# 0215Arthur/Pytorch_News_Recommender

Measured on AMD Instinct MI355X. Metric: users/sec (train step) NRMS MIND-small hist=50 cand=5, higher is better.
Workload: dtype f16 (MFMA inputs and saved activations; fp32 accumulate, softmax, loss, master weights and Adam); 1 GPU; configs[1] shapes: NRMS(nrms_v0) train step, 512 users/GPU, hist=50, cand=5, title_len=30, d=300, h=10, q=200, V=45800, dropout=0.2, Adam(lr=1e-3); users_per_gpu=512, global_batch=512, parallelism=dp1, precision=fp16, resident_batches=32

## Files before the change

include/nrms_hip.h:

```cpp
#ifndef NRMS_HIP_H
#define NRMS_HIP_H

#include <stddef.h>
#include <stdint.h>

#ifdef __cplusplus
extern "C" {
#endif

#define NRMS_OK            0
#define NRMS_EINVAL       -1
#define NRMS_ELAUNCH      -2
#define NRMS_EWORKSPACE   -3

#define NRMS_PRECISION_FP32   0
#define NRMS_PRECISION_BF16X3 1
#define NRMS_PRECISION_BF16   2
#define NRMS_FP16_KP 320
#define NRMS_FP16_DP 320
#define NRMS_FP16_QP 224
#define NRMS_PRECISION_FP16   3

#define NRMS_FLAG_PAD_ROW_ZERO 1
#define NRMS_FLAG_DEFER_WQKV 2
#define NRMS_FLAG_FWD_SCRATCH_KEPT 4
#define NRMS_FLAG_FUSED_SEQ64 8
#define NRMS_FLAG_DEFER_USER_JOIN 16

#define NRMS_FLAG_TABLE_ADAM 32

typedef struct nrms_encoder_desc {
    int32_t  n_seq;
    int32_t  seq_len;
    int32_t  d_model;
    int32_t  n_heads;
    int32_t  q_dim;
    int32_t  vocab;
    float    p_drop_embed;
    float    p_drop_ctx;
    int32_t  precision;
    int32_t  use_output_proj;
    int32_t  mask_mode;
    int32_t  flags;
    uint64_t seed;
    float    loss_scale;
    float    p_drop_attn;
    const int32_t* seq_index;
} nrms_encoder_desc;

typedef struct nrms_encoder_weights {
    const float* table;
    const float* w_qkv;
    const float* b_qkv;
    const float* w_o;
    const float* b_o;
    const float* w_add;
    const float* b_add;
    const float* q_vec;
} nrms_encoder_weights;

typedef struct nrms_encoder_grads {
    float* table;
    float* w_qkv;
    float* b_qkv;
    float* w_o;
    float* b_o;
    float* w_add;
    float* b_add;
    float* q_vec;
} nrms_encoder_grads;

typedef struct nrms_encoder_acts {
    float* x;
    float* qkv;
    float* attn;
    float* ctx;
    float* t;
    float* w;
    void*  scratch;
} nrms_encoder_acts;

size_t nrms_encoder_fwd_scratch_bytes(const nrms_encoder_desc* desc);
size_t nrms_encoder_fused_qkv_bytes(const nrms_encoder_desc* desc);
int nrms_encoder_fwd(const nrms_encoder_desc* desc, const nrms_encoder_weights* w,
                     const int64_t* ids, const float* x, const uint8_t* mask ,
                     const nrms_encoder_acts* acts, float* out, void* stream);

size_t nrms_encoder_bwd_workspace_bytes(const nrms_encoder_desc* desc);
int nrms_encoder_bwd(const nrms_encoder_desc* desc, const nrms_encoder_weights* w,
                     const int64_t* ids, const float* x, const uint8_t* mask,
                     const nrms_encoder_acts* acts, const float* dout,
                     const nrms_encoder_grads* grads, float* dx,
                     void* workspace, size_t workspace_bytes, void* stream);
typedef struct nrms_table_adam {
    float*   param;
    float*   exp_avg;
    float*   exp_avg_sq;
    double   lr, beta1, beta2, eps;
    int32_t  step;
    float    grad_scale;
    int32_t* n_nonfinite;
} nrms_table_adam;
int nrms_encoder_bwd_adam(const nrms_encoder_desc* desc, const nrms_encoder_weights* w,
                          const int64_t* ids, const float* x, const uint8_t* mask,
                          const nrms_encoder_acts* acts, const float* dout,
                          const nrms_encoder_grads* grads, float* dx,
                          void* workspace, size_t workspace_bytes, const nrms_table_adam* table_adam, void* stream);
int nrms_encoder_bwd_wqkv(const nrms_encoder_desc* desc, const int64_t* ids, const float* x,
                          const nrms_encoder_acts* acts, const nrms_encoder_grads* grads,
                          void* workspace, size_t workspace_bytes, void* stream);
int nrms_encoder_join(void* stream);

int nrms_sanitize_ids(const int64_t* src, int64_t* dst, int64_t n, int32_t vocab, int32_t* n_bad, void* stream);
int nrms_sanitize_ids_i32(const int32_t* src, int64_t* dst, int64_t n, int32_t vocab, int32_t* n_bad, void* stream);

int nrms_title_dedup(const int64_t* ids, int64_t n_titles, int32_t seq_len, int32_t* table, int64_t table_size,
                     int32_t* inverse, int32_t* rep_rows, int32_t* n_unique, void* stream);

int nrms_click_score_fwd(int32_t B, int32_t C, int32_t d, const float* cand, const float* user,
                         const uint8_t* mask, float* scores, void* stream);
int nrms_click_score_indexed(int32_t B, int32_t C, int32_t d, const float* news_vec, int64_t n_vec, const int32_t* index,
                             const float* user, const uint8_t* mask, float* scores, void* stream);
int nrms_click_score_bwd(int32_t B, int32_t C, int32_t d, const float* cand, const float* user,
                         const uint8_t* mask, const float* dscores, float* dcand, float* duser,
                         void* stream);

int nrms_ce_loss_fwd_bwd(int32_t B, int32_t C, const float* scores, float* loss_sum,
                         float* dscores, float grad_scale, void* stream);

int nrms_adam_step(size_t n, float* param, const float* grad, float* exp_avg, float* exp_avg_sq,
                   double lr, double beta1, double beta2, double eps, int32_t step, float grad_scale,
                   void* stream);

int nrms_adam_step_guarded(size_t n, float* param, const float* grad, float* exp_avg, float* exp_avg_sq,
                           double lr, double beta1, double beta2, double eps, int32_t step, float grad_scale,
                           int32_t* n_nonfinite, void* stream);
int nrms_adam_step_rest(size_t n, float* param, const float* grad, float* exp_avg, float* exp_avg_sq,
                        double lr, double beta1, double beta2, double eps, int32_t step, float grad_scale,
                        int32_t* n_nonfinite, void* stream);
int nrms_grad_guard(size_t n, float* grad, int32_t* n_nonfinite, void* stream);

int nrms_impression_auc(int32_t n_imp, int32_t max_c, const float* scores, const uint8_t* labels,
                        const int32_t* lens, double* auc, void* stream);

int nrms_impression_metrics(int32_t n_imp, int32_t max_c, const float* scores, const uint8_t* labels,
                            const int32_t* lens, int32_t k_a, int32_t k_b, double* auc, double* mrr, double* ndcg_a,
                            double* ndcg_b, int32_t* ranks, void* stream);

size_t nrms_topk_dot_workspace_bytes(int32_t B, int64_t N, int32_t d, int32_t k);
int nrms_topk_dot(int32_t B, int64_t N, int32_t d, int32_t k, const float* user, const float* items, const int64_t* exclude,
                  int32_t n_exclude, float* top_scores, int64_t* top_ids, void* workspace, size_t workspace_bytes, void* stream);

size_t nrms_topk_grouped_dot_workspace_bytes(int32_t B, int64_t N, int32_t d, int32_t k, int32_t G);
int nrms_topk_grouped_dot(int32_t B, int64_t N, int32_t d, int32_t k, int32_t G, const float* query, const float* items,
                          const int32_t* item_ids, const int64_t* group_ptr, const int64_t* exclude, int32_t n_exclude,
                          float* top_scores, int64_t* top_ids, void* workspace, size_t workspace_bytes, void* stream);

size_t nrms_rank_dot_workspace_bytes(int32_t B, int64_t N, int32_t d, int32_t T, int32_t n_exclude);
int nrms_rank_dot(int32_t B, int64_t N, int32_t d, int32_t T, const float* user, const float* items, const int64_t* targets,
                  const int64_t* exclude, int32_t n_exclude, int32_t* ranks, float* target_scores, void* workspace,
                  size_t workspace_bytes, void* stream);

size_t nrms_topk_dot_biased_workspace_bytes(int32_t B, int64_t N, int32_t d, int32_t k);
int nrms_topk_dot_biased(int32_t B, int64_t N, int32_t d, int32_t k, const float* user, const float* items,
                         const float* bias , const int64_t* exclude, int32_t n_exclude, float* top_scores,
                         int64_t* top_ids, void* workspace, size_t workspace_bytes, void* stream);
size_t nrms_rank_dot_biased_workspace_bytes(int32_t B, int64_t N, int32_t d, int32_t T, int32_t n_exclude);
int nrms_rank_dot_biased(int32_t B, int64_t N, int32_t d, int32_t T, const float* user, const float* items,
                         const float* bias , const int64_t* targets, const int64_t* exclude,
                         int32_t n_exclude, int32_t* ranks, float* target_scores, void* workspace, size_t workspace_bytes,
                         void* stream);

size_t nrms_softmax_sample_dot_workspace_bytes(int32_t B, int64_t N, int32_t d, int32_t S, int32_t n_exclude);
int nrms_softmax_sample_dot(int32_t B, int64_t N, int32_t d, int32_t S, const float* user, const float* items,
                            const int64_t* row_key , float inv_temperature, uint64_t seed,
                            const int64_t* exclude , int32_t n_exclude, int64_t* ids ,
                            float* keys , void* workspace, size_t workspace_bytes, void* stream);
int nrms_softmax_sample_noise(int32_t B, int64_t N, const int64_t* row_key , uint64_t seed,
                              uint32_t* words , float* gumbel , void* stream);

size_t nrms_mmr_rerank_workspace_bytes(int32_t B, int32_t M, int32_t d, int32_t k);
int nrms_mmr_rerank(int32_t B, int32_t M, int32_t d, int32_t k, int64_t N, float lambda,
                    const float* items , const int64_t* short_ids ,
                    const float* short_scores ,
                    int64_t* out_ids , float* out_scores ,
                    float* out_value , float* ild ,
                    void* workspace, size_t workspace_bytes, void* stream);

int nrms_layernorm_fwd(int64_t n_rows, int32_t d, const float* x, const float* gamma, const float* beta, float eps,
                       float* y, float* stats, void* stream);
size_t nrms_layernorm_bwd_workspace_bytes(int32_t d);
int nrms_layernorm_bwd(int64_t n_rows, int32_t d, const float* x, const float* gamma, const float* stats, const float* dy,
                       float* dx, float* dgamma_dbeta, void* workspace, size_t workspace_bytes, void* stream);

typedef struct nrms_news_features {
    int64_t n;
    int32_t d_text;
    int32_t d_cat;
    int32_t n_cat, n_sub;
    float   p_drop;
    uint64_t seed;
    const float* title_vec;
    const float* abst_vec;
    const float* cat_table;
    const float* sub_table;
    const int64_t* categ;
    const int64_t* subcateg;
} nrms_news_features;
// ... 130 lines not shown
```

pytorch_news_recommender_amd/_lib.py:

```python
from __future__ import annotations

import ctypes as C
import os

PKG = os.path.dirname(os.path.abspath(__file__))
LIB_PATH = os.environ.get("NRMS_HIP_LIB") or os.path.join(PKG, "libnrms_hip.so")

NRMS_OK, NRMS_EINVAL, NRMS_ELAUNCH, NRMS_EWORKSPACE = 0, -1, -2, -3
NRMS_FLAG_PAD_ROW_ZERO = 1
NRMS_FLAG_DEFER_WQKV = 2
NRMS_FLAG_FWD_SCRATCH_KEPT = 4
NRMS_FLAG_FUSED_SEQ64 = 8
NRMS_FLAG_DEFER_USER_JOIN = 16
NRMS_FLAG_TABLE_ADAM = 32
NRMS_PRECISION_FP32 = 0
NRMS_PRECISION_BF16X3 = 1
NRMS_PRECISION_BF16 = 2
NRMS_PRECISION_FP16 = 3
NRMS_DROPOUT_FIELDS16 = 0x100
NRMS_DROPOUT_SITE_NEWSVEC = 4
NRMS_FP16_KP, NRMS_FP16_DP, NRMS_FP16_QP = 320, 320, 224
PRECISIONS = {"fp32": 0, "bf16x3": 1, "bf16": 2, "fp16": 3}


class NrmsError(RuntimeError):
    pass


class EncoderDesc(C.Structure):
    _fields_ = [("n_seq", C.c_int32), ("seq_len", C.c_int32), ("d_model", C.c_int32),
                ("n_heads", C.c_int32), ("q_dim", C.c_int32), ("vocab", C.c_int32),
                ("p_drop_embed", C.c_float), ("p_drop_ctx", C.c_float), ("precision", C.c_int32),
                ("use_output_proj", C.c_int32), ("mask_mode", C.c_int32), ("flags", C.c_int32),
                ("seed", C.c_uint64), ("loss_scale", C.c_float), ("p_drop_attn", C.c_float), ("seq_index", C.c_void_p)]


class EncoderWeights(C.Structure):
    _fields_ = [("table", C.c_void_p), ("w_qkv", C.c_void_p), ("b_qkv", C.c_void_p), ("w_o", C.c_void_p),
                ("b_o", C.c_void_p), ("w_add", C.c_void_p), ("b_add", C.c_void_p), ("q_vec", C.c_void_p)]


class EncoderGrads(C.Structure):
    _fields_ = [("table", C.c_void_p), ("w_qkv", C.c_void_p), ("b_qkv", C.c_void_p), ("w_o", C.c_void_p),
                ("b_o", C.c_void_p), ("w_add", C.c_void_p), ("b_add", C.c_void_p), ("q_vec", C.c_void_p)]


class TableAdam(C.Structure):
    _fields_ = [("param", C.c_void_p), ("exp_avg", C.c_void_p), ("exp_avg_sq", C.c_void_p), ("lr", C.c_double), ("beta1", C.c_double),
                ("beta2", C.c_double), ("eps", C.c_double), ("step", C.c_int32), ("grad_scale", C.c_float), ("n_nonfinite", C.c_void_p)]


class EncoderActs(C.Structure):
    _fields_ = [("x", C.c_void_p), ("qkv", C.c_void_p), ("attn", C.c_void_p), ("ctx", C.c_void_p),
                ("t", C.c_void_p), ("w", C.c_void_p), ("scratch", C.c_void_p)]


class SegPoolDesc(C.Structure):
    _fields_ = [("n_rows", C.c_int64), ("n_seg", C.c_int64), ("nnz", C.c_int64), ("d", C.c_int32), ("q", C.c_int32),
                ("precision", C.c_int32), ("flags", C.c_int32)]


NRMS_SEGPOOL_ROWS_UNIQUE = 1


class ClickGraphDesc(C.Structure):
    _fields_ = [("n_users", C.c_int64), ("n_news", C.c_int64), ("n_edges", C.c_int64), ("user_ptr", C.c_void_p),
                ("user_news", C.c_void_p), ("news_ptr", C.c_void_p), ("news_users", C.c_void_p)]


class NewsFeatures(C.Structure):
    _fields_ = [("n", C.c_int64), ("d_text", C.c_int32), ("d_cat", C.c_int32), ("n_cat", C.c_int32), ("n_sub", C.c_int32),
                ("p_drop", C.c_float), ("seed", C.c_uint64), ("title_vec", C.c_void_p), ("abst_vec", C.c_void_p),
                ("cat_table", C.c_void_p), ("sub_table", C.c_void_p), ("categ", C.c_void_p), ("subcateg", C.c_void_p)]


class NewsvecDesc(C.Structure):
    _fields_ = [("n_slots", C.c_int64), ("n_rows", C.c_int32), ("d", C.c_int32), ("precision", C.c_int32),
                ("p_drop", C.c_float), ("seed", C.c_uint64)]


SIGNATURES = {
    "nrms_encoder_fwd": (C.c_int, [C.POINTER(EncoderDesc), C.POINTER(EncoderWeights), C.c_void_p, C.c_void_p,
                                   C.c_void_p, C.POINTER(EncoderActs), C.c_void_p, C.c_void_p]),
    "nrms_encoder_bwd_workspace_bytes": (C.c_size_t, [C.POINTER(EncoderDesc)]),
    "nrms_encoder_fwd_scratch_bytes": (C.c_size_t, [C.POINTER(EncoderDesc)]),
    "nrms_encoder_fused_qkv_bytes": (C.c_size_t, [C.POINTER(EncoderDesc)]),
    "nrms_encoder_bwd": (C.c_int, [C.POINTER(EncoderDesc), C.POINTER(EncoderWeights), C.c_void_p, C.c_void_p,
                                   C.c_void_p, C.POINTER(EncoderActs), C.c_void_p, C.POINTER(EncoderGrads), C.c_void_p,
                                   C.c_void_p, C.c_size_t, C.c_void_p]),
    "nrms_encoder_bwd_adam": (C.c_int, [C.POINTER(EncoderDesc), C.POINTER(EncoderWeights), C.c_void_p, C.c_void_p,
                                        C.c_void_p, C.POINTER(EncoderActs), C.c_void_p, C.POINTER(EncoderGrads), C.c_void_p,
                                        C.c_void_p, C.c_size_t, C.POINTER(TableAdam), C.c_void_p]),
    "nrms_encoder_bwd_wqkv": (C.c_int, [C.POINTER(EncoderDesc), C.c_void_p, C.c_void_p, C.POINTER(EncoderActs),
                                        C.POINTER(EncoderGrads), C.c_void_p, C.c_size_t, C.c_void_p]),
    "nrms_encoder_join": (C.c_int, [C.c_void_p]),
    "nrms_sanitize_ids": (C.c_int, [C.c_void_p, C.c_void_p, C.c_int64, C.c_int32, C.c_void_p, C.c_void_p]),
    "nrms_sanitize_ids_i32": (C.c_int, [C.c_void_p, C.c_void_p, C.c_int64, C.c_int32, C.c_void_p, C.c_void_p]),
    "nrms_title_dedup": (C.c_int, [C.c_void_p, C.c_int64, C.c_int32, C.c_void_p, C.c_int64, C.c_void_p, C.c_void_p,
                                   C.c_void_p, C.c_void_p]),
    "nrms_click_score_indexed": (C.c_int, [C.c_int32, C.c_int32, C.c_int32, C.c_void_p, C.c_int64, C.c_void_p, C.c_void_p,
                                           C.c_void_p, C.c_void_p, C.c_void_p]),
    "nrms_click_score_fwd": (C.c_int, [C.c_int32, C.c_int32, C.c_int32, C.c_void_p, C.c_void_p, C.c_void_p,
                                       C.c_void_p, C.c_void_p]),
    "nrms_click_score_bwd": (C.c_int, [C.c_int32, C.c_int32, C.c_int32, C.c_void_p, C.c_void_p, C.c_void_p,
                                       C.c_void_p, C.c_void_p, C.c_void_p, C.c_void_p]),
    "nrms_ce_loss_fwd_bwd": (C.c_int, [C.c_int32, C.c_int32, C.c_void_p, C.c_void_p, C.c_void_p, C.c_float,
                                       C.c_void_p]),
    "nrms_adam_step": (C.c_int, [C.c_size_t, C.c_void_p, C.c_void_p, C.c_void_p, C.c_void_p, C.c_double,
                                 C.c_double, C.c_double, C.c_double, C.c_int32, C.c_float, C.c_void_p]),
    "nrms_adam_step_guarded": (C.c_int, [C.c_size_t, C.c_void_p, C.c_void_p, C.c_void_p, C.c_void_p, C.c_double,
                                         C.c_double, C.c_double, C.c_double, C.c_int32, C.c_float, C.c_void_p, C.c_void_p]),
    "nrms_adam_step_rest": (C.c_int, [C.c_size_t, C.c_void_p, C.c_void_p, C.c_void_p, C.c_void_p, C.c_double,
                                      C.c_double, C.c_double, C.c_double, C.c_int32, C.c_float, C.c_void_p, C.c_void_p]),
    "nrms_grad_guard": (C.c_int, [C.c_size_t, C.c_void_p, C.c_void_p, C.c_void_p]),
    "nrms_segment_pool_workspace_bytes": (C.c_size_t, [C.POINTER(SegPoolDesc)]),
    "nrms_segment_pool_fwd": (C.c_int, [C.POINTER(SegPoolDesc)] + [C.c_void_p] * 10 + [C.c_void_p, C.c_size_t, C.c_void_p]),
    "nrms_segment_pool_bwd": (C.c_int, [C.POINTER(SegPoolDesc)] + [C.c_void_p] * 12 + [C.c_void_p, C.c_size_t, C.c_void_p]),
    "nrms_hier_tree_scratch_bytes": (C.c_size_t, [C.c_int32, C.c_int32]),
    "nrms_hier_tree_build": (C.c_int, [C.c_int32, C.c_int32] + [C.c_void_p] * 16 + [C.c_size_t, C.c_void_p]),
    "nrms_hier_add_embedding_fwd": (C.c_int, [C.c_int64, C.c_int32, C.c_int32, C.c_void_p, C.c_void_p, C.c_void_p, C.c_void_p, C.c_void_p]),
    "nrms_sequence_partition_count_ints": (C.c_size_t, [C.c_int32]),
    "nrms_sequence_partition": (C.c_int, [C.c_void_p, C.c_int32, C.c_int32, C.c_void_p, C.c_void_p, C.c_void_p]),
    "nrms_encoder_empty_workspace_bytes": (C.c_size_t, [C.POINTER(EncoderDesc)]),
    "nrms_encoder_empty_saved_bytes": (C.c_size_t, [C.POINTER(EncoderDesc)]),
    "nrms_encoder_empty_fwd": (C.c_int, [C.POINTER(EncoderDesc), C.POINTER(EncoderWeights), C.c_void_p, C.c_void_p, C.c_void_p, C.c_void_p, C.c_size_t,
                                         C.c_void_p]),
    "nrms_encoder_empty_bwd": (C.c_int, [C.POINTER(EncoderDesc), C.POINTER(EncoderWeights), C.c_void_p, C.c_void_p, C.c_void_p, C.POINTER(EncoderGrads),
                                         C.c_void_p, C.c_size_t, C.c_void_p]),
    "nrms_csr_from_padded": (C.c_int, [C.c_int64, C.c_int32, C.c_void_p, C.c_int64, C.c_void_p, C.c_void_p, C.c_void_p]),
    "nrms_graph_sample_workspace_bytes": (C.c_size_t, [C.c_int64, C.c_int32]),
    "nrms_graph_sample_neighbors": (C.c_int, [C.POINTER(ClickGraphDesc), C.c_int64, C.c_int32, C.c_void_p, C.c_uint64, C.c_void_p, C.c_void_p,
                                              C.c_void_p, C.c_size_t, C.c_void_p]),
    "nrms_graph_resolve_workspace_bytes": (C.c_size_t, [C.c_int64]),
    "nrms_graph_resolve_rows": (C.c_int, [C.c_int64, C.c_int32, C.c_int64, C.c_void_p, C.c_void_p, C.c_int32] + [C.c_void_p] * 4
                                + [C.c_void_p, C.c_size_t, C.c_void_p]),
    "nrms_negative_sample_workspace_bytes": (C.c_size_t, [C.c_int64, C.c_int64, C.c_int32]),
    "nrms_negative_sample": (C.c_int, [C.c_int64] + [C.c_void_p] * 4 + [C.c_int32, C.c_int32, C.c_uint64] + [C.c_void_p] * 3
                             + [C.c_void_p, C.c_size_t, C.c_void_p]),
    "nrms_catalogue_negative_sample_workspace_bytes": (C.c_size_t, [C.c_int64, C.c_int64, C.c_int32]),
    "nrms_catalogue_negative_sample": (C.c_int, [C.c_int64] + [C.c_void_p] * 3 + [C.c_int64, C.c_void_p, C.c_void_p, C.c_int64, C.c_void_p, C.c_int32,
                                                 C.c_uint64] + [C.c_void_p] * 4 + [C.c_void_p, C.c_size_t, C.c_void_p]),
    "nrms_hier_add_embedding_bwd_workspace_bytes": (C.c_size_t, [C.c_int64, C.c_int32, C.c_int32]),
    "nrms_hier_add_embedding_bwd": (C.c_int, [C.c_int64, C.c_int32, C.c_int32, C.c_void_p, C.c_void_p, C.c_void_p, C.c_void_p, C.c_void_p,
                                              C.c_size_t, C.c_void_p]),
    "nrms_hier_match": (C.c_int, [C.c_int32, C.c_int32, C.c_int32] + [C.c_void_p] * 11 + [C.c_void_p]),
    "nrms_hier_score_fwd": (C.c_int, [C.c_int32, C.c_int32, C.c_int32] + [C.c_void_p] * 9 + [C.c_float, C.c_float, C.c_void_p, C.c_void_p]),
    "nrms_hier_score_bwd": (C.c_int, [C.c_int32, C.c_int32, C.c_int32] + [C.c_void_p] * 9 + [C.c_float, C.c_float] + [C.c_void_p] * 5 + [C.c_void_p]),
    "nrms_impression_auc": (C.c_int, [C.c_int32, C.c_int32, C.c_void_p, C.c_void_p, C.c_void_p, C.c_void_p,
                                      C.c_void_p]),
    "nrms_impression_metrics": (C.c_int, [C.c_int32, C.c_int32, C.c_void_p, C.c_void_p, C.c_void_p, C.c_int32, C.c_int32]
                                + [C.c_void_p] * 5 + [C.c_void_p]),
    "nrms_topk_dot_workspace_bytes": (C.c_size_t, [C.c_int32, C.c_int64, C.c_int32, C.c_int32]),
    "nrms_topk_dot": (C.c_int, [C.c_int32, C.c_int64, C.c_int32, C.c_int32, C.c_void_p, C.c_void_p, C.c_void_p, C.c_int32,
                                C.c_void_p, C.c_void_p, C.c_void_p, C.c_size_t, C.c_void_p]),
    "nrms_topk_grouped_dot_workspace_bytes": (C.c_size_t, [C.c_int32, C.c_int64, C.c_int32, C.c_int32, C.c_int32]),
    "nrms_topk_grouped_dot": (C.c_int, [C.c_int32, C.c_int64, C.c_int32, C.c_int32, C.c_int32] + [C.c_void_p] * 5 + [C.c_int32]
                              + [C.c_void_p] * 3 + [C.c_size_t, C.c_void_p]),
    "nrms_rank_dot_workspace_bytes": (C.c_size_t, [C.c_int32, C.c_int64, C.c_int32, C.c_int32, C.c_int32]),
    "nrms_rank_dot": (C.c_int, [C.c_int32, C.c_int64, C.c_int32, C.c_int32] + [C.c_void_p] * 4 + [C.c_int32]
                      + [C.c_void_p] * 3 + [C.c_size_t, C.c_void_p]),
    "nrms_topk_dot_biased_workspace_bytes": (C.c_size_t, [C.c_int32, C.c_int64, C.c_int32, C.c_int32]),
    "nrms_topk_dot_biased": (C.c_int, [C.c_int32, C.c_int64, C.c_int32, C.c_int32] + [C.c_void_p] * 4 + [C.c_int32]
                             + [C.c_void_p] * 3 + [C.c_size_t, C.c_void_p]),
    "nrms_rank_dot_biased_workspace_bytes": (C.c_size_t, [C.c_int32, C.c_int64, C.c_int32, C.c_int32, C.c_int32]),
    "nrms_rank_dot_biased": (C.c_int, [C.c_int32, C.c_int64, C.c_int32, C.c_int32] + [C.c_void_p] * 5 + [C.c_int32]
                             + [C.c_void_p] * 3 + [C.c_size_t, C.c_void_p]),
    "nrms_softmax_sample_dot_workspace_bytes": (C.c_size_t, [C.c_int32, C.c_int64, C.c_int32, C.c_int32, C.c_int32]),
    "nrms_softmax_sample_dot": (C.c_int, [C.c_int32, C.c_int64, C.c_int32, C.c_int32] + [C.c_void_p] * 3 + [C.c_float, C.c_uint64, C.c_void_p,
                                          C.c_int32] + [C.c_void_p] * 3 + [C.c_size_t, C.c_void_p]),
    "nrms_mmr_rerank_workspace_bytes": (C.c_size_t, [C.c_int32] * 4),
    "nrms_mmr_rerank": (C.c_int, [C.c_int32] * 4 + [C.c_int64, C.c_float] + [C.c_void_p] * 8 + [C.c_size_t, C.c_void_p]),
    "nrms_softmax_sample_noise": (C.c_int, [C.c_int32, C.c_int64, C.c_void_p, C.c_uint64, C.c_void_p, C.c_void_p, C.c_void_p]),
    "nrms_hier_query": (C.c_int, [C.c_int32] * 4 + [C.c_void_p] * 10 + [C.c_float, C.c_float, C.c_void_p, C.c_void_p]),
    "nrms_dropout_keep_mask": (C.c_int, [C.c_uint64, C.c_int32, C.c_int64, C.c_int32, C.c_float, C.c_void_p,
                                         C.c_void_p]),
    "nrms_layernorm_fwd": (C.c_int, [C.c_int64, C.c_int32, C.c_void_p, C.c_void_p, C.c_void_p, C.c_float, C.c_void_p,
                                     C.c_void_p, C.c_void_p]),
    "nrms_layernorm_bwd_workspace_bytes": (C.c_size_t, [C.c_int32]),
    "nrms_layernorm_bwd": (C.c_int, [C.c_int64, C.c_int32, C.c_void_p, C.c_void_p, C.c_void_p, C.c_void_p, C.c_void_p,
                                     C.c_void_p, C.c_void_p, C.c_size_t, C.c_void_p]),
    "nrms_news_features_fwd": (C.c_int, [C.POINTER(NewsFeatures), C.c_void_p, C.c_void_p]),
    "nrms_news_features_bwd": (C.c_int, [C.POINTER(NewsFeatures), C.c_void_p, C.c_void_p, C.c_void_p, C.c_void_p,
                                         C.c_void_p, C.c_void_p]),
    "nrms_newsvec_saved_bytes": (C.c_size_t, [C.POINTER(NewsvecDesc)]),
    "nrms_newsvec_workspace_bytes": (C.c_size_t, [C.POINTER(NewsvecDesc)]),
    "nrms_newsvec_fwd": (C.c_int, [C.POINTER(NewsvecDesc)] + [C.c_void_p] * 6 + [C.c_size_t, C.c_void_p, C.c_void_p, C.c_size_t,
                                                                                C.c_void_p]),
    "nrms_newsvec_bwd": (C.c_int, [C.POINTER(NewsvecDesc)] + [C.c_void_p] * 4 + [C.c_size_t] + [C.c_void_p] * 4
# ... 44 lines not shown
```

pytorch_news_recommender_amd/csrc/capi.hip:

```cpp
#include <stdarg.h>

#include <algorithm>

#include <mutex>
#include <vector>

#include "gemm.h"

namespace nrms {

int launch_attention(bool bwd, int n_seq, int S, int d, int h, const float* qkv, float* ctx, const Dropout& drop,
                     const float* dctx, float* dqkv, const uint8_t* mask, const int64_t* ids, const float* bias_hm,
                     const int* pos, float* padsum, float* dbias, hipStream_t stream, const Dropout* pdrop = nullptr,
                     bool split = false);
size_t attention_padsum_floats();
int launch_addattn_fwd(int n_seq, int S, int d, int q, const float* ctx, const float* w_add, const float* b_add,
                       const float* q_vec, float* T, float* wout, float* out, const uint8_t* mask, int npass,
                       void* wplanes, hipStream_t stream);
int addattn_bwd_rows_waves(int n_seq);
int launch_addattn_bwd_rows(int n_seq, int S, int d, int q, const float* ctx, const float* dout, const float* w,
                            const float* T, float* ds, float* dq_partial, float* dq, const uint8_t* mask,
                            hipStream_t stream);

int launch_attention_wide(bool bwd, int n_seq, int S, int d, int h, const float* qkv, float* ctx, const Dropout& pdrop,
// ... 274 lines not shown
        if (!forked) return NRMS_OK;
        forked = false;
        if (hipEventRecord(ss->ev[4], s_prep) != hipSuccess || hipStreamWaitEvent(s, ss->ev[4], 0) != hipSuccess) {
            set_error("encoder_fwd(fp16): joining the helper stream failed");
            return NRMS_ELAUNCH;
        }
        return NRMS_OK;
    };
    rc = v1 ? launch_prep16v1(d, h, q, w->w_qkv, w->b_qkv, w->w_o, w->b_o, w->w_add, w->b_add, w->q_vec, base + fs.planes, s_prep)
            : launch_prep16(d, h, q, w->w_qkv, w->b_qkv, w->w_add, w->b_add, w->q_vec, base + fs.planes, s_prep);
    if (rc) { (void)join_prep(); return rc; }
    Fused16Fwd f{};
    f.n_seq = desc->n_seq; f.S = S; f.d = d; f.h = h; f.q = q;
    f.planes = base + fs.planes; f.x16 = acts->x; f.ctx16 = acts->ctx; f.t16 = acts->t; f.w = acts->w; f.out = out;
    f.drop = make_dropout(desc->seed, desc->p_drop_ctx);
    if (gather) {
        const Dropout drop_e = make_dropout(desc->seed, desc->p_drop_embed);
        if (skip_pad_rows(desc)) {
            int* live = (int*)(base + fs.live);
            int* pos = (int*)(base + fs.pos);
            int* n_live = (int*)(base + fs.n_live);
            int* order = (int*)(base + fs.order);
            int* order_cnt = (int*)(base + fs.order_cnt);
            rc = S <= 32 ? launch_title_order(desc->n_seq, S, ids, order, order_cnt, s_prep, 3) : NRMS_OK;
            if (rc) { (void)join_prep(); return rc; }
            rc = launch_compact_live_rows(M, ids, live, pos, n_live, (int*)(base + fs.cscr), s);
            if (rc == NRMS_OK) rc = launch_gather16(M, d, L.KP, ids, live, n_live, w->table, drop_e, acts->x, s);
            const int rj = join_prep();
            if (rc) return rc;
            if (rj) return rj;
            f.pos = pos;
            f.n_rows = n_live;
            f.ids = ids;
            if (S <= 32) { f.order = order; f.order_cnt = order_cnt; }
        } else {
            rc = launch_gather16(M, d, L.KP, ids, nullptr, nullptr, w->table, drop_e, acts->x, s);
            if (rc) return rc;
        }
    } else {
        rc = launch_cast16(M, d, L.KP, x, acts->x, s);
        if (rc) return rc;
    }
    rc = v1 ? launch_fused_fwd16v1(f, h, acts->attn, s) : launch_fused_fwd16(f, s);
    if (rc == NRMS_OK && gather && skip_pad_rows(desc)) kept_record(desc, acts->scratch, ids);
    return rc;
}

struct Bwd16Layout { size_t fused, live, pos, n_live, cscr, order, order_cnt, dxc, sscr, total; };
static Bwd16Layout bwd16_layout(const nrms_encoder_desc* d) {
    Bwd16Layout L;
    const size_t M = (size_t)d->n_seq * d->seq_len;
    const bool gather = d->vocab > 0;
    size_t off = 0;
    auto take = [&](size_t bytes) { size_t o = off; off = align_up(off + bytes, 256); return o; };
    L.fused = take(d->use_output_proj ? fused16v1_bwd_bytes((long)M, d->n_seq, d->n_heads) : fused16_bwd_layout((long)M, d->n_seq).total);
    L.live = take(gather ? M * sizeof(int) : 0);
    L.pos = take(gather ? M * sizeof(int) : 0);
    L.n_live = take(gather ? 256 : 0);
    L.cscr = take(gather ? compact_scratch_ints((long)M) * sizeof(int) : 0);
    L.order = take(gather ? (size_t)3 * d->n_seq * sizeof(int) : 0);
    L.order_cnt = take(gather ? title_order_cnt_ints(d->n_seq) * sizeof(int) : 0);
    L.dxc = take(gather ? M * std::max((size_t)d->d_model * sizeof(float), (size_t)NRMS_FP16_KP * 2) : 0);
    L.sscr = take(gather ? scatter_grouped_scratch_ints((long)M, d->vocab) * sizeof(int) : 0);
    L.total = off;
    return L;
}

static int table_adam_args(const nrms_encoder_desc* desc, const nrms_encoder_weights* w, const nrms_encoder_grads* grads,
                           const nrms_table_adam* ta, TableAdam* out) {
    NRMS_REQUIRE(ta->param && ta->exp_avg && ta->exp_avg_sq && ta->step >= 1, "encoder_bwd: NRMS_FLAG_TABLE_ADAM: bad operands");
    NRMS_REQUIRE(w != nullptr && ta->param == w->table, "encoder_bwd: NRMS_FLAG_TABLE_ADAM: param must be the table the encoder reads");
    NRMS_REQUIRE(grads != nullptr && grads->table != nullptr, "encoder_bwd: NRMS_FLAG_TABLE_ADAM: grads.table missing");
    NRMS_REQUIRE((((uintptr_t)ta->param | (uintptr_t)grads->table | (uintptr_t)ta->exp_avg | (uintptr_t)ta->exp_avg_sq) & 15) == 0,
                 "encoder_bwd: NRMS_FLAG_TABLE_ADAM: buffers must be 16-byte aligned");
    out->p = ta->param; out->m = ta->exp_avg; out->v = ta->exp_avg_sq;
    out->c = adam_consts(ta->lr, ta->beta1, ta->beta2, ta->eps, ta->step);
    out->gscale = ta->grad_scale;
    out->n_bad = (int*)ta->n_nonfinite;
    return NRMS_OK;
}

static int encoder_bwd16(const nrms_encoder_desc* desc, const nrms_encoder_weights* w, const int64_t* ids, const float* x,
                         const nrms_encoder_acts* acts, const float* dout, const nrms_encoder_grads* grads, float* dx,
                         void* workspace, size_t workspace_bytes, const TableAdam* tadam, hipStream_t s) {
    NRMS_REQUIRE(w && acts && dout && grads && workspace, "encoder_bwd(fp16): null argument");
    const bool v1 = desc->use_output_proj != 0;
    NRMS_REQUIRE(!v1 || (w->w_o && acts->attn && grads->w_o && grads->b_o),
                 "encoder_bwd(fp16): use_output_proj needs w_o, acts.attn, grads.w_o, grads.b_o");
    NRMS_REQUIRE(acts->x && acts->ctx && acts->t && acts->w, "encoder_bwd(fp16): acts.x, ctx, t, w are required");
    NRMS_REQUIRE(grads->w_qkv && grads->b_qkv && grads->w_add && grads->b_add && grads->q_vec, "encoder_bwd(fp16): null gradient buffer");
    const bool gather = desc->vocab > 0;
    NRMS_REQUIRE(gather ? (ids != nullptr && grads->table != nullptr) : (dx != nullptr), "encoder_bwd(fp16): %s missing",
                 gather ? "ids / grads.table" : "dx");
    const Bwd16Layout L = bwd16_layout(desc);
    if (workspace_bytes < L.total) { set_error("encoder_bwd(fp16): workspace %zu < required %zu bytes", workspace_bytes, L.total); return NRMS_EWORKSPACE; }
    NRMS_REQUIRE(((uintptr_t)workspace & 255) == 0, "encoder_bwd(fp16): workspace must be 256-byte aligned");
    if (desc->n_seq == 0) return NRMS_OK;
    const int S = desc->seq_len, d = desc->d_model;
    const long M = (long)desc->n_seq * S;
    char* base = (char*)workspace;
    Fused16Bwd f{};
    f.n_seq = desc->n_seq; f.S = S; f.d = d; f.h = desc->n_heads; f.q = desc->q_dim;
    f.workspace = base + L.fused;
    f.w_qkv = w->w_qkv; f.b_qkv = w->b_qkv; f.w_add = w->w_add; f.q_vec = w->q_vec;
    f.x16 = acts->x; f.ctx16 = acts->ctx; f.t16 = acts->t; f.w = acts->w; f.dout = dout;
    f.loss_scale = desc->loss_scale;
    f.drop = make_dropout(desc->seed, desc->p_drop_ctx);
    f.dw_qkv = grads->w_qkv; f.db_qkv = grads->b_qkv; f.dw_add = grads->w_add; f.db_add = grads->b_add; f.dq_vec = grads->q_vec;
    if (v1) { f.w_o = w->w_o; f.attn16 = acts->attn; f.dw_o = grads->w_o; f.db_o = grads->b_o; }
    int rc;
    int* live = (int*)(base + L.live);
    int* n_live = (int*)(base + L.n_live);
    if (gather) {
        const bool kept = (desc->flags & NRMS_FLAG_FWD_SCRATCH_KEPT) != 0 && skip_pad_rows(desc) && acts->scratch != nullptr &&
                          kept_matches(desc, acts->scratch, ids);
        if (kept) {
            const Fwd16Scratch fs = fwd16_scratch(desc);
            char* fb = (char*)acts->scratch;
            live = (int*)(fb + fs.live);
            n_live = (int*)(fb + fs.n_live);
            f.pos = (int*)(fb + fs.pos); f.n_rows_dev = n_live; f.ids = ids;
            if (S <= 32) { f.order = (int*)(fb + fs.order); f.order_cnt = (int*)(fb + fs.order_cnt); }
        } else {
            int* pos = (int*)(base + L.pos);
            rc = launch_compact_live_rows(M, ids, live, pos, n_live, (int*)(base + L.cscr), s);
            if (rc) return rc;
            if (skip_pad_rows(desc)) {
                int* order = (int*)(base + L.order);
                int* order_cnt = (int*)(base + L.order_cnt);
                f.pos = pos; f.n_rows_dev = n_live; f.ids = ids;
                if (S <= 32) {
                    rc = launch_title_order(desc->n_seq, S, ids, order, order_cnt, s, 3);
                    if (rc) return rc;
                    f.order = order; f.order_cnt = order_cnt;
                }
            }
        }
        f.dx = (float*)(base + L.dxc);
        f.dx_fp16 = skip_pad_rows(desc);
    } else {
        f.dx = dx;
    }
    SideSet* ss_prep = (gather && skip_pad_rows(desc)) ? side_streams_for(s) : nullptr;
    bool prepared = false;
    if (ss_prep != nullptr) {
        rc = side_order(ss_prep, 5, s, ss_prep->s[1], "encoder_bwd(fp16)");
        if (rc) return rc;
        rc = launch_scatter_prepare(M, desc->vocab, ids, live, n_live, (int*)(base + L.sscr), ss_prep->s[1]);
        if (hipEventRecord(ss_prep->ev[4], ss_prep->s[1]) != hipSuccess) { set_error("encoder_bwd(fp16): hipEventRecord failed"); return NRMS_ELAUNCH; }
        if (rc) { (void)hipStreamWaitEvent(s, ss_prep->ev[4], 0); return rc; }
        prepared = true;
    }
    auto join_prepare = [&]() -> int {
        if (!prepared) return NRMS_OK;
        if (hipStreamWaitEvent(s, ss_prep->ev[4], 0) != hipSuccess) { set_error("encoder_bwd(fp16): hipStreamWaitEvent failed"); return NRMS_ELAUNCH; }
        return NRMS_OK;
    };
    const float* sc_dev = nullptr;
    f.sc_out = &sc_dev;
    f.defer_join = (desc->flags & NRMS_FLAG_DEFER_WQKV) != 0;
    rc = v1 ? launch_fused_bwd16v1(f, s) : launch_fused_bwd16(f, s);
    {
        const int rj = join_prepare();
        if (rc) return rc;
        if (rj) return rj;
    }
    if (gather) {
        const Dropout drop_e = make_dropout(desc->seed, desc->p_drop_embed);
        if (tadam != nullptr)
            rc = launch_scatter_grouped_adam(M, desc->vocab, d, ids, live, n_live, f.dx, drop_e, grads->table, (int*)(base + L.sscr), s,
                                             f.dx_fp16, NRMS_FP16_KP, sc_dev, prepared, *tadam);
        else if (skip_pad_rows(desc))
            rc = launch_scatter_grouped(M, desc->vocab, d, ids, live, n_live, f.dx, drop_e, grads->table, (int*)(base + L.sscr), s,
                                        f.dx_fp16, NRMS_FP16_KP, sc_dev, prepared);
        else
            rc = launch_scatter_dense_rows(M, d, ids, live, n_live, f.dx, drop_e, grads->table, s);
    }
    return rc;
}

extern "C" int nrms_encoder_fwd(const nrms_encoder_desc* desc, const nrms_encoder_weights* w, const int64_t* ids,
                                const float* x, const uint8_t* mask, const nrms_encoder_acts* acts, float* out,
                                void* stream) {
    int rc = validate_desc(desc, "encoder_fwd");
    if (rc) return rc;
    NRMS_REQUIRE((desc->flags & NRMS_FLAG_TABLE_ADAM) == 0, "encoder_fwd: flags 0x%x: NRMS_FLAG_TABLE_ADAM belongs to nrms_encoder_bwd_adam", desc->flags);
    if (acts != nullptr) kept_forget(acts->scratch);
    if (desc->precision == NRMS_PRECISION_FP16) {
        NRMS_REQUIRE(w && acts && out, "encoder_fwd: null argument");
        NRMS_REQUIRE(w->w_qkv && w->b_qkv && w->w_add && w->b_add && w->q_vec, "encoder_fwd: null weight");
        NRMS_REQUIRE(desc->vocab > 0 ? (ids != nullptr && w->table != nullptr) : (x != nullptr), "encoder_fwd: input missing");
        if (desc->n_seq == 0) return NRMS_OK;
        return encoder_fwd16(desc, w, ids, x, acts, out, (hipStream_t)stream);
    }
    NRMS_REQUIRE(w && acts && out, "encoder_fwd: null argument");
    NRMS_REQUIRE(w->w_qkv && w->b_qkv && w->w_add && w->b_add && w->q_vec, "encoder_fwd: null weight");
    if (desc->flags & NRMS_FLAG_FUSED_SEQ64) {
        NRMS_REQUIRE(x != nullptr && acts->qkv != nullptr && acts->scratch != nullptr, "encoder_fwd(fused): x, acts.qkv and acts.scratch are required");
        const bool train = acts->ctx != nullptr && acts->t != nullptr && acts->w != nullptr;
        if (desc->n_seq == 0) return NRMS_OK;
        rc = fused_bwd16_join((hipStream_t)stream);
        if (rc) return rc;
        return launch_user64_fwd(desc->n_seq, desc->seq_len, desc->d_model, desc->n_heads, desc->q_dim, x, w->w_qkv, w->b_qkv, w->w_add,
                                 w->b_add, w->q_vec, acts->scratch, acts->ctx, acts->t, acts->w, acts->qkv, out, train, (hipStream_t)stream);
    }
    NRMS_REQUIRE(acts->qkv && acts->ctx, "encoder_fwd: acts.qkv / acts.ctx are required");
    const bool gather = desc->vocab > 0, wo = desc->use_output_proj != 0;
    NRMS_REQUIRE(gather ? (ids != nullptr && w->table != nullptr) : (x != nullptr),
                 "encoder_fwd: %s input missing", gather ? "ids/table" : "x");
    NRMS_REQUIRE(!wo || (w->w_o && w->b_o && acts->attn), "encoder_fwd: use_output_proj needs w_o, b_o and acts.attn");
    NRMS_REQUIRE(desc->mask_mode == 0 || mask != nullptr, "encoder_fwd: mask_mode=%d but mask is null", desc->mask_mode);
    if (desc->n_seq == 0) return NRMS_OK;
    hipStream_t s = (hipStream_t)stream;
    const int S = desc->seq_len, d = desc->d_model, q = desc->q_dim, M = desc->n_seq * S;
    const Dropout drop_e = make_dropout(desc->seed, desc->p_drop_embed);
    const Dropout drop_c = make_dropout(desc->seed, desc->p_drop_ctx);
    const Dropout no_drop = make_dropout(0, 0.f);
    const uint8_t* amask = (desc->mask_mode & 1) ? mask : nullptr;
    const uint8_t* pmask = (desc->mask_mode & 2) ? mask : nullptr;

    NRMS_REQUIRE(acts->scratch != nullptr, "encoder_fwd: acts.scratch (nrms_encoder_fwd_scratch_bytes) is required");
    const FwdScratch fs = fwd_scratch(desc);
    float* wq_hm = (float*)((char*)acts->scratch + fs.wq);
    float* bq_hm = (float*)((char*)acts->scratch + fs.bq);
    void* wplanes = (char*)acts->scratch + fs.planes;
    const HeadPerm perm{d / desc->n_heads, desc->n_heads};
    rc = launch_permute_rows(w->w_qkv, w->b_qkv, wq_hm, bq_hm, 3 * d, d, perm, s);
    if (rc) return rc;

    NTArgs g{};
    g.M = M; g.N = 3 * d; g.K = d; g.rows_per_tile = NT_BM;
    g.W = wq_hm; g.bias = bq_hm; g.C = acts->qkv; g.ldc = 3 * d;
    const float* xin = x;
    if (gather) {
        NRMS_REQUIRE(acts->x != nullptr, "encoder_fwd: acts.x (gathered embeddings) is required for the news encoder");
        if (skip_pad_rows(desc)) {
            int* live = (int*)((char*)acts->scratch + fs.live);
            int* n_live = (int*)((char*)acts->scratch + fs.n_live);
            int* cscr = (int*)((char*)acts->scratch + fs.cscr);
            rc = launch_compact_live_rows((long)M, ids, live, nullptr, n_live, cscr, s);
            if (rc) return rc;
            rc = launch_gather_dropout_compact((long)M, d, ids, live, n_live, w->table, drop_e, acts->x, s);
            if (rc) return rc;
// ... 72 lines not shown
        if (e.device == dev && e.caller == caller) return e.set;
    if (g_side_sets.size() >= 32) return nullptr;
    SideSet* ss = new SideSet();
    bool ok = true;
    for (int i = 0; i < 2 && ok; ++i) ok = hipStreamCreateWithFlags(&ss->s[i], hipStreamNonBlocking) == hipSuccess;
    for (int i = 0; i < SIDE_EVENTS && ok; ++i) ok = hipEventCreateWithFlags(&ss->ev[i], hipEventDisableTiming) == hipSuccess;
    if (!ok) {
        for (int i = 0; i < 2; ++i) if (ss->s[i]) (void)hipStreamDestroy(ss->s[i]);
        for (int i = 0; i < SIDE_EVENTS; ++i) if (ss->ev[i]) (void)hipEventDestroy(ss->ev[i]);
        delete ss;
        ss = nullptr;
        (void)hipGetLastError();
    }
    g_side_sets.push_back(SideEntry{dev, caller, ss});
    return ss;
}

int side_order(SideSet* ss, int e, hipStream_t from, hipStream_t to, const char* what) {
    if (hipEventRecord(ss->ev[e], from) != hipSuccess || hipStreamWaitEvent(to, ss->ev[e], 0) != hipSuccess) {
        set_error("%s: ordering the helper stream failed: %s", what, hipGetErrorString(hipGetLastError()));
        return NRMS_ELAUNCH;
    }
    return NRMS_OK;
}

int side_join_user(SideSet* ss, hipStream_t caller, const char* what) {
    if (ss == nullptr || !ss->pending_user) return NRMS_OK;
    ss->pending_user = false;
    if (hipStreamWaitEvent(caller, ss->ev[SIDE_EV_USER], 0) != hipSuccess) {
        set_error("%s: hipStreamWaitEvent failed", what);
        return NRMS_ELAUNCH;
    }
    return NRMS_OK;
}

SideJoinGuard::~SideJoinGuard() {
    if (!armed) return;
    for (int i = 0; i < 2; ++i)
        if (hipEventRecord(ss->ev[6 + i], ss->s[i]) == hipSuccess) (void)hipStreamWaitEvent(caller, ss->ev[6 + i], 0);
}
}

static int bwd_wqkv(const nrms_encoder_desc* desc, const float* xin, const float* dqkv, const int* n_live,
                    const nrms_encoder_grads* grads, float* tn_partial, hipStream_t s) {
    const int d = desc->d_model, M = desc->n_seq * desc->seq_len;
    TNArgs t{};
    t.M = M; t.N = 3 * d; t.K = d; t.amode = A_PLAIN;
    t.A = dqkv; t.lda = 3 * d; t.B = xin; t.ldb = d;
    t.dW = grads->w_qkv; t.dbias = grads->b_qkv; t.partial = tn_partial;
    t.perm = HeadPerm{d / desc->n_heads, desc->n_heads};
    if (skip_pad_rows(desc)) t.m_dev = n_live;
    return tn_gemm(desc, t, s, "dwqkv_bwd");
}

extern "C" int nrms_encoder_bwd_wqkv(const nrms_encoder_desc* desc, const int64_t* ids, const float* x,
                                     const nrms_encoder_acts* acts, const nrms_encoder_grads* grads, void* workspace,
                                     size_t workspace_bytes, void* stream) {
    int rc = validate_desc(desc, "encoder_bwd_wqkv");
    if (rc) return rc;
    NRMS_REQUIRE((desc->flags & NRMS_FLAG_TABLE_ADAM) == 0, "encoder_bwd_wqkv: flags 0x%x: NRMS_FLAG_TABLE_ADAM belongs to nrms_encoder_bwd_adam", desc->flags);
    if (desc->precision == NRMS_PRECISION_FP16) return fused_bwd16_join((hipStream_t)stream);
    NRMS_REQUIRE(acts && grads && workspace, "encoder_bwd_wqkv: null argument");
    NRMS_REQUIRE(grads->w_qkv && grads->b_qkv, "encoder_bwd_wqkv: null gradient buffer");
    const bool gather = desc->vocab > 0;
    NRMS_REQUIRE(gather ? (ids != nullptr && acts->x != nullptr) : (x != nullptr), "encoder_bwd_wqkv: input missing");
    if (desc->n_seq == 0) return NRMS_OK;
    const BwdWorkspace L = bwd_layout(desc);
    if (workspace_bytes < L.total) {
        set_error("encoder_bwd_wqkv: workspace %zu < required %zu bytes", workspace_bytes, L.total);
        return NRMS_EWORKSPACE;
    }
    rc = fused_bwd16_join((hipStream_t)stream);
    if (rc) return rc;
    char* base = (char*)workspace;
    return bwd_wqkv(desc, gather ? acts->x : x, (const float*)(base + L.dqkv), (const int*)(base + L.n_live), grads,
                    (float*)(base + L.tn_partial), (hipStream_t)stream);
}

extern "C" int nrms_encoder_join(void* stream) { return fused_bwd16_join((hipStream_t)stream); }

static int encoder_bwd_chain(const nrms_encoder_desc* desc, const nrms_encoder_weights* w, const int64_t* ids,
                             const float* x, const uint8_t* mask, const nrms_encoder_acts* acts, const float* dout,
                             const nrms_encoder_grads* grads, float* dx, void* workspace, size_t workspace_bytes,
                             const TableAdam* tadam, hipStream_t s) {
    int rc;
    NRMS_REQUIRE(w && acts && dout && grads && workspace, "encoder_bwd: null argument");
    NRMS_REQUIRE(acts->qkv && acts->ctx && acts->t && acts->w, "encoder_bwd: all saved activations are required");
    NRMS_REQUIRE(grads->w_qkv && grads->b_qkv && grads->w_add && grads->b_add && grads->q_vec,
                 "encoder_bwd: null gradient buffer");
    const bool gather = desc->vocab > 0, wo = desc->use_output_proj != 0;
    NRMS_REQUIRE(gather ? (ids != nullptr && acts->x != nullptr && grads->table != nullptr) : (x != nullptr && dx != nullptr),
                 "encoder_bwd: %s missing", gather ? "ids/acts.x/grads.table" : "x/dx");
    NRMS_REQUIRE(!wo || (w->w_o && acts->attn && grads->w_o && grads->b_o),
                 "encoder_bwd: use_output_proj needs w_o, acts.attn, grads.w_o, grads.b_o");
    NRMS_REQUIRE(desc->mask_mode == 0 || mask != nullptr, "encoder_bwd: mask_mode=%d but mask is null", desc->mask_mode);
    const BwdWorkspace L = bwd_layout(desc);
    if (workspace_bytes < L.total) {
        set_error("encoder_bwd: workspace %zu < required %zu bytes", workspace_bytes, L.total);
        return NRMS_EWORKSPACE;
    }
    NRMS_REQUIRE(((uintptr_t)workspace & 255) == 0, "encoder_bwd: workspace must be 256-byte aligned");
    if (desc->n_seq == 0) return NRMS_OK;
    const int S = desc->seq_len, d = desc->d_model, q = desc->q_dim, M = desc->n_seq * S;
    const Dropout drop_e = make_dropout(desc->seed, desc->p_drop_embed);
    const Dropout drop_c = make_dropout(desc->seed, desc->p_drop_ctx);
    const Dropout no_drop = make_dropout(0, 0.f);
    const uint8_t* amask = (desc->mask_mode & 1) ? mask : nullptr;
    const uint8_t* pmask = (desc->mask_mode & 2) ? mask : nullptr;
    char* base = (char*)workspace;
    float* dctx = (float*)(base + L.dctx);
    float* dqkv = (float*)(base + L.dqkv);
    float* dattn = (float*)(base + L.dattn);
    float* ds = (float*)(base + L.ds);
    float* wqkv_t = (float*)(base + L.wqkv_t);
    float* wadd_t = (float*)(base + L.wadd_t);
    float* wo_t = (float*)(base + L.wo_t);
    float* tn_partial = (float*)(base + L.tn_partial);
    float* dq_partial = (float*)(base + L.dq_partial);
    void* wplanes = (void*)(base + L.wplanes);

    rc = fused_bwd16_join(s);
    if (rc) return rc;
    SideSet* ss = side_streams_for(s);
    const bool side = ss != nullptr;
    hipStream_t s2 = side ? ss->s[0] : s;
    SideJoinGuard join_guard(ss, s);
    auto fork = [&](int i) -> int {
        return side ? side_order(ss, i, s, s2, "encoder_bwd") : NRMS_OK;
    };

    const bool fused64 = (desc->flags & NRMS_FLAG_FUSED_SEQ64) != 0;
    if (fused64) {
        rc = launch_user64_bwd(desc->n_seq, S, d, desc->n_heads, q, w->w_add, w->q_vec, base + L.u64planes, dout, acts->t, acts->w,
                               acts->qkv, ds, dq_partial, grads->q_vec, dqkv, s);
        if (rc) return rc;
    } else {
        if (wide_additive(desc))
            rc = launch_addattn_rows_bwd_wide(desc->n_seq, S, d, q, acts->ctx, dout, acts->w, acts->t, ds, dq_partial, grads->q_vec,
                                              pmask, s);
        else
            rc = launch_addattn_bwd_rows(desc->n_seq, S, d, q, acts->ctx, dout, acts->w, acts->t, ds, dq_partial, grads->q_vec,
                                         pmask, s);
        if (rc) return rc;
    }
    rc = fork(0);
    if (rc) return rc;
    {
        TNArgs t{};
        t.M = M; t.N = q; t.K = d; t.amode = A_DZ;
        t.ds = ds; t.qv = w->q_vec; t.T = acts->t; t.B = acts->ctx; t.ldb = d;
        t.dW = grads->w_add; t.dbias = grads->b_add; t.partial = tn_partial;
        rc = tn_gemm(desc, t, s2, "dwadd_bwd");
        if (rc) return rc;
    }
    if (!fused64) {
        rc = launch_transpose(w->w_add, wadd_t, q, d, s);
        if (rc) return rc;
        {
            NTArgs g{};
            g.M = M; g.N = d; g.K = q; g.rows_per_tile = NT_BM;
            g.ds = ds; g.qv = w->q_vec; g.T = acts->t;
            g.W = wadd_t; g.C = dctx; g.ldc = d;
            g.wrow = acts->w; g.dout = dout; g.seq_of_row = make_row_div((uint32_t)S);
            g.drop = drop_c;
            rc = nt_gemm(desc, A_DZ, E_DCTX, g, wplanes, s, "dctx_bwd");
            if (rc) return rc;
        }
}
    const float* dattn_in = dctx;
    if (wo) {
        rc = fork(1);
        if (rc) return rc;
        TNArgs t{};
        t.M = M; t.N = d; t.K = d; t.amode = A_PLAIN;
        t.A = dctx; t.lda = d; t.B = acts->attn; t.ldb = d;
        t.dW = grads->w_o; t.dbias = grads->b_o; t.partial = tn_partial;
        rc = tn_gemm(desc, t, s2, "dwo_bwd");
        if (rc) return rc;
        if (side && hipEventRecord(ss->ev[3], s2) != hipSuccess) {
            set_error("encoder_bwd: hipEventRecord failed");
            return NRMS_ELAUNCH;
        }
        rc = launch_transpose(w->w_o, wo_t, d, d, s);
        if (rc) return rc;
        NTArgs g{};
        g.M = M; g.N = d; g.K = d; g.rows_per_tile = NT_BM;
        g.A = dctx; g.lda = d; g.W = wo_t; g.C = dattn; g.ldc = d;
        rc = nt_gemm(desc, A_PLAIN, E_STORE, g, wplanes, s, "dattn_bwd");
        if (rc) return rc;
        dattn_in = dattn;
    }
    int* live = (int*)(base + L.live);
    int* pos = (int*)(base + L.pos);
    int* n_live = (int*)(base + L.n_live);
    const bool compact = skip_pad_rows(desc);
    const HeadPerm perm{d / desc->n_heads, desc->n_heads};
    if (gather) {
        rc = launch_compact_live_rows((long)M, ids, live, compact ? pos : nullptr, n_live, (int*)(base + L.cscr), s);
        if (rc) return rc;
    }
    Dropout pdrop_attn = make_dropout(desc->seed, desc->p_drop_attn);
    pdrop_attn.seq_index = desc->seq_index; pdrop_attn.seq_h = desc->n_heads;
    if (fused64)
        rc = NRMS_OK;
    else if (wide_attention(desc))
        rc = launch_attention_wide(true, desc->n_seq, S, d, desc->n_heads, acts->qkv, nullptr, pdrop_attn, dattn_in, dqkv, amask, s);
    else
        rc = launch_attention(true, desc->n_seq, S, d, desc->n_heads, acts->qkv, nullptr, no_drop, dattn_in, dqkv, amask,
                              nullptr, nullptr, compact ? pos : nullptr, compact ? (float*)(base + L.padsum) : nullptr,
                              compact ? grads->b_qkv : nullptr, s, &pdrop_attn, desc->precision != NRMS_PRECISION_FP32);
    if (rc) return rc;
    if ((desc->flags & NRMS_FLAG_DEFER_WQKV) == 0) {
        rc = fork(2);
        if (rc) return rc;
        rc = bwd_wqkv(desc, gather ? acts->x : x, dqkv, n_live, grads, tn_partial, s2);
        if (rc) return rc;
    }
    rc = launch_transpose(w->w_qkv, wqkv_t, 3 * d, d, s, perm);
    if (rc) return rc;
    {
        NTArgs g{};
        g.M = M; g.N = d; g.K = 3 * d; g.rows_per_tile = NT_BM;
        g.A = dqkv; g.lda = 3 * d; g.W = wqkv_t;
        g.C = gather ? dctx : dx; g.ldc = d;
        if (gather) { g.a_rows = compact ? nullptr : live; g.m_dev = n_live; }
        if (side && wo && gather && hipStreamWaitEvent(s, ss->ev[3], 0) != hipSuccess) {
            set_error("encoder_bwd: hipStreamWaitEvent failed");
            return NRMS_ELAUNCH;
        }
        rc = nt_gemm(desc, A_PLAIN, E_STORE, g, wplanes, s, "dx_bwd");
        if (rc) return rc;
    }
    if (gather) {
        const bool atomic_scatter = getenv("NRMS_ATOMIC_SCATTER") != nullptr;
        if (tadam != nullptr)
            rc = launch_scatter_grouped_adam((long)M, desc->vocab, d, ids, live, n_live, dctx, drop_e, grads->table,
                                             (int*)(base + L.sscr), s, false, 0, nullptr, false, *tadam);
        else if (atomic_scatter) rc = launch_scatter_dropout_compact((long)M, d, ids, live, n_live, dctx, drop_e, grads->table, s);
        else rc = launch_scatter_grouped((long)M, desc->vocab, d, ids, live, n_live, dctx, drop_e, grads->table,
                                         (int*)(base + L.sscr), s);
    }
    if (side && rc == NRMS_OK) {
        if (!gather && (desc->flags & NRMS_FLAG_DEFER_USER_JOIN) != 0) {
            if (hipEventRecord(ss->ev[SIDE_EV_USER], s2) != hipSuccess) { set_error("encoder_bwd: hipEventRecord failed"); return NRMS_ELAUNCH; }
            ss->pending_user = true;
            join_guard.disarm();
        } else {
            rc = side_order(ss, 4, s2, s, "encoder_bwd");
            if (rc == NRMS_OK) join_guard.disarm();
        }
    }
    return rc;
}

extern "C" int nrms_encoder_bwd(const nrms_encoder_desc* desc, const nrms_encoder_weights* w, const int64_t* ids,
                                const float* x, const uint8_t* mask, const nrms_encoder_acts* acts, const float* dout,
                                const nrms_encoder_grads* grads, float* dx, void* workspace, size_t workspace_bytes,
                                void* stream) {
    return nrms_encoder_bwd_adam(desc, w, ids, x, mask, acts, dout, grads, dx, workspace, workspace_bytes, nullptr, stream);
}

extern "C" int nrms_encoder_bwd_adam(const nrms_encoder_desc* desc, const nrms_encoder_weights* w, const int64_t* ids,
                                     const float* x, const uint8_t* mask, const nrms_encoder_acts* acts, const float* dout,
                                     const nrms_encoder_grads* grads, float* dx, void* workspace, size_t workspace_bytes,
                                     const nrms_table_adam* table_adam, void* stream) {
    int rc = validate_desc(desc, "encoder_bwd");
    if (rc) return rc;
    NRMS_REQUIRE(((desc->flags & NRMS_FLAG_TABLE_ADAM) != 0) == (table_adam != nullptr),
                 "encoder_bwd: NRMS_FLAG_TABLE_ADAM and the nrms_table_adam operands (nrms_encoder_bwd_adam) go together");
    TableAdam tadam_v{};
    const TableAdam* tadam = nullptr;
    if (table_adam != nullptr) {
        rc = table_adam_args(desc, w, grads, table_adam, &tadam_v);
        if (rc) return rc;
        tadam = &tadam_v;
        NRMS_REQUIRE(desc->precision == NRMS_PRECISION_FP16 || getenv("NRMS_ATOMIC_SCATTER") == nullptr,
                     "encoder_bwd: NRMS_FLAG_TABLE_ADAM needs the grouped scatter (NRMS_ATOMIC_SCATTER is set)");
    }
    if (desc->precision == NRMS_PRECISION_FP16)
        rc = encoder_bwd16(desc, w, ids, x, acts, dout, grads, dx, workspace, workspace_bytes, tadam, (hipStream_t)stream);
    else
        rc = encoder_bwd_chain(desc, w, ids, x, mask, acts, dout, grads, dx, workspace, workspace_bytes, tadam, (hipStream_t)stream);
    if (rc == NRMS_OK && tadam != nullptr && desc->n_seq == 0) {
        const size_t n = (size_t)desc->vocab * desc->d_model;
        if (hipMemsetAsync(grads->table, 0, n * sizeof(float), (hipStream_t)stream) != hipSuccess) {
            set_error("encoder_bwd: memset failed");
            return NRMS_ELAUNCH;
        }
        rc = table_adam->n_nonfinite != nullptr
                 ? nrms_adam_step_guarded(n, table_adam->param, grads->table, table_adam->exp_avg, table_adam->exp_avg_sq, table_adam->lr,
                                          table_adam->beta1, table_adam->beta2, table_adam->eps, table_adam->step, table_adam->grad_scale,
                                          table_adam->n_nonfinite, stream)
                 : nrms_adam_step(n, table_adam->param, grads->table, table_adam->exp_avg, table_adam->exp_avg_sq, table_adam->lr,
                                  table_adam->beta1, table_adam->beta2, table_adam->eps, table_adam->step, table_adam->grad_scale, stream);
    }
    return rc;
}

extern "C" int nrms_layernorm_fwd(int64_t n_rows, int32_t d, const float* x, const float* gamma, const float* beta, float eps,
                                  float* y, float* stats, void* stream) {
    NRMS_REQUIRE(n_rows >= 0 && d > 0 && eps > 0.f, "layernorm_fwd: n_rows=%ld d=%d eps=%g", (long)n_rows, d, (double)eps);
    NRMS_REQUIRE(n_rows == 0 || (x && gamma && beta && y), "layernorm_fwd: null argument");
    return launch_layernorm_fwd((long)n_rows, d, x, gamma, beta, eps, y, stats, (hipStream_t)stream);
}

extern "C" size_t nrms_layernorm_bwd_workspace_bytes(int32_t d) { return d > 0 ? layernorm_bwd_workspace_floats(d) * sizeof(float) : 0; }

extern "C" int nrms_layernorm_bwd(int64_t n_rows, int32_t d, const float* x, const float* gamma, const float* stats,
                                  const float* dy, float* dx, float* dgamma_dbeta, void* workspace, size_t workspace_bytes,
                                  void* stream) {
    NRMS_REQUIRE(n_rows >= 0 && d > 0, "layernorm_bwd: n_rows=%ld d=%d", (long)n_rows, d);
    NRMS_REQUIRE(n_rows == 0 || (x && gamma && stats && dy && dx && dgamma_dbeta && workspace), "layernorm_bwd: null argument");
    if (workspace_bytes < nrms_layernorm_bwd_workspace_bytes(d)) {
        set_error("layernorm_bwd: workspace %zu < required %zu bytes", workspace_bytes, nrms_layernorm_bwd_workspace_bytes(d));
        return NRMS_EWORKSPACE;
    }
    return launch_layernorm_bwd((long)n_rows, d, x, gamma, stats, dy, dx, dgamma_dbeta, (float*)workspace, (hipStream_t)stream);
}

static int features_args(const nrms_news_features* f, FeatArgs* a, const char* who) {
    NRMS_REQUIRE(f != nullptr, "%s: null descriptor", who);
    NRMS_REQUIRE(f->n >= 0 && f->d_text > 0 && f->d_cat > 0 && f->n_cat > 0 && f->n_sub > 0, "%s: bad sizes", who);
    NRMS_REQUIRE(f->p_drop >= 0.f && f->p_drop < 1.f, "%s: p_drop must be in [0,1)", who);
    NRMS_REQUIRE((long)f->n * (2 * f->d_text + 2 * f->d_cat) < (1L << 40), "%s: too many elements", who);
    NRMS_REQUIRE(f->n == 0 || (f->categ && f->subcateg), "%s: null ids", who);
    a->n = (long)f->n; a->dt = f->d_text; a->dc = f->d_cat; a->n_cat = f->n_cat; a->n_sub = f->n_sub;
    a->title = f->title_vec; a->abst = f->abst_vec; a->cat_table = f->cat_table; a->sub_table = f->sub_table;
    a->categ = f->categ; a->subcateg = f->subcateg;
    a->drop = make_dropout(f->seed, f->p_drop);
    return NRMS_OK;
}

extern "C" int nrms_news_features_fwd(const nrms_news_features* f, float* out, void* stream) {
    FeatArgs a{};
    int rc = features_args(f, &a, "news_features_fwd");
    if (rc) return rc;
    NRMS_REQUIRE(f->n == 0 || (f->title_vec && f->abst_vec && f->cat_table && f->sub_table && out), "news_features_fwd: null argument");
    a.out = out;
    return launch_features_fwd(a, (hipStream_t)stream);
}

extern "C" int nrms_news_features_bwd(const nrms_news_features* f, const float* dout, float* d_title_vec, float* d_abst_vec,
                                      float* d_cat_table, float* d_sub_table, void* stream) {
    FeatArgs a{};
    int rc = features_args(f, &a, "news_features_bwd");
    if (rc) return rc;
    NRMS_REQUIRE(f->n == 0 || (dout && d_title_vec && d_abst_vec && d_cat_table && d_sub_table), "news_features_bwd: null argument");
    a.dout = dout; a.d_title = d_title_vec; a.d_abst = d_abst_vec; a.d_cat_table = d_cat_table; a.d_sub_table = d_sub_table;
    return launch_features_bwd(a, (hipStream_t)stream);
}

extern "C" int nrms_sanitize_ids(const int64_t* src, int64_t* dst, int64_t n, int32_t vocab, int32_t* n_bad, void* stream) {
    NRMS_REQUIRE(n >= 0 && vocab > 0, "sanitize_ids: n=%ld vocab=%d", (long)n, vocab);
    NRMS_REQUIRE(n == 0 || (src && dst && n_bad), "sanitize_ids: null argument");
    return launch_sanitize_ids((long)n, src, false, dst, vocab, n_bad, (hipStream_t)stream);
}

extern "C" int nrms_sanitize_ids_i32(const int32_t* src, int64_t* dst, int64_t n, int32_t vocab, int32_t* n_bad, void* stream) {
    NRMS_REQUIRE(n >= 0 && vocab > 0, "sanitize_ids_i32: n=%ld vocab=%d", (long)n, vocab);
    NRMS_REQUIRE(n == 0 || (src && dst && n_bad), "sanitize_ids_i32: null argument");
    return launch_sanitize_ids((long)n, src, true, dst, vocab, n_bad, (hipStream_t)stream);
}

extern "C" size_t nrms_sequence_partition_count_ints(int32_t n_seq) { return n_seq >= 0 ? title_order_cnt_ints(n_seq) : 0; }

// ... 50 lines not shown
```

pytorch_news_recommender_amd/csrc/common.h:

```cpp
#pragma once
#include <hip/hip_runtime.h>
#include <stdint.h>
#include <stdio.h>
#include <string>

#include "../../include/nrms_hip.h"

namespace nrms {

typedef float f32x4 __attribute__((ext_vector_type(4)));
typedef float f32x16 __attribute__((ext_vector_type(16)));

constexpr int WAVE = 64;

__device__ __forceinline__ f32x4 mfma16(float a, float b, f32x4 c) {
    return __builtin_amdgcn_mfma_f32_16x16x4f32(a, b, c, 0, 0, 0);
}
__device__ __forceinline__ f32x16 mfma32(float a, float b, f32x16 c) {
    return __builtin_amdgcn_mfma_f32_32x32x2f32(a, b, c, 0, 0, 0);
}
__device__ __forceinline__ int crow32(int r, int hh) { return (r & 3) + 8 * (r >> 2) + 4 * hh; }

struct Keep4 { bool k[4]; };

// ... 54 lines not shown
    uint32_t r[4];
    philox4x32_7(seed, group8, site, r);
#pragma unroll
    for (int w = 0; w < 4; ++w) {
        s[2 * w] = (r[w] & 0xFFFFu) >= thresh16 ? inv_keep : 0.f;
        s[2 * w + 1] = (r[w] >> 16) >= thresh16 ? inv_keep : 0.f;
    }
}
__device__ __forceinline__ float dropout_scale1(uint64_t seed, uint32_t site, uint64_t elem,
                                                uint32_t thresh, float inv_keep) {
    uint32_t r[4];
    philox4x32_7(seed, elem >> 2, site, r);
    return r[elem & 3] >= thresh ? inv_keep : 0.f;
}

__device__ __forceinline__ float fast_tanh(float x) {
    const float e = __expf(2.0f * x);
    const float r = 1.0f - 2.0f * __builtin_amdgcn_rcpf(e + 1.0f);
    const float x2 = x * x;
    const float p = x * (1.0f + x2 * (-0.33333333f + x2 * (0.13333333f + x2 * -0.053968254f)));
    return fabsf(x) < 0.12f ? p : r;
}

struct HeadPerm {
    int dk, h;
    __host__ __device__ __forceinline__ int src(int np) const {
        if (dk == 0) return np;
        const int head = np / (3 * dk), r = np - head * 3 * dk;
        const int which = r / dk, j = r - which * dk;
        return which * h * dk + head * dk + j;
    }
};

struct Dropout {
    uint64_t seed;
    uint32_t thresh;
    float inv_keep;
    uint32_t thresh16;
    const int* seq_index;
    int seq_h;
    __device__ __forceinline__ long unit_of(long unit) const {
        if (seq_index == nullptr) return unit;
        const long seq = unit / seq_h;
        return (long)seq_index[seq] * seq_h + (unit - seq * seq_h);
    }
};

inline Dropout make_dropout(uint64_t seed, float p) {
    Dropout d;
    d.seed = seed;
    d.thresh = drop_threshold(p);
    d.thresh16 = drop_threshold16(p);
    d.inv_keep = p > 0.f ? 1.0f / (1.0f - p) : 1.0f;
    d.seq_index = nullptr;
    d.seq_h = 1;
    return d;
}

__device__ __forceinline__ float wave_sum(float v) {
#pragma unroll
    for (int o = 32; o > 0; o >>= 1) v += __shfl_xor(v, o, 64);
    return v;
}
__device__ __forceinline__ float wave_max(float v) {
#pragma unroll
    for (int o = 32; o > 0; o >>= 1) v = fmaxf(v, __shfl_xor(v, o, 64));
    return v;
}

__device__ __forceinline__ void adam_update(float& p, float& m, float& v, float g, float step_size, float b1, float b2, float omb1,
                                            float omb2, float inv_sqrt_bc2, float eps) {
#pragma clang fp contract(off)
    m = b1 * m + omb1 * g;
    v = b2 * v + omb2 * g * g;
    const float denom = sqrtf(v) * inv_sqrt_bc2 + eps;
    p = __builtin_fmaf(-step_size, m / denom, p);
}
struct AdamConsts { float step_size, b1, b2, omb1, omb2, inv_sqrt_bc2, eps; };
AdamConsts adam_consts(double lr, double beta1, double beta2, double eps, int32_t step);

void set_error(const char* fmt, ...);
int check_launch(const char* what);

constexpr int SIDE_EVENTS = 9, SIDE_EV_USER = 8;
struct SideSet {
    hipStream_t s[2] = {nullptr, nullptr};
    hipEvent_t ev[SIDE_EVENTS] = {nullptr, nullptr, nullptr, nullptr, nullptr, nullptr, nullptr, nullptr, nullptr};
    bool pending = false;
    bool pending_user = false;
};
int side_join_user(SideSet* ss, hipStream_t caller, const char* what);
SideSet* side_streams_for(hipStream_t caller);
int side_order(SideSet* ss, int e, hipStream_t from, hipStream_t to, const char* what);
struct SideJoinGuard {
    SideSet* ss; hipStream_t caller; bool armed;
    SideJoinGuard(SideSet* set, hipStream_t c) : ss(set), caller(c), armed(set != nullptr) {}
    void disarm() { armed = false; }
    ~SideJoinGuard();
};

struct TimingScope {
    TimingScope(const char* name, hipStream_t s);
    ~TimingScope();
    bool active;
    int slot;
    hipStream_t stream;
};

#define NRMS_REQUIRE(cond, ...)                         \
    do {                                                \
        if (!(cond)) {                                  \
            ::nrms::set_error(__VA_ARGS__);             \
            return NRMS_EINVAL;                         \
        }                                               \
    } while (0)

__host__ __device__ inline int cdiv(long a, long b) { return (int)((a + b - 1) / b); }

}
```

pytorch_news_recommender_amd/csrc/fused16_bwd.hip:

```cpp
#include <stdlib.h>

#include "fused16_bwd.h"

namespace nrms {

template <int SB>
__global__ __launch_bounds__(F16_THREADS, SB == 1 ? 8 / F16_WAVES : 1) void fused_bwd16_pool_kernel(Bwd16Args a) {
    extern __shared__ __attribute__((aligned(16))) char smem[];
    float* red = reinterpret_cast<float*>(smem + 3 * F16_SLOT);
    float* stg_t = red + B16_RED;
    float* stg_h = stg_t + F16_WAVES * SB * 2 * F16_QT * 32;
    const int tid = threadIdx.x, lane = tid & 63;
    const int wave = __builtin_amdgcn_readfirstlane(tid >> 6);
    const int l32 = lane & 31, hh = lane >> 5;
    const int S = a.S;
    constexpr int DP = F16_DP, QP = F16_QP;

    for (int i = tid; i < B16_RED; i += F16_THREADS) red[i] = 0.f;

    h8 idf[2], sel[2];
#pragma unroll
    for (int s = 0; s < 2; ++s)
#pragma unroll
        for (int j = 0; j < 8; ++j) {
// ... 800 lines not shown
            }
        }
#pragma unroll
        for (int i = 0; i < T16_B_IT; ++i) {
            int r, c;
            slot_rc(tid + T16_THREADS * i, T16_BW, r, c);
            if (r < T16_MC) {
                const bool ok = m0 + r < m_end && kcol0 + c < a.K;
                *reinterpret_cast<h8*>(st + T16_A_BYTES + (r * T16_PB + c) * 2) = ok ? R.b[i] : z8;
            }
        }
    };
    f32x4 acc[T16_NTN][T16_NTK];
#pragma unroll
    for (int i = 0; i < T16_NTN; ++i)
#pragma unroll
        for (int j = 0; j < T16_NTK; ++j) acc[i][j] = f32x4{0.f, 0.f, 0.f, 0.f};
    auto compute = [&](const char* st) {
        h8 bf[T16_NTK];
#pragma unroll
        for (int j = 0; j < T16_NTK; ++j) bf[j] = tr16_frag(st + T16_A_BYTES, T16_PB * 2, (wk * T16_NTK + j) * 16, lane);
#pragma unroll
        for (int i = 0; i < T16_NTN; ++i) {
            const h8 af = tr16_frag(st, T16_PA * 2, (wn * T16_NTN + i) * 16, lane);
#pragma unroll
            for (int j = 0; j < T16_NTK; ++j) acc[i][j] = __builtin_amdgcn_mfma_f32_16x16x32_f16(af, bf[j], acc[i][j], 0, 0, 0);
        }
    };
    int n_stage = m_end > m_begin ? (m_end - m_begin + T16_MC - 1) / T16_MC : 0;
    if (n_stage > 0) {
        n_stage = (n_stage + 1) & ~1;
        Regs R0, R1;
        load_stage(R1, m_begin);
        store_stage(R1, m_begin, smem);
        load_stage(R0, m_begin + T16_MC);
        __syncthreads();
        auto body = [&](const Regs& Rs, Regs& Rl, int s) {
            load_stage(Rl, m_begin + (s + 2) * T16_MC);
            store_stage(Rs, m_begin + (s + 1) * T16_MC, smem + ((s + 1) & 1) * T16_STAGE);
            compute(smem + (s & 1) * T16_STAGE);
            __syncthreads();
        };
        for (int s = 0; s < n_stage; s += 2) {
            body(R0, R1, s);
            body(R1, R0, s + 1);
        }
    }
    float* slab = a.partial + (long)split * a.N * a.K;
    const int r16 = lane & 15, kq = lane >> 4;
#pragma unroll
    for (int i = 0; i < T16_NTN; ++i)
#pragma unroll
        for (int j = 0; j < T16_NTK; ++j)
#pragma unroll
            for (int reg = 0; reg < 4; ++reg) {
                const int nn = ncol0 + (wn * T16_NTN + i) * 16 + 4 * kq + reg;
                const int kk = kcol0 + (wk * T16_NTK + j) * 16 + r16;
                if (nn < a.N && kk < a.K) slab[(long)nn * a.K + kk] = acc[i][j][reg];
            }
}

__global__ void tn16_reduce_kernel(const float* partial, int splits, int N, int K, const int* nmap, const int* kmap,
                                   const float* nscale, int ldw, float* dW, float* dbias) {
    const long total = (long)N * K;
    for (long idx = (long)blockIdx.x * blockDim.x + threadIdx.x; idx < total; idx += (long)gridDim.x * blockDim.x) {
        const int n = (int)(idx / K), k = (int)(idx - (long)n * K);
        const int nd = nmap[n], kd = kmap[k];
        if (nd < 0 || kd == -1 || (kd < 0 && dbias == nullptr)) continue;
        const float* pp = partial + idx;
        float s[8] = {0.f, 0.f, 0.f, 0.f, 0.f, 0.f, 0.f, 0.f};
        int sp = 0;
        for (; sp + 8 <= splits; sp += 8) {
#pragma unroll
            for (int u = 0; u < 8; ++u) s[u] += pp[(long)(sp + u) * total];
        }
        for (; sp < splits; ++sp) s[0] += pp[(long)sp * total];
        const float tot = (((s[0] + s[1]) + (s[2] + s[3])) + ((s[4] + s[5]) + (s[6] + s[7]))) * nscale[n];
        if (kd >= 0) dW[(long)nd * ldw + kd] += tot;
        else dbias[nd] += tot;
    }
}

__global__ __launch_bounds__(1024) void red16_kernel(const float* red, int n_wg, int h, int dk, int d, int q, const float* sc,
                                                    float qscale, float* db_qkv, float* db_add, float* dq_vec) {
    const float inv_scale = sc[1];
    __shared__ float part[32][33];
    const int c = threadIdx.x & 31, rg = threadIdx.x >> 5;
    const int i = blockIdx.x * 32 + c;
    float s = 0.f;
    if (i < B16_RED) {
        float s0 = 0.f, s1 = 0.f, s2 = 0.f, s3 = 0.f;
        int g = rg;
        for (; g + 96 < n_wg; g += 128) {
            s0 += red[(long)g * B16_RED + i];
            s1 += red[(long)(g + 32) * B16_RED + i];
            s2 += red[(long)(g + 64) * B16_RED + i];
            s3 += red[(long)(g + 96) * B16_RED + i];
        }
        for (; g < n_wg; g += 32) s0 += red[(long)g * B16_RED + i];
        s = (s0 + s1) + (s2 + s3);
    }
    part[rg][c] = s;
    __syncthreads();
    if (rg != 0 || i >= B16_RED) return;
    s = 0.f;
#pragma unroll
    for (int r = 0; r < 32; ++r) s += part[r][c];
    s *= inv_scale;
    if (i < B16_RED_QKV) {
        const int tile = i >> 5, f = i & 31, head = tile / 3, which = tile - 3 * head;
        if (head < h && f < dk) db_qkv[which * d + head * dk + f] += s * (which == 0 ? qscale : 1.0f);
    } else if (i < B16_RED_QKV + F16_QP) {
        const int qq = i - B16_RED_QKV;
        if (qq < q) db_add[qq] += s;
    } else {
        const int qq = i - B16_RED_QKV - F16_QP;
        if (qq < q) dq_vec[qq] += s;
    }
}

struct Maps16 { int *nmap_qkv, *kmap_x, *nmap_add, *kmap_ctx; float *nscale_qkv, *nscale_add; };
__device__ __forceinline__ void maps16_entry(int i, int d, int h, int dk, int q, float inv_scale, float qscale, const Maps16& m) {
    int* const nmap_qkv = m.nmap_qkv; int* const kmap_x = m.kmap_x; int* const nmap_add = m.nmap_add; int* const kmap_ctx = m.kmap_ctx;
    float* const nscale_qkv = m.nscale_qkv; float* const nscale_add = m.nscale_add;
    if (i < B16_DQ) {
        const int head = i / 96, rem = i - head * 96, which = rem >> 5, p = rem & 31;
        const int s = p >> 4, t = p & 15, hh = t >> 3, jj = t & 7;
        const int f = 16 * s + 8 * (jj >> 2) + 4 * hh + (jj & 3);
        nmap_qkv[i] = (head < h && f < dk) ? which * d + head * dk + f : -1;
        nscale_qkv[i] = inv_scale * (which == 0 ? qscale : 1.0f);
    }
    if (i < F16_KP) kmap_x[i] = i < d ? i : -1;
    if (i < F16_QP) { nmap_add[i] = i < q ? i : -1; nscale_add[i] = inv_scale; }
    if (i < F16_DP) {
        const int b16 = i >> 4, t = i & 15, hh = t >> 3, jj = t & 7;
        const int fpad = 16 * b16 + 8 * (jj >> 2) + 4 * hh + (jj & 3);
        const int head = fpad >> 5, f = fpad & 31;
        kmap_ctx[i] = (head < h && f < dk) ? head * dk + f : -1;
    }
}

constexpr int MAPS16_BLOCKS = (B16_DQ + 255) / 256;
static_assert(B16_DQ >= F16_KP && B16_DQ >= F16_QP && B16_DQ >= F16_DP, "maps16_entry: one thread per entry of the longest map");
__global__ __launch_bounds__(256) void dout16_maps_kernel(long n_seq, int d, int h, int dk, int q, float fixed_scale, float qscale,
                                                          const unsigned* max_bits, float* sc, const float* dout, _Float16* dout16,
                                                          Maps16 m) {
    const float scale = loss_scale_from_max(*max_bits, fixed_scale);
    const int n_rows_blocks = (int)gridDim.x - MAPS16_BLOCKS;
    if ((int)blockIdx.x >= n_rows_blocks) {
        maps16_entry(((int)blockIdx.x - n_rows_blocks) * 256 + (int)threadIdx.x, d, h, dk, q, 1.0f / scale, qscale, m);
        return;
    }
    dout16_rows(n_seq, d, h, dk, scale, sc, dout, dout16, n_rows_blocks);
}

static size_t up256(size_t x) { return (x + 255) / 256 * 256; }


Fused16BwdLayout fused16_bwd_layout(long M, int n_seq) {
    Fused16BwdLayout L;
    const long Mp = (long)n_seq * (M > (long)n_seq * 32 ? 64 : 32);
    size_t off = 0;
    auto take = [&](size_t bytes) { size_t o = off; off = up256(off + bytes); return o; };
    L.n_wg = 512;
    L.btiles = take((size_t)40 * 32 * F16_KP * 2);
    L.xtiles = take((size_t)DX_SLABS * DX_B_BYTES);
    L.qv16 = take((size_t)F16_QP * 2);
    L.bqkv32 = take((size_t)30 * 32 * 4);
    L.dout16 = take((size_t)n_seq * F16_DP * 2);
    L.dz16 = take((size_t)Mp * F16_QP * 2);
    L.dctx16 = take((size_t)Mp * F16_DP * 2);
    L.dqkv16 = take((size_t)(M + 32) * B16_DQ * 2);
    L.red = take((size_t)2 * L.n_wg * B16_RED * 4);
    L.maps = take((size_t)(B16_DQ * 2 + F16_KP + F16_QP * 2 + F16_DP) * 4);
    L.scale = take(256);
    L.tn_splits_qkv = 40;
    L.tn_splits_add = 192;
    if (const char* e = getenv("NRMS_TN_SPLITS_QKV")) L.tn_splits_qkv = atoi(e);
    if (const char* e = getenv("NRMS_TN_SPLITS_ADD")) L.tn_splits_add = atoi(e);
    const size_t p1 = (size_t)L.tn_splits_qkv * B16_DQ * F16_KP * 4, p2 = (size_t)L.tn_splits_add * F16_QP * F16_DP * 4;
    L.partial = take(up256(p1) + p2);
    L.total = off;
    return L;
}

int launch_tn16(int geom, const _Float16* A, int lda, int N, const _Float16* B, int ldb, int K, int M, const int* m_dev,
                float* partial, int splits, const int* nmap, const int* kmap, const float* nscale, int ldw, float* dW,
                hipStream_t stream, const char* name, float* dbias, const int* blk_list, const int* blk_cnt, int blk_stride) {
    Tn16Args t{};
    t.M = M; t.m_dev = m_dev; t.A = A; t.lda = lda; t.N = N; t.B = B; t.ldb = ldb; t.K = K; t.partial = partial;
    t.blk_list = geom != 0 ? blk_list : nullptr; t.blk_cnt = blk_cnt; t.blk_stride = blk_stride;
    typedef void (*Kern)(Tn16Args);
    const Kern fn = geom == 1 ? (Kern)gemm16_tn_kernel<true, 2, 7, 4, 5> : geom == 2 ? (Kern)gemm16_tn_kernel<true, 4, 5, 2, 5>
                                                                                     : (Kern)gemm16_tn_kernel<false, 4, 5, 2, 5>;
    const int aw = geom == 1 ? Tn16Add::AW : Tn16Qkv::AW, bw = geom == 1 ? Tn16Add::BW : Tn16Qkv::BW;
    t.splits = splits; t.n_blk = cdiv(N, aw); t.k_blk = cdiv(K, bw);
    const size_t lds = 2 * (size_t)(geom == 1 ? Tn16Add::STAGE : Tn16Qkv::STAGE);
    const hipError_t e = hipFuncSetAttribute((const void*)fn, hipFuncAttributeMaxDynamicSharedMemorySize, (int)lds);
    if (e != hipSuccess) { set_error("%s: hipFuncSetAttribute: %s", name, hipGetErrorString(e)); return NRMS_ELAUNCH; }
    {
        TimingScope ts(name, stream);
        hipLaunchKernelGGL(fn, dim3(splits * t.n_blk * t.k_blk), dim3(T16_THREADS), lds, stream, t);
    }
    int rc = check_launch(name);
    if (rc) return rc;
    TimingScope ts("tn_reduce", stream);
    hipLaunchKernelGGL(tn16_reduce_kernel, dim3(cdiv((long)N * K, 256)), dim3(256), 0, stream, partial, splits, N, K, nmap, kmap,
                       nscale, ldw, dW, dbias);
    return check_launch("tn16_reduce");
}

size_t bwd16_fused_lds(bool two) {
    static_assert(F16_WAVES * 2 * F16_QT * 32 + 2 * F16_WAVES * 32 >= 2 * F16_WAVES * 3 * 32, "the attention kernel's staging fits the same size");
    return (size_t)3 * F16_SLOT + (size_t)B16_RED * 4 + (size_t)(F16_WAVES * (two ? 2 : 1) * 2 * F16_QT * 32 + 2 * F16_WAVES * 32) * 4;
}

int launch_bwd16_pool(const Bwd16Args& a, int n_wg, bool two, hipStream_t stream) {
    const size_t lds = bwd16_fused_lds(two);
    const void* fp = two ? (const void*)fused_bwd16_pool_kernel<2> : (const void*)fused_bwd16_pool_kernel<1>;
    const hipError_t e = hipFuncSetAttribute(fp, hipFuncAttributeMaxDynamicSharedMemorySize, (int)lds);
    if (e != hipSuccess) { set_error("fused_bwd16: hipFuncSetAttribute: %s", hipGetErrorString(e)); return NRMS_ELAUNCH; }
    TimingScope ts(two ? "fused64_bwd16_pool" : "fused_bwd16_pool", stream);
    if (two) hipLaunchKernelGGL(fused_bwd16_pool_kernel<2>, dim3(n_wg), dim3(F16_THREADS), lds, stream, a);
    else hipLaunchKernelGGL(fused_bwd16_pool_kernel<1>, dim3(n_wg), dim3(F16_THREADS), lds, stream, a);
    return check_launch("fused_bwd16_pool");
}

int launch_dx16(const Dx16Args& g, bool out16, hipStream_t stream) {
    if ((g.d & 3) != 0 || ((uintptr_t)g.c & 15) != 0) { set_error("gemm16_dx: dx must be 16-byte aligned, d %% 4 == 0"); return NRMS_EINVAL; }
    const size_t lds = (size_t)2 * DX_SLOT;
    const void* fn = out16 ? (const void*)gemm16_dx_kernel<true> : (const void*)gemm16_dx_kernel<false>;
    const hipError_t e = hipFuncSetAttribute(fn, hipFuncAttributeMaxDynamicSharedMemorySize, (int)lds);
    if (e != hipSuccess) { set_error("gemm16_dx: hipFuncSetAttribute: %s", hipGetErrorString(e)); return NRMS_ELAUNCH; }
    TimingScope ts("dx_bwd", stream);
    if (out16) hipLaunchKernelGGL(gemm16_dx_kernel<true>, dim3(cdiv(g.M, DX_BM)), dim3(DX_THREADS), lds, stream, g);
    else hipLaunchKernelGGL(gemm16_dx_kernel<false>, dim3(cdiv(g.M, DX_BM)), dim3(DX_THREADS), lds, stream, g);
    return check_launch("gemm16_dx");
}

int launch_dout16(long n_seq, int d, int h, int dk, float fixed_scale, float* sc, const float* dout, _Float16* dout16, hipStream_t stream) {
    unsigned* max_bits = (unsigned*)(sc + 2);
    if (hipMemsetAsync(max_bits, 0, sizeof(unsigned), stream) != hipSuccess) { set_error("fused_bwd16: memset failed"); return NRMS_ELAUNCH; }
    const long nd = n_seq * d;
    if (!(fixed_scale > 0.f))
        hipLaunchKernelGGL(absmax_kernel, dim3(nd > 512L * 1024 ? 512 : (int)cdiv(nd, 1024)), dim3(256), 0, stream, nd, dout, max_bits);
    hipLaunchKernelGGL(dout16_kernel, dim3(cdiv(n_seq * F16_DP, 256) > 4096 ? 4096 : cdiv(n_seq * F16_DP, 256)),
                       dim3(256), 0, stream, n_seq, d, h, dk, fixed_scale, max_bits, sc, dout, dout16);
    return check_launch("dout16");
}

static int launch_dout16_maps(long n_seq, int d, int h, int dk, int q, float fixed_scale, float qscale, float* sc, const float* dout,
                              _Float16* dout16, const Maps16& m, hipStream_t stream) {
    unsigned* max_bits = (unsigned*)(sc + 2);
    const long nd = n_seq * d;
    if (!(fixed_scale > 0.f))
        hipLaunchKernelGGL(absmax_kernel, dim3(nd > 512L * 1024 ? 512 : (int)cdiv(nd, 1024)), dim3(256), 0, stream, nd, dout, max_bits);
    const int row_blocks = cdiv(n_seq * F16_DP, 256) > 4096 ? 4096 : cdiv(n_seq * F16_DP, 256);
    hipLaunchKernelGGL(dout16_maps_kernel, dim3(row_blocks + MAPS16_BLOCKS), dim3(256), 0, stream, n_seq, d, h, dk, q, fixed_scale,
                       qscale, max_bits, sc, dout, dout16, m);
    return check_launch("dout16");
}

int launch_fused_bwd16(const Fused16Bwd& f, hipStream_t stream) {
    if (f.n_seq <= 0) return NRMS_OK;
    const long M = (long)f.n_seq * f.S;
    const Fused16BwdLayout L = fused16_bwd_layout(M, f.n_seq);
    char* base = (char*)f.workspace;
    const int dk = f.d / f.h;
    const float qscale = 1.0f / sqrtf((float)dk);
    _Float16* btiles = (_Float16*)(base + L.btiles);
    _Float16* xtiles = (_Float16*)(base + L.xtiles);
    _Float16* qv16 = (_Float16*)(base + L.qv16);
    float* bqkv32 = (float*)(base + L.bqkv32);
    _Float16* dout16 = (_Float16*)(base + L.dout16);
    _Float16* dz16 = (_Float16*)(base + L.dz16);
    _Float16* dctx16 = (_Float16*)(base + L.dctx16);
    _Float16* dqkv16 = (_Float16*)(base + L.dqkv16);
    float* red = (float*)(base + L.red);
    int* nmap_qkv = (int*)(base + L.maps);
    float* nscale_qkv = (float*)(nmap_qkv + B16_DQ);
    int* kmap_x = (int*)(nscale_qkv + B16_DQ);
    int* nmap_add = kmap_x + F16_KP;
    float* nscale_add = (float*)(nmap_add + F16_QP);
    int* kmap_ctx = (int*)(nscale_add + F16_QP);
    float* sc = (float*)(base + L.scale);
    if (f.sc_out != nullptr) *f.sc_out = sc;
    float* partial_qkv = (float*)(base + L.partial);
    float* partial_add = (float*)(base + L.partial + up256((size_t)L.tn_splits_qkv * B16_DQ * F16_KP * 4));
    { const int jr = fused_bwd16_join(stream, false); if (jr) return jr; }
    SideSet* ss = side_streams_for(stream);
    const bool side = ss != nullptr;
    hipStream_t s_add = side ? ss->s[0] : stream, s_qkv = side ? ss->s[1] : stream;
    SideJoinGuard join_guard(ss, stream);
    const int Mp = f.n_seq * 32 * (f.S > 32 ? 2 : 1);
    {
        Prep16bArgs p{};
        p.d = f.d; p.h = f.h; p.dk = dk; p.q = f.q; p.w_qkv = f.w_qkv; p.b_qkv = f.b_qkv; p.w_add = f.w_add; p.q_vec = f.q_vec;
        p.btiles = btiles; p.xtiles = xtiles; p.qv16 = qv16; p.bqkv32 = bqkv32;
        p.max_bits = (unsigned*)(sc + 2);
        TimingScope ts("prep16", stream);
        hipLaunchKernelGGL(prep16b_kernel, dim3(2048), dim3(256), 0, stream, p);
        int rc = check_launch("prep16b");
        if (rc) return rc;
        Maps16 mp;
        mp.nmap_qkv = nmap_qkv; mp.nscale_qkv = nscale_qkv; mp.kmap_x = kmap_x; mp.nmap_add = nmap_add; mp.nscale_add = nscale_add;
        mp.kmap_ctx = kmap_ctx;
        rc = launch_dout16_maps((long)f.n_seq, f.d, f.h, dk, f.q, f.loss_scale, qscale, sc, f.dout, dout16, mp, stream);
        if (rc) return rc;
    }
    Bwd16Args a{};
    a.n_seq = f.n_seq; a.S = f.S; a.d = f.d; a.h = f.h; a.dk = dk; a.q = f.q;
    const bool lists = f.order != nullptr && f.S <= 32;
    a.n_groups = cdiv(f.n_seq, F16_WAVES) + (lists ? 2 : 0);
    a.n_cls = lists ? 3 : 2;
    a.x16 = (const _Float16*)f.x16; a.pos = f.pos; a.n_rows = f.n_rows_dev; a.ids = f.ids;
    a.order = lists ? f.order : nullptr; a.order_cnt = lists ? f.order_cnt : nullptr;
    a.btiles = btiles; a.bqkv32 = bqkv32; a.qv16 = qv16;
    a.ctx16 = (const _Float16*)f.ctx16; a.t16 = (const _Float16*)f.t16; a.w = f.w; a.dout16 = dout16;
    a.dz16 = dz16; a.dctx16 = dctx16; a.dqkv16 = dqkv16; a.red = red; a.drop = f.drop;
    a.dbg = 0;
#ifdef NRMS_F16_EXPERIMENTS
    { const char* e = getenv("NRMS_F16_DBG"); a.dbg = e ? atoi(e) : 0; }
#endif
    const int n_wg = a.n_groups < L.n_wg ? a.n_groups : L.n_wg;
    {
        const bool two = f.S > 32;
        const size_t lds = bwd16_fused_lds(two);
        const void* fa = two ? (const void*)fused_bwd16_attn_kernel<2> : (const void*)fused_bwd16_attn_kernel<1>;
        const hipError_t e = hipFuncSetAttribute(fa, hipFuncAttributeMaxDynamicSharedMemorySize, (int)lds);
        if (e != hipSuccess) { set_error("fused_bwd16: hipFuncSetAttribute: %s", hipGetErrorString(e)); return NRMS_ELAUNCH; }
        {
            const int rcp = launch_bwd16_pool(a, n_wg, two, stream);
            if (rcp) return rcp;
        }
        if (side) {
            int rc = side_order(ss, 0, stream, s_add, "fused_bwd16");
            if (rc) return rc;
            rc = launch_tn16(1, dz16, F16_QP, F16_QP, (const _Float16*)f.ctx16, F16_DP, F16_DP, Mp, nullptr, partial_add,
                             L.tn_splits_add, nmap_add, kmap_ctx, nscale_add, f.d, f.dw_add, s_add, "dwadd_bwd");
            if (rc) return rc;
            if (hipEventRecord(ss->ev[2], s_add) != hipSuccess) { set_error("fused_bwd16: hipEventRecord failed"); return NRMS_ELAUNCH; }
        }
        Bwd16Args b = a;
        b.red = red + (long)n_wg * B16_RED;
        {
            TimingScope ts(two ? "fused64_bwd16_attn" : "fused_bwd16_attn", stream);
            if (two) hipLaunchKernelGGL(fused_bwd16_attn_kernel<2>, dim3(n_wg), dim3(F16_THREADS), lds, stream, b);
            else hipLaunchKernelGGL(fused_bwd16_attn_kernel<1>, dim3(n_wg), dim3(F16_THREADS), lds, stream, b);
        }
        int rc = check_launch("fused_bwd16");
        if (rc) return rc;
    }
    int rc = NRMS_OK;
    if (!side) {
        rc = launch_tn16(1, dz16, F16_QP, F16_QP, (const _Float16*)f.ctx16, F16_DP, F16_DP, Mp, nullptr, partial_add,
                         L.tn_splits_add, nmap_add, kmap_ctx, nscale_add, f.d, f.dw_add, stream, "dwadd_bwd");
        if (rc) return rc;
    }
    if (side) {
        rc = side_order(ss, 1, stream, s_qkv, "fused_bwd16");
        if (rc) return rc;
    }
    rc = launch_tn16(0, dqkv16, B16_DQ, B16_DQ, (const _Float16*)f.x16, F16_KP, F16_KP, (int)M, f.n_rows_dev, partial_qkv,
                     L.tn_splits_qkv, nmap_qkv, kmap_x, nscale_qkv, f.d, f.dw_qkv, s_qkv, "dwqkv_bwd");
    if (rc) return rc;
    if (side && hipEventRecord(ss->ev[3], s_qkv) != hipSuccess) { set_error("fused_bwd16: hipEventRecord failed"); return NRMS_ELAUNCH; }
    {
        Dx16Args g{};
        g.M = (int)M; g.m_dev = f.n_rows_dev; g.a16 = dqkv16; g.xtiles = xtiles; g.c = f.dx; g.ldc = f.d; g.d = f.d;
        g.sc = sc; g.lda = B16_DQ; g.n_slabs = DX_SLABS;
        rc = launch_dx16(g, f.dx_fp16, stream);
    }
    if (rc == NRMS_OK) {
        TimingScope ts("red16", stream);
        hipLaunchKernelGGL(red16_kernel, dim3(cdiv(B16_RED, 32)), dim3(1024), 0, stream, red, 2 * n_wg, f.h, dk, f.d, f.q, sc,
                           qscale, f.db_qkv, f.db_add, f.dq_vec);
        rc = check_launch("red16");
    }
    if (side && rc == NRMS_OK) {
        if (f.defer_join) ss->pending = true;
        else if (hipStreamWaitEvent(stream, ss->ev[2], 0) != hipSuccess || hipStreamWaitEvent(stream, ss->ev[3], 0) != hipSuccess) {
            set_error("fused_bwd16: hipStreamWaitEvent failed");
            return NRMS_ELAUNCH;
        } else if ((rc = side_join_user(ss, stream, "fused_bwd16")) != NRMS_OK) return rc;
        join_guard.disarm();
    }
    return rc;
}

int fused_bwd16_join(hipStream_t stream, bool user) {
    SideSet* ss = side_streams_for(stream);
    if (ss == nullptr) return NRMS_OK;
    if (ss->pending) {
        ss->pending = false;
        if (hipStreamWaitEvent(stream, ss->ev[2], 0) != hipSuccess || hipStreamWaitEvent(stream, ss->ev[3], 0) != hipSuccess) {
            set_error("fused_bwd16_join: hipStreamWaitEvent failed");
            return NRMS_ELAUNCH;
        }
    }
    return user ? side_join_user(ss, stream, "fused_bwd16_join") : NRMS_OK;
}

}
```

pytorch_news_recommender_amd/csrc/gemm.h:

```cpp
#pragma once
#include "common.h"
#include "rowdiv.h"

namespace nrms {

constexpr int NT_BM = 128;
constexpr int NT_BK = 16;
constexpr int NT_STAGE_A = NT_BM * NT_BK;

enum { A_PLAIN = 0, A_DZ = 2 };
enum { E_STORE = 0, E_DCTX = 1 };

struct NTArgs {
    int M, N, K;
    int rows_per_tile;
    const float* A; int lda;
    const float* ds;
    const float* qv;
    const float* T;
    const float* W;
    const float* bias;
    float* C; int ldc;
    const float* wrow;
    const float* dout;
    RowDiv seq_of_row;
    Dropout drop;
    const int* a_rows;
    const int* m_dev;
    const int* c_rows;
};

__device__ __forceinline__ int nt_swz(int row) { return (0x1230 >> (((row >> 2) & 3) * 4)) & 3; }

template <int NT, int AMODE>
__device__ __forceinline__ void gemm_nt_mainloop(const NTArgs& a, int row0, int rows_valid, int col0,
                                                 f32x4 (&acc)[2][NT], float* lds) {
    constexpr int STAGE = (NT_BM + 16 * NT) * NT_BK;
    constexpr int B_F4 = NT * 16 * 4;
    constexpr int B_IT = (B_F4 + 255) / 256;
    const int tid = threadIdx.x;
    const int lane = tid & 63, wave = tid >> 6;
    const int r16 = lane & 15, kq = lane >> 4;

    const int chunk = tid & 3;
    const float* arow[2];
    float ascale[2];
    bool a_ok[2];
    int a_lds[2];
#pragma unroll
    for (int i = 0; i < 2; ++i) {
        const int r = (tid >> 2) + 64 * i;
        const long g = (long)row0 + min(r, rows_valid - 1);
        a_ok[i] = r < rows_valid;
        a_lds[i] = (r * 4 + (chunk ^ nt_swz(r))) * 4;
        if (AMODE == A_PLAIN) { arow[i] = a.A + (a.a_rows != nullptr ? (long)a.a_rows[g] : g) * a.lda; ascale[i] = 0.f; }
        else { arow[i] = a.T + g * (long)a.K; ascale[i] = a.ds[g]; }
    }
    const float* brow[B_IT];
    bool b_ok[B_IT];
    int b_lds[B_IT];
#pragma unroll
    for (int i = 0; i < B_IT; ++i) {
        const int idx = tid + 256 * i;
        const int r = idx >> 2;
        const int n = col0 + r;
        b_ok[i] = idx < B_F4 && n < a.N;
        brow[i] = a.W + (long)min(n, a.N - 1) * a.K;
        b_lds[i] = idx < B_F4 ? NT_STAGE_A + (r * 4 + (chunk ^ nt_swz(r))) * 4 : -1;
    }
    const int fsw = kq ^ nt_swz(r16);
    const int a_frag0 = ((32 * wave + r16) * 4 + fsw) * 4;
    const int a_frag1 = ((32 * wave + 16 + r16) * 4 + fsw) * 4;
    const int b_frag = NT_STAGE_A + (r16 * 4 + fsw) * 4;

    f32x4 av[2], bv[B_IT], qv4;
    const int k_last = a.K - 4;
    auto load_stage = [&](int k0) {
        const int k = min(k0 + chunk * 4, k_last);
#pragma unroll
        for (int i = 0; i < 2; ++i) av[i] = *reinterpret_cast<const f32x4*>(arow[i] + k);
        if (AMODE == A_DZ) qv4 = *reinterpret_cast<const f32x4*>(a.qv + k);
#pragma unroll
        for (int i = 0; i < B_IT; ++i) bv[i] = *reinterpret_cast<const f32x4*>(brow[i] + k);
    };
    const f32x4 zero4 = {0.f, 0.f, 0.f, 0.f};
    auto store_stage = [&](int k0, float* st) {
        const bool kok = k0 + chunk * 4 < a.K;
#pragma unroll
        for (int i = 0; i < 2; ++i) {
            f32x4 v = av[i];
            if (AMODE == A_DZ) v = ascale[i] * qv4 * (1.0f - v * v);
            *reinterpret_cast<f32x4*>(st + a_lds[i]) = (a_ok[i] && kok) ? v : zero4;
        }
#pragma unroll
        for (int i = 0; i < B_IT; ++i)
            if (b_lds[i] >= 0) *reinterpret_cast<f32x4*>(st + b_lds[i]) = (b_ok[i] && kok) ? bv[i] : zero4;
    };

    const int n_stage = (a.K + NT_BK - 1) / NT_BK;
    load_stage(0);
    store_stage(0, lds);
    __syncthreads();
    for (int s = 0; s < n_stage; ++s) {
        const float* cur = lds + (s & 1) * STAGE;
        load_stage((s + 1) * NT_BK);
        const f32x4 a0 = *reinterpret_cast<const f32x4*>(cur + a_frag0);
        const f32x4 a1 = *reinterpret_cast<const f32x4*>(cur + a_frag1);
#pragma unroll
        for (int nt = 0; nt < NT; ++nt) {
            const f32x4 b = *reinterpret_cast<const f32x4*>(cur + b_frag + nt * 16 * NT_BK);
#pragma unroll
            for (int e = 0; e < 4; ++e) {
                acc[0][nt] = mfma16(a0[e], b[e], acc[0][nt]);
                acc[1][nt] = mfma16(a1[e], b[e], acc[1][nt]);
            }
        }
        store_stage((s + 1) * NT_BK, lds + ((s + 1) & 1) * STAGE);
        __syncthreads();
    }
}

template <int NT, int EMODE>
__device__ __forceinline__ void nt_epilogue(const NTArgs& g, const f32x4 (&acc)[2][NT], int row0, int rows_valid,
                                            int col0, int wave, int lane, float* wave_lds) {
    constexpr int S = 16 * NT + 8;
    constexpr int F4_ROW = 4 * NT;
    constexpr int LPR = F4_ROW >= 64 ? 64 : F4_ROW;
    constexpr int RPI = 64 / LPR;
    constexpr int REM = F4_ROW - LPR * (RPI == 1 ? 1 : 0) > 0 && F4_ROW > 64 ? F4_ROW - 64 : 0;
    static_assert(8 % RPI == 0, "strip rows must divide into store instructions");
    const int r16 = lane & 15, kq = lane >> 4;
    const int sub = RPI == 1 ? 0 : lane / LPR;
    const int c4a = RPI == 1 ? lane : lane - sub * LPR;
    const int na = col0 + 4 * c4a;
    const bool ok_a = c4a < F4_ROW && sub < RPI && na < g.N;
    f32x4 bias_a = {0.f, 0.f, 0.f, 0.f};
    if (EMODE == E_STORE && g.bias != nullptr && ok_a) bias_a = *reinterpret_cast<const f32x4*>(g.bias + na);

    auto fix = [&](f32x4 v, long gr, int n, const f32x4& bias4) {
        if (EMODE == E_STORE) return v + bias4;
        const long seq = (long)row_div((uint32_t)gr, g.seq_of_row);
        return v + g.wrow[gr] * *reinterpret_cast<const f32x4*>(g.dout + seq * (long)g.N + n);
    };
    const bool dropped = g.drop.thresh != 0u;
    auto rem_pos = [&](int idx, int rbase, int& sr, int& c4, int& rl, int& n) {
        constexpr int REMD = REM > 0 ? REM : 1;
        sr = idx / REMD; c4 = 64 + idx - sr * REMD;
        rl = rbase + 4 * (sr >> 1) + (sr & 1);
        n = col0 + 4 * c4;
        return rl < rows_valid && n < g.N;
    };

#pragma unroll
    for (int mt = 0; mt < 2; ++mt) {
#pragma unroll
        for (int h = 0; h < 2; ++h) {
#pragma unroll
            for (int b = 0; b < 2; ++b)
#pragma unroll
                for (int nt = 0; nt < NT; ++nt) wave_lds[(2 * kq + b) * S + 16 * nt + r16] = acc[mt][nt][2 * h + b];
            __builtin_amdgcn_fence(__ATOMIC_RELEASE, "wavefront");
            __builtin_amdgcn_wave_barrier();
            __builtin_amdgcn_fence(__ATOMIC_ACQUIRE, "wavefront");
            const int rbase = 32 * wave + 16 * mt + 2 * h;
            if (dropped) {
#pragma unroll 1
                for (int it = 0; it < 8 / RPI; ++it) {
                    const int sr = it * RPI + sub;
                    const int rl = rbase + 4 * (sr >> 1) + (sr & 1);
                    if (ok_a && rl < rows_valid) {
                        const long gr = (long)row0 + rl;
                        f32x4* q = reinterpret_cast<f32x4*>(wave_lds + sr * S + 4 * c4a);
                        *q = fix(*q, gr, na, bias_a) *
                             dropout_scale4(g.drop.seed, 1u, (uint64_t)(gr * g.N + na) >> 2, g.drop.thresh, g.drop.inv_keep);
                    }
                }
                if (REM > 0) {
                    for (int idx = lane; idx < 8 * REM; idx += 64) {
                        int sr, c4, rl, n;
                        if (!rem_pos(idx, rbase, sr, c4, rl, n)) continue;
                        const long gr = (long)row0 + rl;
                        f32x4 b4 = {0.f, 0.f, 0.f, 0.f};
                        if (EMODE == E_STORE && g.bias != nullptr) b4 = *reinterpret_cast<const f32x4*>(g.bias + n);
                        f32x4* q = reinterpret_cast<f32x4*>(wave_lds + sr * S + 4 * c4);
                        *q = fix(*q, gr, n, b4) *
                             dropout_scale4(g.drop.seed, 1u, (uint64_t)(gr * g.N + n) >> 2, g.drop.thresh, g.drop.inv_keep);
                    }
                }
                __builtin_amdgcn_fence(__ATOMIC_RELEASE, "wavefront");
                __builtin_amdgcn_wave_barrier();
                __builtin_amdgcn_fence(__ATOMIC_ACQUIRE, "wavefront");
            }
#pragma unroll
            for (int it = 0; it < 8 / RPI; ++it) {
                const int sr = it * RPI + sub;
                const int rl = rbase + 4 * (sr >> 1) + (sr & 1);
                if (ok_a && rl < rows_valid) {
                    const long gr = (long)row0 + rl;
                    f32x4 v = *reinterpret_cast<const f32x4*>(wave_lds + sr * S + 4 * c4a);
                    if (!dropped) v = fix(v, gr, na, bias_a);
                    *reinterpret_cast<f32x4*>(g.C + (g.c_rows != nullptr ? (long)g.c_rows[gr] : gr) * g.ldc + na) = v;
                }
            }
            if (REM > 0) {
                for (int idx = lane; idx < 8 * REM; idx += 64) {
                    int sr, c4, rl, n;
                    if (!rem_pos(idx, rbase, sr, c4, rl, n)) continue;
                    const long gr = (long)row0 + rl;
                    f32x4 v = *reinterpret_cast<const f32x4*>(wave_lds + sr * S + 4 * c4);
                    if (!dropped) {
                        f32x4 b4 = {0.f, 0.f, 0.f, 0.f};
                        if (EMODE == E_STORE && g.bias != nullptr) b4 = *reinterpret_cast<const f32x4*>(g.bias + n);
                        v = fix(v, gr, n, b4);
                    }
                    *reinterpret_cast<f32x4*>(g.C + (g.c_rows != nullptr ? (long)g.c_rows[gr] : gr) * g.ldc + n) = v;
                }
            }
            __builtin_amdgcn_fence(__ATOMIC_RELEASE, "wavefront");
            __builtin_amdgcn_wave_barrier();
            __builtin_amdgcn_fence(__ATOMIC_ACQUIRE, "wavefront");
        }
    }
}

int launch_gemm_nt(int amode, int emode, const NTArgs& a, hipStream_t stream, const char* name);

struct TNArgs {
    int M, N, K;
    int amode;
    const float* A; int lda;
    const float* ds;
    const float* qv;
    const float* T;
    const float* B; int ldb;
    float* dW;
    float* dbias;
    float* partial;
    int splits;
    int rows_per_split;
    HeadPerm perm;
    const int* m_dev;
};
size_t gemm_tn_workspace_floats(int M, int N, int K, int* splits_out);
int launch_gemm_tn(const TNArgs& a, hipStream_t stream, const char* name);

int launch_transpose(const float* in, float* out, int rows, int cols, hipStream_t stream, HeadPerm perm = HeadPerm{0, 0});
int launch_permute_rows(const float* w, const float* b, float* w2, float* b2, int rows, int cols, HeadPerm perm,
                        hipStream_t stream);

int launch_gemm_nt_bf16(int amode, int emode, int npass, const NTArgs& a, void* wplanes, hipStream_t stream,
                        const char* name);
size_t gemm_nt_bf16_wplane_bytes(int N, int K);
int launch_gemm_tn_bf16(int npass, const TNArgs& a, hipStream_t stream, const char* name);

struct AddFwdArgs {
    NTArgs g;
    const float* qv;
    float* T;
    float* wout;
    float* out;
    int S, d;
    const uint8_t* mask;
};
int launch_addattn_fwd_bf16(int npass, const AddFwdArgs& a, void* wplanes, hipStream_t stream);
int launch_colsum_add(const float* partial, int rows, int cols, float* out, hipStream_t stream);

struct Fused16Layout { int KP, DP, QP; size_t wqkv16, wadd16, bqkv32, badd32, qv32, total; };
Fused16Layout fused16_layout(int d, int h, int q);
bool fused16_supported(int S, int d, int h, int q, const char** why);
int launch_prep16(int d, int h, int q, const float* w_qkv, const float* b_qkv, const float* w_add, const float* b_add,
                  const float* q_vec, void* planes, hipStream_t stream);
int launch_gather16(long M, int d, int KP, const int64_t* ids, const int* live, const int* n_live, const float* table,
                    const Dropout& drop, void* x16, hipStream_t stream);
int launch_cast16(long M, int d, int KP, const float* x, void* x16, hipStream_t stream);
struct Fused16Fwd {
    int n_seq, S, d, h, q;
    const void* planes;
    const void* x16;
    const int* pos;
    const int* n_rows;
    const int64_t* ids;
    const int* order;
    const int* order_cnt;
    void* ctx16;
    void* t16;
    float* w;
    float* out;
    Dropout drop;
};
int launch_fused_fwd16(const Fused16Fwd& f, hipStream_t stream);
bool fused16v1_supported(int S, int d, int h, int q, const char** why);
size_t fused16v1_planes_bytes(int d, int h, int q);
int launch_prep16v1(int d, int h, int q, const float* w_qkv, const float* b_qkv, const float* w_o, const float* b_o,
                    const float* w_add, const float* b_add, const float* q_vec, void* planes, hipStream_t stream);
int launch_fused_fwd16v1(const Fused16Fwd& f, int h, void* attn16, hipStream_t stream);
size_t title_order_cnt_ints(int n_seq);
int launch_title_order(int n_seq, int S, const int64_t* ids, int* order, int* cnt, hipStream_t stream, int n_classes = 2);

struct Fused16BwdLayout { int n_wg, tn_splits_qkv, tn_splits_add; size_t btiles, xtiles, qv16, bqkv32, dout16, dz16, dctx16, dqkv16, red, maps, scale, partial, total; };
Fused16BwdLayout fused16_bwd_layout(long M, int n_seq);
struct Fused16Bwd {
    int n_seq, S, d, h, q;
    void* workspace;
    const float* w_qkv; const float* b_qkv; const float* w_add; const float* q_vec;
    const void* x16;
    const int* pos;
    const int* n_rows_dev;
    const int64_t* ids;
    const int* order; const int* order_cnt;
    const void* ctx16; const void* t16; const float* w;
    const float* dout;
    float loss_scale;
    Dropout drop;
    float* dw_qkv; float* db_qkv; float* dw_add; float* db_add; float* dq_vec;
    float* dx;
    bool dx_fp16;
    const float** sc_out;
    bool defer_join;
    const float* w_o; const void* attn16; float* dw_o; float* db_o;
};
int launch_fused_bwd16(const Fused16Bwd& f, hipStream_t stream);
size_t fused16v1_bwd_bytes(long M, int n_seq, int h);
int launch_fused_bwd16v1(const Fused16Bwd& f, hipStream_t stream);
int fused_bwd16_join(hipStream_t stream, bool user = true);

bool user64_supported(int S, int d, int h, int q, const char** why);
size_t user64_qkv_bytes(int n_seq, int h);
size_t user64_fwd_planes_bytes(int h);
size_t user64_bwd_planes_bytes(int h);
size_t user64_dq_partial_floats(int n_seq);
int launch_user64_fwd(int n_seq, int S, int d, int h, int q, const float* x, const float* w_qkv, const float* b_qkv,
                      const float* w_add, const float* b_add, const float* q_vec, void* planes, float* ctx, float* t, float* w,
                      void* qkv, float* out, bool train, hipStream_t stream);
int launch_user64_bwd(int n_seq, int S, int d, int h, int q, const float* w_add, const float* q_vec, void* planes, const float* dout,
                      const float* t, const float* w, const void* qkv, float* ds, float* dq_partial, float* dq_vec, float* dqkv,
                      hipStream_t stream);

int launch_sanitize_ids(long n, const void* src, bool src_is_int32, int64_t* dst, int vocab, int* n_bad, hipStream_t stream);
int launch_title_dedup(long n, int L, const int64_t* ids, int* table, long table_size, int* inverse, int* rep_rows,
                       int* n_unique, hipStream_t stream);
int launch_gather_dropout(long M, int d, const int64_t* ids, const float* table, const Dropout& drop, float* x,
                          hipStream_t stream);
int launch_gather_dropout_compact(long M, int d, const int64_t* ids, const int* live, const int* n_live,
                                  const float* table, const Dropout& drop, float* x, hipStream_t stream);
int launch_fill_pad_rows(long n_seq, int S, int n, const int64_t* ids, const float* row, float* out, bool skip_all_pad,
                         hipStream_t stream);
size_t compact_scratch_ints(long M);
int launch_compact_live_rows(long M, const int64_t* ids, int* live, int* pos, int* n_live, int* scratch,
                             hipStream_t stream);
size_t scatter_grouped_scratch_ints(long M, int V);
int launch_scatter_grouped(long M, int V, int d, const int64_t* ids, const int* live, const int* n_live, const void* dx,
                           const Dropout& drop, float* dtable, int* scratch, hipStream_t stream, bool dx_fp16 = false, int ldx = 0,
                           const float* sc = nullptr, bool prepared = false);
struct TableAdam {
    float *p, *m, *v;
    AdamConsts c;
    float gscale;
    int* n_bad;
};
int launch_scatter_grouped_adam(long M, int V, int d, const int64_t* ids, const int* live, const int* n_live, const void* dx,
                                const Dropout& drop, float* dtable, int* scratch, hipStream_t stream, bool dx_fp16, int ldx,
                                const float* sc, bool prepared, const TableAdam& a);
int launch_scatter_prepare(long M, int V, const int64_t* ids, const int* live, const int* n_live, int* scratch, hipStream_t stream);
int launch_scatter_dense_rows(long M, int d, const int64_t* ids, const int* live, const int* n_live, const float* dx,
                              const Dropout& drop, float* dtable, hipStream_t stream);
int launch_scatter_dropout_compact(long M, int d, const int64_t* ids, const int* live, const int* n_live, const float* dx,
                                   const Dropout& drop, float* dtable, hipStream_t stream);

}
```

pytorch_news_recommender_amd/csrc/gemm.hip:

```cpp
#include "gemm.h"

namespace nrms {

template <int NT, int AMODE, int EMODE>
__global__ __launch_bounds__(256, 2) void gemm_nt_kernel(NTArgs a) {
    __shared__ __attribute__((aligned(16))) float lds[2 * (NT_BM + 16 * NT) * NT_BK];

    const int n_ct = (a.N + NT * 16 - 1) / (NT * 16);
    const int xcd = blockIdx.x & 7, j = blockIdx.x >> 3;
    const int rt = (j / n_ct) * 8 + xcd;
    const int row0 = rt * a.rows_per_tile;
    const int M = a.m_dev != nullptr ? *a.m_dev : a.M;
    if (row0 >= M) return;
    const int rows_valid = min(a.rows_per_tile, M - row0);
    const int col0 = (j % n_ct) * (NT * 16);

    f32x4 acc[2][NT];
#pragma unroll
    for (int mt = 0; mt < 2; ++mt)
#pragma unroll
        for (int nt = 0; nt < NT; ++nt) acc[mt][nt] = f32x4{0.f, 0.f, 0.f, 0.f};

    gemm_nt_mainloop<NT, AMODE>(a, row0, rows_valid, col0, acc, lds);

    static_assert(4 * 8 * (16 * NT + 8) <= 2 * (NT_BM + 16 * NT) * NT_BK, "epilogue strips must fit the stage buffers");
    const int lane = threadIdx.x & 63, wave = __builtin_amdgcn_readfirstlane(threadIdx.x >> 6);
    nt_epilogue<NT, EMODE>(a, acc, row0, rows_valid, col0, wave, lane, lds + wave * 8 * (16 * NT + 8));
}

template <int NT, int AMODE, int EMODE>
static int launch_nt_inst(const NTArgs& a, hipStream_t stream, const char* name) {
    dim3 grid(cdiv(cdiv(a.M, a.rows_per_tile), 8) * 8 * cdiv(a.N, NT * 16));
    TimingScope ts(name, stream);
    hipLaunchKernelGGL((gemm_nt_kernel<NT, AMODE, EMODE>), grid, dim3(256), 0, stream, a);
    return check_launch(name);
}

static int pick_nt(int N) {
    const int cand[5] = {19, 13, 8, 4, 2};
    int best = 19;
    long best_pad = -1;
    for (int i = 0; i < 5; ++i) {
        if (cand[i] < 8 && N > 128) continue;
        const int w = cand[i] * 16;
        const long pad = (long)cdiv(N, w) * w;
        if (best_pad < 0 || pad < best_pad) { best_pad = pad; best = cand[i]; }
    }
    return best;
}

template <int AMODE, int EMODE>
static int launch_nt_mode(const NTArgs& a, hipStream_t stream, const char* name) {
    switch (pick_nt(a.N)) {
        case 19: return launch_nt_inst<19, AMODE, EMODE>(a, stream, name);
        case 13: return launch_nt_inst<13, AMODE, EMODE>(a, stream, name);
        case 8: return launch_nt_inst<8, AMODE, EMODE>(a, stream, name);
        case 4: return launch_nt_inst<4, AMODE, EMODE>(a, stream, name);
        default: return launch_nt_inst<2, AMODE, EMODE>(a, stream, name);
    }
}

int launch_gemm_nt(int amode, int emode, const NTArgs& a, hipStream_t stream, const char* name) {
    if (a.M <= 0) return NRMS_OK;
    if ((a.K & 3) != 0) { set_error("%s: K=%d must be a multiple of 4", name, a.K); return NRMS_EINVAL; }
    if (amode == A_PLAIN && emode == E_STORE) return launch_nt_mode<A_PLAIN, E_STORE>(a, stream, name);
    if (amode == A_DZ && emode == E_DCTX) return launch_nt_mode<A_DZ, E_DCTX>(a, stream, name);
    if (amode == A_DZ && emode == E_STORE) return launch_nt_mode<A_DZ, E_STORE>(a, stream, name);
    set_error("%s: unsupported gemm_nt mode %d/%d", name, amode, emode);
    return NRMS_EINVAL;
}

constexpr int TN_WN = 4, TN_WK = 2;
constexpr int TN_NTN = 5;
constexpr int TN_NTK = 5;
constexpr int TN_MC = 32;
constexpr int TN_AW = TN_WN * TN_NTN * 16;
constexpr int TN_BW = TN_WK * TN_NTK * 16;
constexpr int TN_SA = TN_AW + 4;
constexpr int TN_SB = TN_BW + 4;
constexpr int TN_STAGE = TN_MC * (TN_SA + TN_SB);
constexpr int TN_THREADS = 64 * TN_WN * TN_WK;
constexpr int TN_A_IT = (TN_MC * TN_AW / 4) / TN_THREADS;
constexpr int TN_B_IT = (TN_MC * TN_BW / 4 + TN_THREADS - 1) / TN_THREADS;

struct TNGeom {
    int n_tiles, k_tiles;
    int n_wg, k_wg;
    int n_tpw, k_tpw;
};

static TNGeom tn_geom(int N, int K) {
    TNGeom g;
    g.n_tiles = cdiv(N, 16);
    g.k_tiles = cdiv(K + 1, 16);
    g.n_wg = cdiv(g.n_tiles, TN_WN * TN_NTN);
    g.k_wg = cdiv(g.k_tiles, TN_WK * TN_NTK);
    const int n0 = g.n_wg;
    for (int n = n0; n <= 2 * n0 + 1 && n <= g.n_tiles; ++n)
        if (n * g.k_wg <= 32 && 32 % (n * g.k_wg) == 0) { g.n_wg = n; break; }
    g.n_tpw = cdiv(g.n_tiles, g.n_wg);
    g.k_tpw = cdiv(g.k_tiles, g.k_wg);
    return g;
}

template <int AMODE, int NTN, int NTK>
__global__ __launch_bounds__(TN_THREADS, 2) void gemm_tn_kernel(TNArgs a, TNGeom g) {
    extern __shared__ __attribute__((aligned(16))) float lds[];

    const int tid = threadIdx.x, lane = tid & 63;
    const int wave = __builtin_amdgcn_readfirstlane(tid >> 6);
// ... 255 lines not shown
```

pytorch_news_recommender_amd/csrc/gemm_bf16.hip:

```cpp
#include <stdlib.h>

#include <atomic>

#include "gemm.h"

namespace nrms {

typedef __bf16 bf16x8 __attribute__((ext_vector_type(8)));

constexpr int BF_BM = 256;
constexpr int BF_BK = 32;
constexpr int BF_THREADS = 512;
constexpr int BF_ROWB = 64;

struct Split8 { bf16x8 hi, lo; };

__device__ __forceinline__ Split8 split8(const f32x4& u, const f32x4& v) {
    Split8 s;
#pragma unroll
    for (int i = 0; i < 4; ++i) {
        const __bf16 h0 = (__bf16)u[i], h1 = (__bf16)v[i];
        s.hi[i] = h0; s.hi[4 + i] = h1;
        s.lo[i] = (__bf16)(u[i] - (float)h0);
        s.lo[4 + i] = (__bf16)(v[i] - (float)h1);
// ... 128 lines not shown
    };

    const int n_stage = (g.K + BF_BK - 1) / BF_BK;
    load_b(a.whi, 0);
    store_b(smem);
    if (NPASS == 3) { load_b(a.wlo, 0); store_b(smem + B_PLANE); }
    load_a(0);
    __syncthreads();
    constexpr int HALF = (NT + 1) / 2;
#pragma unroll 2
    for (int s = 0; s < n_stage; ++s) {
        const char* cur = smem + (s & 1) * STAGE;
        char* nxt = smem + ((s + 1) & 1) * STAGE;
        const bool more = s + 1 < n_stage;
        const int kn = (s + 1) * BF_BK;
        Split8 a0, a1;
        split_a(s * BF_BK, a0, a1);
        if (more) {
            load_b(a.whi, kn);
            load_a(kn);
        }
        bf16x8 bh0, bl0, bh1, bl1;
        read_b(cur, 0, bh0, bl0);
#pragma unroll
        for (int nt = 0; nt < HALF; nt += 2) {
            if (nt + 1 < NT) read_b(cur, nt + 1, bh1, bl1);
            mma(nt, a0, a1, bh0, bl0);
            if (nt + 1 < HALF) {
                if (nt + 2 < NT) read_b(cur, nt + 2, bh0, bl0);
                mma(nt + 1, a0, a1, bh1, bl1);
            }
        }
        if (more) {
            store_b(nxt);
            if (NPASS == 3) load_b(a.wlo, kn);
        }
        if (HALF % 2 == 0) {
#pragma unroll
            for (int nt = HALF; nt < NT; nt += 2) {
                if (nt + 1 < NT) read_b(cur, nt + 1, bh1, bl1);
                mma(nt, a0, a1, bh0, bl0);
                if (nt + 1 < NT) {
                    if (nt + 2 < NT) read_b(cur, nt + 2, bh0, bl0);
                    mma(nt + 1, a0, a1, bh1, bl1);
                }
            }
        } else {
#pragma unroll
            for (int nt = HALF; nt < NT; nt += 2) {
                if (nt + 1 < NT) read_b(cur, nt + 1, bh0, bl0);
                mma(nt, a0, a1, bh1, bl1);
                if (nt + 1 < NT) {
                    if (nt + 2 < NT) read_b(cur, nt + 2, bh1, bl1);
                    mma(nt + 1, a0, a1, bh0, bl0);
                }
            }
        }
        if (more && NPASS == 3) store_b(nxt + B_PLANE);
        __syncthreads();
    }
}

template <int NT, int AMODE, int EMODE, int NPASS>
__global__ __launch_bounds__(BF_THREADS, 2) void gemm_nt_bf16_kernel(BFArgs a) {
    extern __shared__ __attribute__((aligned(16))) char smem[];
    const NTArgs& g = a.g;
    const int n_ct = (g.N + NT * 16 - 1) / (NT * 16);
    const int xcd = blockIdx.x & 7, jb = blockIdx.x >> 3;
    const int rt = (jb / n_ct) * 8 + xcd;
    const int row0 = rt * g.rows_per_tile;
    const int M = g.m_dev != nullptr ? *g.m_dev : g.M;
    if (row0 >= M) return;
    const int rows_valid = min(g.rows_per_tile, M - row0);
    const int col0 = (jb % n_ct) * (NT * 16);

    f32x4 acc[2][NT];
#pragma unroll
    for (int mt = 0; mt < 2; ++mt)
#pragma unroll
        for (int nt = 0; nt < NT; ++nt) acc[mt][nt] = f32x4{0.f, 0.f, 0.f, 0.f};
    bf16_nt_mainloop<NT, AMODE, NPASS>(a, row0, rows_valid, col0, acc, smem);

    const int lane = threadIdx.x & 63, wave = __builtin_amdgcn_readfirstlane(threadIdx.x >> 6);
    nt_epilogue<NT, EMODE>(g, acc, row0, rows_valid, col0, wave, lane,
                           reinterpret_cast<float*>(smem) + wave * 8 * (16 * NT + 8));
}

template <int NT, int AMODE, int EMODE, int NPASS>
static int launch_bf_inst(const BFArgs& a, hipStream_t stream, const char* name) {
    constexpr int P = NPASS == 3 ? 2 : 1;
    constexpr size_t stage_bytes = 2 * (size_t)P * (NT * 16) * BF_ROWB;
    constexpr size_t strip_bytes = (size_t)8 * 8 * (16 * NT + 8) * sizeof(float);
    constexpr size_t lds_bytes = stage_bytes > strip_bytes ? stage_bytes : strip_bytes;
    const void* fn = (const void*)gemm_nt_bf16_kernel<NT, AMODE, EMODE, NPASS>;
    const hipError_t e = hipFuncSetAttribute(fn, hipFuncAttributeMaxDynamicSharedMemorySize, (int)lds_bytes);
    if (e != hipSuccess) { set_error("%s: hipFuncSetAttribute: %s", name, hipGetErrorString(e)); return NRMS_ELAUNCH; }
    dim3 grid(cdiv(cdiv(a.g.M, a.g.rows_per_tile), 8) * 8 * cdiv(a.g.N, NT * 16));
    TimingScope ts(name, stream);
    hipLaunchKernelGGL((gemm_nt_bf16_kernel<NT, AMODE, EMODE, NPASS>), grid, dim3(BF_THREADS), lds_bytes, stream, a);
    return check_launch(name);
}

static int cu_count() {
    static std::atomic<int> cached{0};
    int n = cached.load(std::memory_order_relaxed);
    if (n > 0) return n;
    int dev = 0;
    hipDeviceProp_t prop;
    if (hipGetDevice(&dev) != hipSuccess || hipGetDeviceProperties(&prop, dev) != hipSuccess || prop.multiProcessorCount <= 0) {
        (void)hipGetLastError();
        return 256;
    }
    cached.store(prop.multiProcessorCount, std::memory_order_relaxed);
    return prop.multiProcessorCount;
}

template <int AMODE, int EMODE, int NPASS>
static int launch_bf_mode(const BFArgs& a, hipStream_t stream, const char* name) {
    const int N = a.g.N;
    const int cand[6] = {19, 15, 13, 10, 8, 4};
    int nt = 19;
    long best = -1;
    for (int i = 0; i < 6; ++i) {
        if (cand[i] < 8 && N > 128) continue;
        const long pad = (long)cdiv(N, cand[i] * 16) * cand[i] * 16;
        if (best < 0 || pad < best) { best = pad; nt = cand[i]; }
    }
    const long row_tiles = cdiv(a.g.M, a.g.rows_per_tile);
    const int n_cu = cu_count();
    if (2 * row_tiles * cdiv(N, nt * 16) <= n_cu && getenv("NRMS_NT_WIDE_TILES") == nullptr) {
        const int blocks0 = cdiv(N, nt * 16);
        long best2 = -1;
        for (int i = 0; i < 6; ++i) {
            if (cand[i] < 8) continue;
            const int blocks = cdiv(N, cand[i] * 16);
            if (blocks <= blocks0 || row_tiles * blocks > n_cu) continue;
            const long pad = (long)blocks * cand[i] * 16;
            if (best2 < 0 || pad < best2) { best2 = pad; nt = cand[i]; }
        }
    }
    switch (nt) {
        case 19: return launch_bf_inst<19, AMODE, EMODE, NPASS>(a, stream, name);
        case 15: return launch_bf_inst<15, AMODE, EMODE, NPASS>(a, stream, name);
        case 13: return launch_bf_inst<13, AMODE, EMODE, NPASS>(a, stream, name);
        case 10: return launch_bf_inst<10, AMODE, EMODE, NPASS>(a, stream, name);
        case 8: return launch_bf_inst<8, AMODE, EMODE, NPASS>(a, stream, name);
        default: return launch_bf_inst<4, AMODE, EMODE, NPASS>(a, stream, name);
    }
}

int launch_gemm_nt_bf16(int amode, int emode, int npass, const NTArgs& g_in, void* wplanes, hipStream_t stream,
                        const char* name) {
    if (g_in.M <= 0) return NRMS_OK;
    if ((g_in.K & 3) != 0) { set_error("%s: K=%d must be a multiple of 4", name, g_in.K); return NRMS_EINVAL; }
    BFArgs a;
    a.g = g_in;
    a.g.rows_per_tile = BF_BM;
    a.Kp = cdiv(g_in.K, BF_BK) * BF_BK;
    a.Np = cdiv(g_in.N, 16) * 16;
    a.whi = (const __bf16*)wplanes;
    a.wlo = a.whi + (long)a.Np * a.Kp;
    int rc = launch_split_planes(g_in.W, g_in.N, a.Np, g_in.K, a.Kp, wplanes, (void*)a.wlo, stream);
    if (rc) return rc;
    if (npass == 3) {
        if (amode == A_PLAIN && emode == E_STORE) return launch_bf_mode<A_PLAIN, E_STORE, 3>(a, stream, name);
        if (amode == A_DZ && emode == E_DCTX) return launch_bf_mode<A_DZ, E_DCTX, 3>(a, stream, name);
        if (amode == A_DZ && emode == E_STORE) return launch_bf_mode<A_DZ, E_STORE, 3>(a, stream, name);
    } else {
// ... 431 lines not shown
```

pytorch_news_recommender_amd/csrc/pool.hip:

```cpp
#include "gemm.h"

namespace nrms {

template <int NT>
__global__ __launch_bounds__(256, 2) void addattn_fwd_kernel(AddFwdArgs a) {
    __shared__ __attribute__((aligned(16))) float lds[2 * (NT_BM + 16 * NT) * NT_BK];
    __shared__ float sc[NT_BM];

    const NTArgs& g = a.g;
    const int row0 = blockIdx.x * g.rows_per_tile;
    const int rows_valid = min(g.rows_per_tile, g.M - row0);
    f32x4 acc[2][NT];
#pragma unroll
    for (int mt = 0; mt < 2; ++mt)
#pragma unroll
        for (int nt = 0; nt < NT; ++nt) acc[mt][nt] = f32x4{0.f, 0.f, 0.f, 0.f};
    gemm_nt_mainloop<NT, A_PLAIN>(g, row0, rows_valid, 0, acc, lds);

    const int tid = threadIdx.x, lane = tid & 63;
    const int wave = __builtin_amdgcn_readfirstlane(tid >> 6);
    const int r16 = lane & 15, kq = lane >> 4;
    float bcol[NT], qcol[NT];
#pragma unroll
    for (int nt = 0; nt < NT; ++nt) {
// ... 153 lines not shown
__global__ __launch_bounds__(1024) void colsum_add_kernel(const float* partial, int rows, int cols, float* out) {
    __shared__ float red[64][17];
    const int cl = threadIdx.x & 15, rg = threadIdx.x >> 4;
    const int c = blockIdx.x * 16 + cl;
    float s0 = 0.f, s1 = 0.f, s2 = 0.f, s3 = 0.f;
    if (c < cols) {
        int r = rg;
        for (; r + 192 < rows; r += 256) {
            s0 += partial[(long)r * cols + c];
            s1 += partial[(long)(r + 64) * cols + c];
            s2 += partial[(long)(r + 128) * cols + c];
            s3 += partial[(long)(r + 192) * cols + c];
        }
        for (; r < rows; r += 64) s0 += partial[(long)r * cols + c];
    }
    red[rg][cl] = (s0 + s1) + (s2 + s3);
    __syncthreads();
    if (rg == 0 && c < cols) {
        float t = 0.f;
#pragma unroll
        for (int i = 0; i < 64; ++i) t += red[i][cl];
        out[c] += t;
    }
}

int addattn_bwd_rows_waves(int n_seq) {
    int blocks = cdiv(n_seq, ROWS_WPB);
    if (blocks > 1024) blocks = 1024;
    if (blocks < 1) blocks = 1;
    return blocks * ROWS_WPB;
}

int launch_addattn_bwd_rows(int n_seq, int S, int d, int q, const float* ctx, const float* dout, const float* w,
                            const float* T, float* ds, float* dq_partial, float* dq, const uint8_t* mask,
                            hipStream_t stream) {
    if (n_seq <= 0) return NRMS_OK;
    const int waves = addattn_bwd_rows_waves(n_seq);
    {
        TimingScope ts("addattn_bwd_rows", stream);
        hipLaunchKernelGGL(addattn_bwd_rows_kernel, dim3(waves / ROWS_WPB), dim3(64 * ROWS_WPB), 0, stream, n_seq, S,
                           d, q, ctx, dout, w, T, ds, dq_partial, mask);
        int rc = check_launch("addattn_bwd_rows");
        if (rc) return rc;
    }
    return launch_colsum_add(dq_partial, waves, q, dq, stream);
}

int launch_colsum_add(const float* partial, int rows, int cols, float* out, hipStream_t stream) {
    TimingScope ts("colsum_add", stream);
    hipLaunchKernelGGL(colsum_add_kernel, dim3(cdiv(cols, 16)), dim3(1024), 0, stream, partial, rows, cols, out);
    return check_launch("colsum_add");
}

__global__ void click_fwd_kernel(int B, int C, int d, const float* cand, const float* user, const uint8_t* mask,
                                 float* scores) {
    const int lane = threadIdx.x & 63;
    const long u = (long)blockIdx.x * (blockDim.x >> 6) + (threadIdx.x >> 6);
    if (u >= (long)B * C) return;
    const long b = u / C;
    const float* cv = cand + u * d;
    const float* uv = user + b * d;
    float p = 0.f;
    for (int k = lane; k < d; k += 64) p += cv[k] * uv[k];
    p = wave_sum(p);
    if (lane == 0) scores[u] = (mask != nullptr && mask[u] == 0) ? -1e9f : p;
}

__global__ void click_indexed_kernel(int B, int C, int d, const float* vec, long n_vec, const int* index, const float* user,
                                     const uint8_t* mask, float* scores) {
    const int lane = threadIdx.x & 63;
    const long u = (long)blockIdx.x * (blockDim.x >> 6) + (threadIdx.x >> 6);
    if (u >= (long)B * C) return;
    const long b = u / C;
    const long r = index[u];
    const bool ok = r >= 0 && r < n_vec;
    const float* cv = vec + (ok ? r : 0) * d;
    const float* uv = user + b * d;
    float p = 0.f;
    for (int k = lane; k < d; k += 64) p += cv[k] * uv[k];
    p = wave_sum(p);
    if (lane == 0) scores[u] = (mask != nullptr && mask[u] == 0) ? -1e9f : (ok ? p : __builtin_nanf(""));
}

__global__ void click_bwd_kernel(int B, int C, int d, const float* cand, const float* user, const uint8_t* mask,
                                 const float* dscores, float* dcand, float* duser) {
    const int b = blockIdx.x;
    for (int k = threadIdx.x; k < d; k += blockDim.x) {
        const float uv = user[(long)b * d + k];
        float du = 0.f;
        for (int c = 0; c < C; ++c) {
            const long u = (long)b * C + c;
            const float g = (mask != nullptr && mask[u] == 0) ? 0.f : dscores[u];
            dcand[u * d + k] = g * uv;
            du += g * cand[u * d + k];
        }
        duser[(long)b * d + k] = du;
    }
}

__global__ void ce_loss_kernel(int B, int C, const float* scores, float* loss_sum, float* dscores, float gscale) {
    __shared__ float red[256];
    float local = 0.f;
    for (int b = threadIdx.x; b < B; b += blockDim.x) {
        const float* s = scores + (long)b * C;
        float mx = -3.0e38f;
        for (int c = 0; c < C; ++c) mx = fmaxf(mx, s[c]);
        double sum = 0.0;
        for (int c0 = 0; c0 < C; c0 += 16) {
            const int c1 = c0 + 16 < C ? c0 + 16 : C;
            float run = 0.f;
            for (int c = c0; c < c1; ++c) run += expf(s[c] - mx);
            sum += (double)run;
        }
        local += (float)(((double)mx - (double)s[0]) + log(sum));
        if (dscores != nullptr) {
            const float inv = (float)(1.0 / sum);
            for (int c = 0; c < C; ++c) {
                const float e = expf(s[c] - mx);
                const float p = (c == 0) ? __builtin_fmaf(e, inv, -1.0f) : e * inv;
                dscores[(long)b * C + c] = p * gscale;
            }
        }
    }
    red[threadIdx.x] = local;
    __syncthreads();
    for (int o = 128; o > 0; o >>= 1) {
        if ((int)threadIdx.x < o) red[threadIdx.x] += red[threadIdx.x + o];
        __syncthreads();
    }
    if (threadIdx.x == 0) loss_sum[0] += red[0];
}

template <bool GUARD>
__global__ void adam_kernel(size_t n4, size_t n, float* p, const float* g, float* m, float* v, float step_size,
                            float b1, float b2, float omb1, float omb2, float inv_sqrt_bc2, float eps, float gscale, int* n_bad) {
    const size_t stride = (size_t)gridDim.x * blockDim.x;
    int bad = 0;
    for (size_t i = (size_t)blockIdx.x * blockDim.x + threadIdx.x; i < n4; i += stride) {
        f32x4 pv = reinterpret_cast<f32x4*>(p)[i];
        const f32x4 gv = reinterpret_cast<const f32x4*>(g)[i] * gscale;
        f32x4 mv = reinterpret_cast<f32x4*>(m)[i];
        f32x4 vv = reinterpret_cast<f32x4*>(v)[i];
#pragma unroll
        for (int e = 0; e < 4; ++e) {
            if (GUARD && (__float_as_uint(gv[e]) & 0x7F800000u) == 0x7F800000u) { ++bad; continue; }
            float pe = pv[e], me = mv[e], ve = vv[e];
            adam_update(pe, me, ve, gv[e], step_size, b1, b2, omb1, omb2, inv_sqrt_bc2, eps);
            pv[e] = pe; mv[e] = me; vv[e] = ve;
        }
        reinterpret_cast<f32x4*>(p)[i] = pv;
        reinterpret_cast<f32x4*>(m)[i] = mv;
        reinterpret_cast<f32x4*>(v)[i] = vv;
    }
    const size_t t = n4 * 4 + (size_t)blockIdx.x * blockDim.x + threadIdx.x;
    if (t < n) {
        const float gv = g[t] * gscale;
        if (GUARD && (__float_as_uint(gv) & 0x7F800000u) == 0x7F800000u) {
            ++bad;
        } else {
            float pe = p[t], me = m[t], ve = v[t];
            adam_update(pe, me, ve, gv, step_size, b1, b2, omb1, omb2, inv_sqrt_bc2, eps);
            p[t] = pe; m[t] = me; v[t] = ve;
        }
    }
    if (GUARD) {
#pragma unroll
        for (int o = 32; o > 0; o >>= 1) bad += __shfl_xor(bad, o, 64);
        if (bad != 0 && (threadIdx.x & 63) == 0) atomicAdd(n_bad, bad);
    }
}

__global__ void grad_guard_kernel(size_t n, float* g, int* n_bad) {
    const size_t stride = (size_t)gridDim.x * blockDim.x;
    int bad = 0;
    const size_t n4 = ((reinterpret_cast<uintptr_t>(g) & 15) == 0) ? n / 4 : 0;
    for (size_t i = (size_t)blockIdx.x * blockDim.x + threadIdx.x; i < n4; i += stride) {
        f32x4 gv = reinterpret_cast<f32x4*>(g)[i];
        int b = 0;
#pragma unroll
// ... 17 lines not shown
    k.x = r[0] >= thresh; k.y = r[1] >= thresh; k.z = r[2] >= thresh; k.w = r[3] >= thresh;
    reinterpret_cast<uchar4*>(keep)[i] = k;
}

__global__ void keep_mask16_kernel(uint64_t seed, uint32_t site, long groups8, uint32_t thresh16, uint8_t* keep) {
    const long i = (long)blockIdx.x * blockDim.x + threadIdx.x;
    if (i >= groups8) return;
    uint32_t r[4];
    philox4x32_7(seed, (uint64_t)i, site, r);
#pragma unroll
    for (int w = 0; w < 4; ++w) {
        keep[8 * i + 2 * w] = (r[w] & 0xFFFFu) >= thresh16;
        keep[8 * i + 2 * w + 1] = (r[w] >> 16) >= thresh16;
    }
}

__global__ __launch_bounds__(256) void impression_auc_kernel(int n_imp, int max_c, const float* scores,
                                                             const uint8_t* labels, const int32_t* lens, double* auc) {
    const int lane = threadIdx.x & 63;
    const int imp = blockIdx.x * 4 + __builtin_amdgcn_readfirstlane(threadIdx.x >> 6);
    if (imp >= n_imp) return;
    const int n = min(lens[imp], max_c);
    const float* s = scores + (long)imp * max_c;
    const uint8_t* y = labels + (long)imp * max_c;
    unsigned long long twice = 0;
    unsigned npos = 0;
    for (int i = lane; i < n; i += 64) {
        if (y[i] == 0) continue;
        ++npos;
        const float si = s[i];
        for (int j = 0; j < n; ++j) {
            if (y[j] != 0) continue;
            const float sj = s[j];
            twice += si > sj ? 2u : (si == sj ? 1u : 0u);
        }
    }
#pragma unroll
    for (int o = 32; o > 0; o >>= 1) {
        twice += __shfl_xor(twice, o, 64);
        npos += __shfl_xor(npos, o, 64);
    }
    if (lane == 0) {
        const unsigned nneg = (unsigned)n - npos;
        auc[imp] = (npos == 0 || nneg == 0) ? __longlong_as_double(0x7FF8000000000000LL)
                                             : 0.5 * (double)twice / ((double)npos * (double)nneg);
    }
}

}

using namespace nrms;

extern "C" int nrms_impression_auc(int32_t n_imp, int32_t max_c, const float* scores, const uint8_t* labels,
                                   const int32_t* lens, double* auc, void* stream) {
    NRMS_REQUIRE(n_imp >= 0 && max_c > 0 && scores && labels && lens && auc, "impression_auc: bad arguments");
    if (n_imp == 0) return NRMS_OK;
    hipStream_t s = (hipStream_t)stream;
    TimingScope ts("impression_auc", s);
    hipLaunchKernelGGL(impression_auc_kernel, dim3(cdiv(n_imp, 4)), dim3(256), 0, s, n_imp, max_c, scores, labels, lens, auc);
    return check_launch("impression_auc");
}

extern "C" int nrms_click_score_fwd(int32_t B, int32_t C, int32_t d, const float* cand, const float* user,
                                    const uint8_t* mask, float* scores, void* stream) {
    NRMS_REQUIRE(B >= 0 && C > 0 && d > 0 && cand && user && scores, "click_score_fwd: bad arguments");
    if (B == 0) return NRMS_OK;
    hipStream_t s = (hipStream_t)stream;
    TimingScope ts("click_fwd", s);
    hipLaunchKernelGGL(click_fwd_kernel, dim3(cdiv((long)B * C, 4)), dim3(256), 0, s, B, C, d, cand, user, mask, scores);
    return check_launch("click_fwd");
}

extern "C" int nrms_click_score_indexed(int32_t B, int32_t C, int32_t d, const float* news_vec, int64_t n_vec, const int32_t* index,
                                        const float* user, const uint8_t* mask, float* scores, void* stream) {
    NRMS_REQUIRE(B >= 0 && C > 0 && d > 0 && n_vec > 0 && news_vec && index && user && scores, "click_score_indexed: bad arguments");
    if (B == 0) return NRMS_OK;
    hipStream_t s = (hipStream_t)stream;
    TimingScope ts("click_fwd", s);
    hipLaunchKernelGGL(click_indexed_kernel, dim3(cdiv((long)B * C, 4)), dim3(256), 0, s, B, C, d, news_vec, (long)n_vec, index,
                       user, mask, scores);
    return check_launch("click_indexed");
}

extern "C" int nrms_click_score_bwd(int32_t B, int32_t C, int32_t d, const float* cand, const float* user,
                                    const uint8_t* mask, const float* dscores, float* dcand, float* duser,
                                    void* stream) {
    NRMS_REQUIRE(B >= 0 && C > 0 && d > 0 && cand && user && dscores && dcand && duser, "click_score_bwd: bad arguments");
    if (B == 0) return NRMS_OK;
    hipStream_t s = (hipStream_t)stream;
    TimingScope ts("click_bwd", s);
    hipLaunchKernelGGL(click_bwd_kernel, dim3(B), dim3(128), 0, s, B, C, d, cand, user, mask, dscores, dcand, duser);
    return check_launch("click_bwd");
}

extern "C" int nrms_ce_loss_fwd_bwd(int32_t B, int32_t C, const float* scores, float* loss_sum, float* dscores,
                                    float grad_scale, void* stream) {
    NRMS_REQUIRE(B >= 0 && C > 0 && scores && loss_sum, "ce_loss: bad arguments");
    if (B == 0) return NRMS_OK;
    hipStream_t s = (hipStream_t)stream;
    TimingScope ts("ce_loss", s);
    hipLaunchKernelGGL(ce_loss_kernel, dim3(1), dim3(256), 0, s, B, C, scores, loss_sum, dscores, grad_scale);
    return check_launch("ce_loss");
}

namespace nrms {
AdamConsts adam_consts(double lr, double beta1, double beta2, double eps, int32_t step) {
    const double bc1 = 1.0 - pow(beta1, (double)step);
    const double bc2 = 1.0 - pow(beta2, (double)step);
    AdamConsts c;
    c.step_size = (float)(lr / bc1);
    c.b1 = (float)beta1; c.b2 = (float)beta2; c.omb1 = (float)(1.0 - beta1); c.omb2 = (float)(1.0 - beta2);
    c.inv_sqrt_bc2 = (float)(1.0 / sqrt(bc2));
    c.eps = (float)eps;
    return c;
}
}

static int adam_step(size_t n, float* param, const float* grad, float* exp_avg, float* exp_avg_sq, double lr, double beta1,
                     double beta2, double eps, int32_t step, float grad_scale, int32_t* n_nonfinite, void* stream,
                     const char* timer = "adam") {
    NRMS_REQUIRE(param && grad && exp_avg && exp_avg_sq && step >= 1, "adam_step: bad arguments");
    NRMS_REQUIRE((((uintptr_t)param | (uintptr_t)grad | (uintptr_t)exp_avg | (uintptr_t)exp_avg_sq) & 15) == 0,
                 "adam_step: buffers must be 16-byte aligned");
    if (n == 0) return NRMS_OK;
    const AdamConsts c = adam_consts(lr, beta1, beta2, eps, step);
    hipStream_t s = (hipStream_t)stream;
    const size_t n4 = n / 4;
    int blocks = (int)((n4 + 255) / 256);
    if (blocks > 256 * 8) blocks = 256 * 8;
    if (blocks < 1) blocks = 1;
    TimingScope ts(timer, s);
    if (n_nonfinite != nullptr)
        hipLaunchKernelGGL(adam_kernel<true>, dim3(blocks), dim3(256), 0, s, n4, n, param, grad, exp_avg, exp_avg_sq, c.step_size,
                           c.b1, c.b2, c.omb1, c.omb2, c.inv_sqrt_bc2, c.eps, grad_scale, (int*)n_nonfinite);
    else
        hipLaunchKernelGGL(adam_kernel<false>, dim3(blocks), dim3(256), 0, s, n4, n, param, grad, exp_avg, exp_avg_sq, c.step_size,
                           c.b1, c.b2, c.omb1, c.omb2, c.inv_sqrt_bc2, c.eps, grad_scale, (int*)nullptr);
    return check_launch("adam");
}

extern "C" int nrms_adam_step_rest(size_t n, float* param, const float* grad, float* exp_avg, float* exp_avg_sq, double lr,
                                   double beta1, double beta2, double eps, int32_t step, float grad_scale, int32_t* n_nonfinite,
                                   void* stream) {
    return adam_step(n, param, grad, exp_avg, exp_avg_sq, lr, beta1, beta2, eps, step, grad_scale, n_nonfinite, stream, "rest_adam");
}

extern "C" int nrms_adam_step(size_t n, float* param, const float* grad, float* exp_avg, float* exp_avg_sq, double lr,
                              double beta1, double beta2, double eps, int32_t step, float grad_scale, void* stream) {
    return adam_step(n, param, grad, exp_avg, exp_avg_sq, lr, beta1, beta2, eps, step, grad_scale, nullptr, stream);
}

extern "C" int nrms_adam_step_guarded(size_t n, float* param, const float* grad, float* exp_avg, float* exp_avg_sq, double lr,
                                      double beta1, double beta2, double eps, int32_t step, float grad_scale,
                                      int32_t* n_nonfinite, void* stream) {
    NRMS_REQUIRE(n_nonfinite != nullptr, "adam_step_guarded: null counter");
    return adam_step(n, param, grad, exp_avg, exp_avg_sq, lr, beta1, beta2, eps, step, grad_scale, n_nonfinite, stream);
}

extern "C" int nrms_grad_guard(size_t n, float* grad, int32_t* n_nonfinite, void* stream) {
    NRMS_REQUIRE(n == 0 || (grad && n_nonfinite), "grad_guard: null argument");
    if (n == 0) return NRMS_OK;
    hipStream_t s = (hipStream_t)stream;
    size_t blocks = (n / 4 + 255) / 256;
    if (blocks > 2048) blocks = 2048;
    if (blocks < 1) blocks = 1;
    TimingScope ts("grad_guard", s);
    hipLaunchKernelGGL(grad_guard_kernel, dim3((int)blocks), dim3(256), 0, s, n, grad, (int*)n_nonfinite);
    return check_launch("grad_guard");
}

extern "C" int nrms_dropout_keep_mask(uint64_t seed, int32_t site, int64_t n_rows, int32_t d, float p_drop,
                                      uint8_t* keep, void* stream) {
    NRMS_REQUIRE(keep && n_rows >= 0 && d > 0 && (d & 3) == 0 && site >= 0, "dropout_keep_mask: bad arguments");
    const long groups = (long)n_rows * d / 4;
    if (groups == 0) return NRMS_OK;
// ... 12 lines not shown
```

pytorch_news_recommender_amd/engine.py:

```python
from __future__ import annotations

import ctypes as C
import math
import os
from dataclasses import dataclass

import torch

from . import _lib
from .synth import ENCODERS


@dataclass(frozen=True)
class ModelDims:
    n_words: int
    word_embed_size: int
    num_attention_heads: int
    query_vector_dim: int
    news_heads: int = 0
    output_proj: bool = False
    style: str = "v0"

    def heads(self, enc):
        return self.news_heads if (enc == "news_encoder" and self.news_heads) else self.num_attention_heads
# ... 19 lines not shown
        out += [(n + ".weight", enc, r) for n, r in zip(qkv, ("wq", "wk", "wv"))]
        out += [(n + ".bias", enc, r) for n, r in zip(qkv, ("bq", "bk", "bv"))]
        if output_proj:
            out += [(wo + ".weight", enc, "wo"), (wo + ".bias", enc, "bo")]
        out += [(enc + ".additive_attention.linear.weight", enc, "wa"),
                (enc + ".additive_attention.linear.bias", enc, "ba"), (qv, enc, "qv")]
    return out


def nrms_entries(dims: ModelDims):
    V, d, q = dims.n_words, dims.word_embed_size, dims.query_vector_dim
    if d % 4 or q % 4:
        raise ValueError("word_embed_size and query_vector_dim must be multiples of 4")
    shapes = {"table": (V, d), "wq": (d, d), "wk": (d, d), "wv": (d, d), "bq": (d,), "bk": (d,), "bv": (d,),
              "wo": (d, d), "bo": (d,), "wa": (q, d), "ba": (q,), "qv": (q,)}
    return [(name, shapes[role], enc, role) for name, enc, role in role_names(dims.style, dims.output_proj)]


class FlatLayout:

    def __init__(self, dims, entries=None):
        self.dims = dims
        self.entries, self.blocks, widths = {}, {}, {}
        off = 0
        for name, shape, enc, role in (nrms_entries(dims) if entries is None else entries):
            n = 1
            for x in shape:
                n *= x
            self.entries[name] = (off, tuple(shape), n)
            if enc is not None:
                self.blocks.setdefault(enc, {})[role] = off
                if role == "wq":
                    widths[enc] = shape[0]
            off += n
        self.total = off
        self.names = list(self.entries)
        for enc, w in widths.items():
            b = self.blocks[enc]
            assert b["wk"] == b["wq"] + w * w and b["wv"] == b["wq"] + 2 * w * w
            assert b["bk"] == b["bq"] + w and b["bv"] == b["bq"] + 2 * w
        self.table = self.blocks["news_encoder"]["table"]
        assert self.table == 0, "the embedding table must be the first entry"

    def view(self, flat: torch.Tensor, name: str) -> torch.Tensor:
        off, shp, n = self.entries[name]
        return flat[off:off + n].view(shp)


def _stream():
    return C.c_void_p(torch.cuda.current_stream().cuda_stream)


def impression_metrics(lib, device, scores, labels, lens, ks=(5, 10), ranks=False):
    k_a, k_b = (int(k) for k in ks)
    n, cmax = scores.shape
    f64 = dict(dtype=torch.float64, device=device)
    out = dict(auc=torch.empty(n, **f64), mrr=torch.empty(n, **f64))
    nd_a, nd_b = torch.empty(n, **f64), torch.empty(n, **f64)
    rk = torch.empty(n, cmax, dtype=torch.int32, device=device) if ranks else None
    scores, labels, lens = scores.contiguous(), labels.contiguous(), lens.contiguous()
    rc = lib.nrms_impression_metrics(n, cmax, _lib.ptr(scores), _lib.ptr(labels), _lib.ptr(lens), k_a, k_b,
                                     _lib.ptr(out["auc"]), _lib.ptr(out["mrr"]), _lib.ptr(nd_a), _lib.ptr(nd_b),
                                     _lib.ptr(rk), _stream())
    _lib.check(rc, "nrms_impression_metrics")
    out["ndcg@%d" % k_a], out["ndcg@%d" % k_b] = nd_a, nd_b
    if ranks:
        out["ranks"] = rk
    return out


class NRMSEngine:

    def __init__(self, dims, device, precision="fp32", layout=None):
        self.lib = _lib.load()
        self.dims = dims
        self.set_precision(precision)
        self.layout = FlatLayout(dims) if layout is None else layout
        self.device = torch.device(device)
        if self.device.type != "cuda":
            raise _lib.NrmsError("the NRMS HIP engine needs a GPU device (got %s); there is no CPU path" % device)
        self._bufs = {}
        self._saved = None
        self._fuse_table_adam = os.environ.get("NRMS_NO_FUSED_TABLE_ADAM", "0") in ("", "0")
        self.fp16_user_encoder = False
        self.fp16_backward = True
        self.loss_scale = 0.0
        self.fp16_wide_heads = False
        self.fp16_inference = False
        self.fused_user_encoder = True
        self.fp16_wide_heads_backward = True
        self._gen = 0
        self._bad_ids = torch.zeros(1, dtype=torch.int32, device=self.device)
        self._bad_host = torch.zeros(1, dtype=torch.int32).pin_memory()
        self._bad_event = None
        self._news_cache = None
        self._grad_bad = torch.zeros(1, dtype=torch.int32, device=self.device)
        self._grad_bad_host = torch.zeros(1, dtype=torch.int32).pin_memory()
        self._grad_bad_event = None
        self.loss_scale_backoff = 0
        self.grad_overflow_steps = 0
        self._clean_polls = 0

    FP16_LIMITS = dict(seq_len=64, d_model=316, d_k=32, n_heads=10, q_dim=224)

    def _fp16_ok(self, enc, seq_len, mask_mode, training):
        d, L = self.dims, self.FP16_LIMITS
        h = d.heads(enc)
        if enc == "user_encoder" and not self.fp16_user_encoder:
            return False
        if not training and not self.fp16_inference:
            return False
        if d.word_embed_size % h:
            return False
        if d.output_proj:
            dk = d.word_embed_size // h
            return (enc == "news_encoder" and self.fp16_wide_heads and self.pad_row_zero and not mask_mode
                    and seq_len <= 32 and d.word_embed_size <= L["d_model"] and d.word_embed_size % 10 == 0
                    and d.word_embed_size // 10 <= 32 and 32 < dk <= 50 and 3 * h + 1 <= 19 and h * max(dk - 48, 0) <= 16
                    and d.query_vector_dim <= L["q_dim"] and (not training or self.fp16_wide_heads_backward))
        return (seq_len <= L["seq_len"] and d.word_embed_size <= L["d_model"] and h <= L["n_heads"]
                and d.word_embed_size // h <= L["d_k"] and d.query_vector_dim <= L["q_dim"]
                and not d.output_proj and not mask_mode and (not training or self.fp16_backward))

    def set_precision(self, precision):
        if precision not in _lib.PRECISIONS:
            raise ValueError("precision must be one of %s" % sorted(_lib.PRECISIONS))
        self.precision = precision
        self.pad_row_zero = False

    def _buf(self, key, numel, dtype=torch.float32):
        t = self._bufs.get(key)
        if t is None or t.numel() < numel or t.dtype != dtype:
            t = torch.empty(max(int(numel), 1), dtype=dtype, device=self.device)
            self._bufs[key] = t
        return t

    def _desc(self, enc, n_seq, seq_len, p_embed=0.0, p_ctx=0.0, seed=0, mask_mode=0, training=False):
        d = self.dims
        prec = self.precision
        if prec == "fp16" and not self._fp16_ok(enc, seq_len, mask_mode, training):
            prec = "bf16x3"
        flags = _lib.NRMS_FLAG_PAD_ROW_ZERO if (self.pad_row_zero and enc == "news_encoder") else 0
        h = d.heads(enc)
        if (enc == "user_encoder" and self.fused_user_encoder and prec == "bf16x3" and not d.output_proj and not mask_mode
                and 32 < seq_len <= 64 and d.word_embed_size <= 300 and d.word_embed_size % h == 0
                and (d.word_embed_size // h) <= 32 and (d.word_embed_size // h) % 2 == 0 and h <= 10 and d.query_vector_dim <= 224):
            flags |= _lib.NRMS_FLAG_FUSED_SEQ64
        return _lib.EncoderDesc(n_seq=n_seq, seq_len=seq_len, d_model=d.word_embed_size, n_heads=h,
                                q_dim=d.query_vector_dim, vocab=d.n_words if enc == "news_encoder" else 0,
                                p_drop_embed=float(p_embed), p_drop_ctx=float(p_ctx),
                                precision=_lib.PRECISIONS[prec], use_output_proj=int(d.output_proj),
                                mask_mode=int(mask_mode),
                                flags=flags,
                                seed=int(seed), loss_scale=float(self.loss_scale), p_drop_attn=0.0)

    def _ptrs(self, cls, flat, enc):
        b = self.layout.blocks[enc]
        base = flat.data_ptr()
        p = lambda role: (base + 4 * b[role]) if role in b else None
        return cls(table=p("table"), w_qkv=p("wq"), b_qkv=p("bq"), w_o=p("wo"), b_o=p("bo"), w_add=p("wa"),
                   b_add=p("ba"), q_vec=p("qv"))

    def _weights(self, flat, enc):
        return self._ptrs(_lib.EncoderWeights, flat, enc)

    def _grads(self, gflat, enc):
# ... 89 lines not shown
            mask = mask.contiguous()
        w = self._weights(flat, "news_encoder")
        step = N if save else min(N, chunk_titles)
        for s0 in range(0, N, max(step, 1)):
            n = min(step, N - s0)
            desc = self._desc("news_encoder", n, L, p_embed, p_ctx, seed, mask_mode if mask is not None else 0, training=save)
            acts = self._acts(tag, n * L, save, gather=True, desc=desc)
            mp = None if mask is None else C.c_void_p(mask[s0:].data_ptr())
            rc = self.lib.nrms_encoder_fwd(C.byref(desc), C.byref(w), C.c_void_p(ids[s0:].data_ptr()), None, mp,
                                           C.byref(acts), C.c_void_p(out[s0:].data_ptr()), _stream())
            _lib.check(rc, "nrms_encoder_fwd(news)")
        return out

    def encode_users(self, flat, news_vectors, out=None, save=False, tag=None, mask=None, mask_mode=0):
        B, H, d = news_vectors.shape
        if tag is None:
            tag = "user" if save else "user_eval"
        if out is None:
            out = torch.empty(B, d, dtype=torch.float32, device=self.device)
        w = self._weights(flat, "user_encoder")
        desc = self._desc("user_encoder", B, H, mask_mode=mask_mode if mask is not None else 0, training=save)
        acts = self._acts(tag, B * H, save, desc=desc)
        rc = self.lib.nrms_encoder_fwd(C.byref(desc), C.byref(w), None, C.c_void_p(news_vectors.data_ptr()),
                                       _lib.ptr(None if mask is None else mask.contiguous()), C.byref(acts),
                                       C.c_void_p(out.data_ptr()), _stream())
        _lib.check(rc, "nrms_encoder_fwd(user)")
        return out

    def click_scores(self, cand_vec, user_vec, cand_mask=None, out=None):
        B, Cn, d = cand_vec.shape
        if out is None:
            out = torch.empty(B, Cn, dtype=torch.float32, device=self.device)
        rc = self.lib.nrms_click_score_fwd(B, Cn, d, _lib.ptr(cand_vec), _lib.ptr(user_vec), _lib.ptr(cand_mask),
                                           _lib.ptr(out), _stream())
        _lib.check(rc, "nrms_click_score_fwd")
        return out

    def forward(self, flat, hist_ids, cand_ids, cand_mask, training, p_drop=0.0, seed=0, user_mask=None,
                user_mask_mode=0):
        B, H, L = hist_ids.shape
        Cn = cand_ids.shape[1]
        d = self.dims.word_embed_size
        N = B * (H + Cn)
        sfx = "" if training else "_eval"
        self.poll_ids()
        ids = self._buf("ids" + sfx, N * L, torch.int64)[:N * L].view(N, L)
        self.sanitize_ids(hist_ids.reshape(B * H, L).contiguous(), ids[:B * H])
        self.sanitize_ids(cand_ids.reshape(B * Cn, L).contiguous(), ids[B * H:])
        nv = self._buf("news_vec" + sfx, N * d)[:N * d].view(N, d)
        p = float(p_drop)
        p_embed = 0.0 if self.dims.style == "v1" else p
        self.encode_titles(flat, ids, out=nv, p_embed=p_embed, p_ctx=p, seed=seed, save=training, tag="news" + sfx,
                           trusted_ids=True)
        hist = nv[:B * H].view(B, H, d)
        cand = nv[B * H:].view(B, Cn, d)
        user = self._buf("user_vec" + sfx, B * d)[:B * d].view(B, d)
        self.encode_users(flat, hist, out=user, save=training, tag="user" + sfx, mask=user_mask, mask_mode=user_mask_mode)
        if cand_mask is not None:
            cand_mask = cand_mask.contiguous()
        scores = torch.empty(B, Cn, dtype=torch.float32, device=self.device)
        self.click_scores(cand, user, cand_mask, out=scores)
        if training:
            self._gen += 1
            self._saved = dict(B=B, H=H, C=Cn, L=L, ids=ids, nv=nv, user=user, mask=cand_mask, p=p, p_embed=p_embed,
                               seed=seed, user_mask=user_mask, user_mask_mode=user_mask_mode if user_mask is not None else 0,
                               gen=self._gen)
        return scores

    def ce_loss(self, scores, grad_scale=None, want_grad=True):
        B, Cn = scores.shape
        loss_sum = torch.zeros(1, dtype=torch.float32, device=self.device)
        dscores = torch.empty_like(scores) if want_grad else None
        gs = (1.0 / B) if grad_scale is None else grad_scale
        rc = self.lib.nrms_ce_loss_fwd_bwd(B, Cn, _lib.ptr(scores), _lib.ptr(loss_sum), _lib.ptr(dscores),
                                           C.c_float(gs), _stream())
        _lib.check(rc, "nrms_ce_loss_fwd_bwd")
        return loss_sum, dscores

    def _bwd_workspace(self, *descs):
        nbytes = max(self.lib.nrms_encoder_bwd_workspace_bytes(C.byref(d)) for d in descs)
        return self._buf("bwd_ws", (nbytes + 3) // 4)

    def encode_users_backward(self, flat, gflat, news_vectors, dout, dx=None, tag="user", mask=None, mask_mode=0,
                              defer_join=False):
        B, H, d = news_vectors.shape
        if dx is None:
            dx = torch.empty(B * H, d, dtype=torch.float32, device=self.device)
        desc = self._desc("user_encoder", B, H, mask_mode=mask_mode if mask is not None else 0, training=True)
        if defer_join and desc.precision != _lib.NRMS_PRECISION_FP16:
            desc.flags |= _lib.NRMS_FLAG_DEFER_USER_JOIN
            nbytes = self.lib.nrms_encoder_bwd_workspace_bytes(C.byref(desc))
            ws = self._buf("bwd_ws_user", (nbytes + 3) // 4)
        else:
            ws = self._bwd_workspace(desc)
        w, g = self._weights(flat, "user_encoder"), self._grads(gflat, "user_encoder")
        acts = self._acts(tag, B * H, True, desc=desc)
        rc = self.lib.nrms_encoder_bwd(C.byref(desc), C.byref(w), None, _lib.ptr(news_vectors),
                                       _lib.ptr(None if mask is None else mask.contiguous()), C.byref(acts),
                                       _lib.ptr(dout.contiguous()), C.byref(g), _lib.ptr(dx), _lib.ptr(ws),
                                       C.c_size_t(ws.numel() * 4), _stream())
        _lib.check(rc, "nrms_encoder_bwd(user)")
        return dx[:B * H].view(B, H, d)

    def join_backward(self):
        _lib.check(self.lib.nrms_encoder_join(_stream()), "nrms_encoder_join")

    POOLED_VEC = ("nv", "d_news_vec")

    def _head_buffers(self, sv, width):
        B, H, Cn = sv["B"], sv["H"], sv["C"]
        N = B * (H + Cn)
        key, dkey = self.POOLED_VEC
        dvec = self._buf(dkey, N * width)[:N * width].view(N, width)
        duser = self._buf("d_user_vec", B * width)[:B * width].view(B, width)
        return sv[key][B * H:], sv["user"], dvec, duser

    def _head_backward(self, dscores, gen, width):
        sv = self._saved
        if sv is None:
            raise _lib.NrmsError("backward() without a training forward()")
        if gen is not None and gen != sv["gen"]:
            raise _lib.NrmsError("backward() for training forward #%d, but the saved activations belong to forward #%d: "
                                 "a later training forward replaced them (one forward/backward pair at a time)" % (gen, sv["gen"]))
        B, H, Cn = sv["B"], sv["H"], sv["C"]
        cand, user, dvec, duser = self._head_buffers(sv, width)
        if dscores is None:
            if getattr(self, "_pooled_gen", None) != sv["gen"]:
                raise _lib.NrmsError("backward(dscores=None) needs the gradients of pooled_ce_loss(), and none was computed for "
                                     "training forward #%d" % sv["gen"])
        else:
            rc = self.lib.nrms_click_score_bwd(B, Cn, width, _lib.ptr(cand), _lib.ptr(user), _lib.ptr(sv["mask"]),
                                               _lib.ptr(dscores.contiguous()), C.c_void_p(dvec[B * H:].data_ptr()), _lib.ptr(duser),
                                               _stream())
            _lib.check(rc, "nrms_click_score_bwd")
        return sv, dvec, duser

    def pooled_ce_loss(self, cand_ids, reject=None, col_bias=None, grad_scale=None, want_grad=True):
        sv = self._saved
        if sv is None:
            raise _lib.NrmsError("pooled_ce_loss() without a training forward()")
        B, Cn = sv["B"], sv["C"]
        key, _ = self.POOLED_VEC
        width = sv[key].shape[1]
        cand, user, dvec, duser = self._head_buffers(sv, width)
        dev = self.device
        ids = torch.as_tensor(cand_ids).to(dev, torch.int64).contiguous()
        if ids.numel() != B * Cn:
            raise _lib.NrmsError("pooled_ce_loss: cand_ids must be [%d, %d] (got %s)" % (B, Cn, tuple(ids.shape)))
        R = 0
        if reject is not None:
            reject = torch.as_tensor(reject).to(dev, torch.int64).contiguous()
            if reject.dim() != 2 or reject.shape[0] != B:
                raise _lib.NrmsError("pooled_ce_loss: reject must be [%d, R] (got %s)" % (B, tuple(reject.shape)))
            R = reject.shape[1]
            if R == 0:
                reject = None
        if col_bias is not None:
            col_bias = torch.as_tensor(col_bias).to(dev, torch.float32).contiguous()
            if col_bias.numel() != B * Cn:
                raise _lib.NrmsError("pooled_ce_loss: col_bias must be [%d, %d] (got %s)" % (B, Cn, tuple(col_bias.shape)))
        nbytes = self.lib.nrms_pooled_ce_workspace_bytes(B, Cn, width, R)
        if nbytes == 0:
            raise _lib.NrmsError("pooled_ce_loss: arguments rejected (B=%d, C=%d, d=%d, R=%d; B <= 4096, C <= 64, B*C <= 32768, "
                                 "d <= 1024, R <= 256)" % (B, Cn, width, R))
        ws = self._buf("pooled_ce_ws", (nbytes + 3) // 4)
        loss_sum = torch.zeros(1, dtype=torch.float32, device=dev)
        self.pooled_pairs = torch.zeros(1, dtype=torch.int64, device=dev)
        gs = (1.0 / B) if grad_scale is None else grad_scale
        H = sv["H"]
        rc = self.lib.nrms_pooled_ce_fwd_bwd(B, Cn, width, R, _lib.ptr(cand), _lib.ptr(user), _lib.ptr(ids), _lib.ptr(sv["mask"]),
                                             _lib.ptr(reject), _lib.ptr(col_bias), C.c_float(gs), _lib.ptr(loss_sum),
                                             C.c_void_p(dvec[B * H:].data_ptr()) if want_grad else None,
                                             _lib.ptr(duser) if want_grad else None, _lib.ptr(self.pooled_pairs), _lib.ptr(ws),
                                             C.c_size_t(ws.numel() * 4), _stream())
        _lib.check(rc, "nrms_pooled_ce_fwd_bwd")
        if want_grad:
            self._pooled_gen = sv["gen"]
        return loss_sum

    single_table_scatter = True

    def __init_subclass__(cls, **kw):
        super().__init_subclass__(**kw)
        if "single_table_scatter" not in cls.__dict__:
            cls.single_table_scatter = False

    def fuses_table_adam(self):
        sv = self._saved
        if (sv is None or not type(self).single_table_scatter or type(self).backward is not NRMSEngine.backward
                or not self._fuse_table_adam or os.environ.get("NRMS_ATOMIC_SCATTER") is not None):
            return False
        return (self.pad_row_zero or self.precision != "fp16"
                or not self._fp16_ok("news_encoder", sv["L"], 0, True))

    def backward(self, flat, gflat, dscores=None, table_grad_ready=None, gen=None, table_adam=None):
        d = self.dims.word_embed_size
        sv, dnv, duser = self._head_backward(dscores, gen, d)
        B, H, Cn, L = sv["B"], sv["H"], sv["C"], sv["L"]
        N = B * (H + Cn)
        self.poll_grad_overflow()
        self.loss_scale = float(getattr(self, "loss_scale_override", None) or -float(self.loss_scale_backoff))
        nv = sv["nv"]
        hist = nv[:B * H]
        desc_u = self._desc("user_encoder", B, H, mask_mode=sv["user_mask_mode"], training=True)
        desc_n = self._desc("news_encoder", N, L, sv["p_embed"], sv["p"], sv["seed"], training=True)
        ws = self._bwd_workspace(desc_u, desc_n)
        defer_user = desc_n.precision == _lib.NRMS_PRECISION_FP16 and not self.dims.output_proj
        self.encode_users_backward(flat, gflat, hist.view(B, H, d), duser, dx=dnv, tag="user", mask=sv["user_mask"],
                                   mask_mode=sv["user_mask_mode"], defer_join=defer_user)
        wn, gn = self._weights(flat, "news_encoder"), self._grads(gflat, "news_encoder")
        acts_n = self._acts("news", N * L, True, gather=True, desc=desc_n)
        if desc_n.precision == _lib.NRMS_PRECISION_FP16:
            desc_n.flags |= _lib.NRMS_FLAG_FWD_SCRATCH_KEPT
        if table_grad_ready is not None:
            desc_n.flags |= _lib.NRMS_FLAG_DEFER_WQKV
        ta = None
        if table_adam is not None:
            if (table_grad_ready is not None or type(self).backward is not NRMSEngine.backward
                    or (desc_n.precision == _lib.NRMS_PRECISION_FP16 and not desc_n.flags & _lib.NRMS_FLAG_PAD_ROW_ZERO)):
                raise _lib.NrmsError("backward(table_adam=...) needs fuses_table_adam() and no table_grad_ready")
            lo, _, n_table = self.layout.entries[self.layout.names[0]]
            if lo != 0 or wn.table != flat.data_ptr():
                raise _lib.NrmsError("backward(table_adam=...): the word-embedding table must open the flat buffer")
            guard = table_adam.get("guard")
            guard = self.precision == "fp16" if guard is None else guard
            betas = table_adam.get("betas", (0.9, 0.999))
            ta = _lib.TableAdam(param=flat.data_ptr(), exp_avg=table_adam["m"].data_ptr(), exp_avg_sq=table_adam["v"].data_ptr(),
                                lr=float(table_adam["lr"]), beta1=float(betas[0]), beta2=float(betas[1]),
                                eps=float(table_adam.get("eps", 1e-8)), step=int(table_adam["step"]),
                                grad_scale=float(table_adam.get("grad_scale", 1.0)),
                                n_nonfinite=self._grad_bad.data_ptr() if guard else None)
            desc_n.flags |= _lib.NRMS_FLAG_TABLE_ADAM
        rc_join = 0
        try:
            rc = self.lib.nrms_encoder_bwd_adam(C.byref(desc_n), C.byref(wn), _lib.ptr(sv["ids"]), None, None, C.byref(acts_n),
                                                _lib.ptr(dnv), C.byref(gn), None, _lib.ptr(ws),
                                                C.c_size_t(ws.numel() * 4), None if ta is None else C.byref(ta), _stream())
            _lib.check(rc, "nrms_encoder_bwd(news)")
            if table_grad_ready is not None:
                table_grad_ready()
                rc = self.lib.nrms_encoder_bwd_wqkv(C.byref(desc_n), _lib.ptr(sv["ids"]), None, C.byref(acts_n), C.byref(gn),
                                                    _lib.ptr(ws), C.c_size_t(ws.numel() * 4), _stream())
                _lib.check(rc, "nrms_encoder_bwd_wqkv(news)")
        finally:
            if defer_user:
                rc_join = self.lib.nrms_encoder_join(_stream())
        _lib.check(rc_join, "nrms_encoder_join")

    def adam_step(self, flat, gflat, exp_avg, exp_avg_sq, step, lr=1e-3, betas=(0.9, 0.999), eps=1e-8,
                  grad_scale=1.0, guard=None, rest=False):
        if guard is None:
            guard = self.precision == "fp16"
        if rest:
            rc = self.lib.nrms_adam_step_rest(C.c_size_t(flat.numel()), _lib.ptr(flat), _lib.ptr(gflat), _lib.ptr(exp_avg),
                                              _lib.ptr(exp_avg_sq), C.c_double(lr), C.c_double(betas[0]), C.c_double(betas[1]),
                                              C.c_double(eps), int(step), C.c_float(grad_scale),
                                              _lib.ptr(self._grad_bad) if guard else None, _stream())
            _lib.check(rc, "nrms_adam_step_rest")
            return
        if guard:
            rc = self.lib.nrms_adam_step_guarded(C.c_size_t(flat.numel()), _lib.ptr(flat), _lib.ptr(gflat), _lib.ptr(exp_avg),
                                                 _lib.ptr(exp_avg_sq), C.c_double(lr), C.c_double(betas[0]), C.c_double(betas[1]),
                                                 C.c_double(eps), int(step), C.c_float(grad_scale), _lib.ptr(self._grad_bad), _stream())
            _lib.check(rc, "nrms_adam_step_guarded")
            return
        rc = self.lib.nrms_adam_step(C.c_size_t(flat.numel()), _lib.ptr(flat), _lib.ptr(gflat), _lib.ptr(exp_avg),
                                     _lib.ptr(exp_avg_sq), C.c_double(lr), C.c_double(betas[0]), C.c_double(betas[1]),
                                     C.c_double(eps), int(step), C.c_float(grad_scale), _stream())
        _lib.check(rc, "nrms_adam_step")

    def grad_guard(self, gflat):
        rc = self.lib.nrms_grad_guard(C.c_size_t(gflat.numel()), _lib.ptr(gflat), _lib.ptr(self._grad_bad), _stream())
        _lib.check(rc, "nrms_grad_guard")

    def note_grad_check(self):
        if self._grad_bad_event is not None and not self._grad_bad_event.query():
            return
        self._grad_bad_host.copy_(self._grad_bad, non_blocking=True)
        ev = torch.cuda.Event()
        ev.record()
        self._grad_bad_event = ev

    def poll_grad_overflow(self, block=False):
        ev = self._grad_bad_event
        if ev is None:
            return self.loss_scale_backoff
        if block:
            ev.synchronize()
        elif not ev.query():
            return self.loss_scale_backoff
        self._grad_bad_event = None
        n = int(self._grad_bad_host.item())
        if n:
            self._grad_bad.zero_()
            self._grad_bad_host.zero_()
            self.grad_overflow_steps += 1
            self._clean_polls = 0
            if self.loss_scale_backoff < 24:
                self.loss_scale_backoff = min(24, self.loss_scale_backoff + 2)
            import warnings
            warnings.warn("NRMS fp16 backward: %d non-finite gradient element(s) were skipped by the optimizer (an fp16 overflow of "
                          "the loss-scaled gradient tensors, or an inf / nan loss); loss-scale head room raised to 2^%d below the "
                          "default" % (n, self.loss_scale_backoff), RuntimeWarning, stacklevel=2)
        else:
            self._clean_polls += 1
            if self._clean_polls >= 2000 and self.loss_scale_backoff > 0:
                self.loss_scale_backoff -= 1
                self._clean_polls = 0
        return self.loss_scale_backoff

    def impression_auc(self, scores, labels, lens):
        n, cmax = scores.shape
        auc = torch.empty(n, dtype=torch.float64, device=self.device)
        rc = self.lib.nrms_impression_auc(n, cmax, _lib.ptr(scores.contiguous()), _lib.ptr(labels.contiguous()),
                                          _lib.ptr(lens.contiguous()), _lib.ptr(auc), _stream())
        _lib.check(rc, "nrms_impression_auc")
        return auc

    def impression_metrics(self, scores, labels, lens, ks=(5, 10), ranks=False):
        return impression_metrics(self.lib, self.device, scores, labels, lens, ks, ranks)
# ... 372 lines not shown
```

Measured before the change: 175,600 users/s.

## Fold dout absmax into click-bwd and user-encoder dx epilogues; overlap fp16 prep on side stream

The fp16 news-encoder backward used to launch a separate absmax pass over the gradient of the news vectors before casting it to fp16. The max is now gathered with atomicMax inside the click-score backward and the user-encoder dx GEMM epilogue, which write those rows, and passed in so the standalone absmax kernel is skipped. The word is reset by the reduction kernel for the next step. Weight-tile prep for the fp16 backward is also launched on a side stream so it overlaps with this work. This adds cross-kernel coupling through one shared word and more stream-event bookkeeping.

```diff
diff --git a/include/nrms_hip.h b/include/nrms_hip.h
--- a/include/nrms_hip.h
+++ b/include/nrms_hip.h
@@ -106,6 +106,12 @@
                           const nrms_encoder_acts* acts, const float* dout,
                           const nrms_encoder_grads* grads, float* dx,
                           void* workspace, size_t workspace_bytes, const nrms_table_adam* table_adam, void* stream);
+int nrms_encoder_bwd_absmax(const nrms_encoder_desc* desc, const nrms_encoder_weights* w,
+                            const int64_t* ids, const float* x, const uint8_t* mask,
+                            const nrms_encoder_acts* acts, const float* dout,
+                            const nrms_encoder_grads* grads, float* dx,
+                            void* workspace, size_t workspace_bytes, const nrms_table_adam* table_adam, uint32_t* absmax,
+                            void* stream);
 int nrms_encoder_bwd_wqkv(const nrms_encoder_desc* desc, const int64_t* ids, const float* x,
                           const nrms_encoder_acts* acts, const nrms_encoder_grads* grads,
                           void* workspace, size_t workspace_bytes, void* stream);
@@ -124,6 +130,10 @@
 int nrms_click_score_bwd(int32_t B, int32_t C, int32_t d, const float* cand, const float* user,
                          const uint8_t* mask, const float* dscores, float* dcand, float* duser,
                          void* stream);
+
+int nrms_click_score_bwd_absmax(int32_t B, int32_t C, int32_t d, const float* cand, const float* user,
+                                const uint8_t* mask, const float* dscores, float* dcand, float* duser,
+                                uint32_t* absmax, void* stream);
 
 int nrms_ce_loss_fwd_bwd(int32_t B, int32_t C, const float* scores, float* loss_sum,
                          float* dscores, float grad_scale, void* stream);
diff --git a/pytorch_news_recommender_amd/_lib.py b/pytorch_news_recommender_amd/_lib.py
--- a/pytorch_news_recommender_amd/_lib.py
+++ b/pytorch_news_recommender_amd/_lib.py
@@ -91,6 +91,9 @@
     "nrms_encoder_bwd_adam": (C.c_int, [C.POINTER(EncoderDesc), C.POINTER(EncoderWeights), C.c_void_p, C.c_void_p,
                                         C.c_void_p, C.POINTER(EncoderActs), C.c_void_p, C.POINTER(EncoderGrads), C.c_void_p,
                                         C.c_void_p, C.c_size_t, C.POINTER(TableAdam), C.c_void_p]),
+    "nrms_encoder_bwd_absmax": (C.c_int, [C.POINTER(EncoderDesc), C.POINTER(EncoderWeights), C.c_void_p, C.c_void_p, C.c_void_p,
+                                          C.POINTER(EncoderActs), C.c_void_p, C.POINTER(EncoderGrads), C.c_void_p,
+                                          C.c_void_p, C.c_size_t, C.POINTER(TableAdam), C.c_void_p, C.c_void_p]),
     "nrms_encoder_bwd_wqkv": (C.c_int, [C.POINTER(EncoderDesc), C.c_void_p, C.c_void_p, C.POINTER(EncoderActs),
                                         C.POINTER(EncoderGrads), C.c_void_p, C.c_size_t, C.c_void_p]),
     "nrms_encoder_join": (C.c_int, [C.c_void_p]),
@@ -104,6 +107,8 @@
                                        C.c_void_p, C.c_void_p]),
     "nrms_click_score_bwd": (C.c_int, [C.c_int32, C.c_int32, C.c_int32, C.c_void_p, C.c_void_p, C.c_void_p,
                                        C.c_void_p, C.c_void_p, C.c_void_p, C.c_void_p]),
+    "nrms_click_score_bwd_absmax": (C.c_int, [C.c_int32, C.c_int32, C.c_int32, C.c_void_p, C.c_void_p, C.c_void_p,
+                                              C.c_void_p, C.c_void_p, C.c_void_p, C.c_void_p, C.c_void_p]),
     "nrms_ce_loss_fwd_bwd": (C.c_int, [C.c_int32, C.c_int32, C.c_void_p, C.c_void_p, C.c_void_p, C.c_float,
                                        C.c_void_p]),
     "nrms_adam_step": (C.c_int, [C.c_size_t, C.c_void_p, C.c_void_p, C.c_void_p, C.c_void_p, C.c_double,
diff --git a/pytorch_news_recommender_amd/csrc/capi.hip b/pytorch_news_recommender_amd/csrc/capi.hip
--- a/pytorch_news_recommender_amd/csrc/capi.hip
+++ b/pytorch_news_recommender_amd/csrc/capi.hip
@@ -380,7 +380,7 @@
 
 static int encoder_bwd16(const nrms_encoder_desc* desc, const nrms_encoder_weights* w, const int64_t* ids, const float* x,
                          const nrms_encoder_acts* acts, const float* dout, const nrms_encoder_grads* grads, float* dx,
-                         void* workspace, size_t workspace_bytes, const TableAdam* tadam, hipStream_t s) {
+                         void* workspace, size_t workspace_bytes, const TableAdam* tadam, unsigned* dout_absmax, hipStream_t s) {
     NRMS_REQUIRE(w && acts && dout && grads && workspace, "encoder_bwd(fp16): null argument");
     const bool v1 = desc->use_output_proj != 0;
     NRMS_REQUIRE(!v1 || (w->w_o && acts->attn && grads->w_o && grads->b_o),
@@ -393,7 +393,13 @@
     const Bwd16Layout L = bwd16_layout(desc);
     if (workspace_bytes < L.total) { set_error("encoder_bwd(fp16): workspace %zu < required %zu bytes", workspace_bytes, L.total); return NRMS_EWORKSPACE; }
     NRMS_REQUIRE(((uintptr_t)workspace & 255) == 0, "encoder_bwd(fp16): workspace must be 256-byte aligned");
-    if (desc->n_seq == 0) return NRMS_OK;
+    if (desc->n_seq == 0) {
+        if (dout_absmax != nullptr && hipMemsetAsync(dout_absmax, 0, sizeof(uint32_t), s) != hipSuccess) {
+            set_error("encoder_bwd(fp16): memset failed");
+            return NRMS_ELAUNCH;
+        }
+        return NRMS_OK;
+    }
     const int S = desc->seq_len, d = desc->d_model;
     const long M = (long)desc->n_seq * S;
     char* base = (char*)workspace;
@@ -406,6 +412,7 @@
     f.drop = make_dropout(desc->seed, desc->p_drop_ctx);
     f.dw_qkv = grads->w_qkv; f.db_qkv = grads->b_qkv; f.dw_add = grads->w_add; f.db_add = grads->b_add; f.dq_vec = grads->q_vec;
     if (v1) { f.w_o = w->w_o; f.attn16 = acts->attn; f.dw_o = grads->w_o; f.db_o = grads->b_o; }
+    f.dout_absmax = dout_absmax;
     int rc;
     int* live = (int*)(base + L.live);
     int* n_live = (int*)(base + L.n_live);
@@ -439,6 +446,9 @@
     } else {
         f.dx = dx;
     }
+    rc = launch_prep16b_side(f, s, &f.prep_on_side);
+    if (rc) return rc;
+    SideJoinGuard prep_guard(f.prep_on_side ? side_streams_for(s) : nullptr, s);
     SideSet* ss_prep = (gather && skip_pad_rows(desc)) ? side_streams_for(s) : nullptr;
     bool prepared = false;
     if (ss_prep != nullptr) {
@@ -457,6 +467,7 @@
     const float* sc_dev = nullptr;
     f.sc_out = &sc_dev;
     f.defer_join = (desc->flags & NRMS_FLAG_DEFER_WQKV) != 0;
+    prep_guard.disarm();
     rc = v1 ? launch_fused_bwd16v1(f, s) : launch_fused_bwd16(f, s);
     {
         const int rj = join_prepare();
@@ -695,7 +706,7 @@
 static int encoder_bwd_chain(const nrms_encoder_desc* desc, const nrms_encoder_weights* w, const int64_t* ids,
                              const float* x, const uint8_t* mask, const nrms_encoder_acts* acts, const float* dout,
                              const nrms_encoder_grads* grads, float* dx, void* workspace, size_t workspace_bytes,
-                             const TableAdam* tadam, hipStream_t s) {
+                             const TableAdam* tadam, unsigned* dx_absmax, hipStream_t s) {
     int rc;
     NRMS_REQUIRE(w && acts && dout && grads && workspace, "encoder_bwd: null argument");
     NRMS_REQUIRE(acts->qkv && acts->ctx && acts->t && acts->w, "encoder_bwd: all saved activations are required");
@@ -743,6 +754,7 @@
     };
 
     const bool fused64 = (desc->flags & NRMS_FLAG_FUSED_SEQ64) != 0;
+    const HeadPerm perm{d / desc->n_heads, desc->n_heads};
     if (fused64) {
         rc = launch_user64_bwd(desc->n_seq, S, d, desc->n_heads, q, w->w_add, w->q_vec, base + L.u64planes, dout, acts->t, acts->w,
                                acts->qkv, ds, dq_partial, grads->q_vec, dqkv, s);
@@ -807,7 +819,6 @@
     int* pos = (int*)(base + L.pos);
     int* n_live = (int*)(base + L.n_live);
     const bool compact = skip_pad_rows(desc);
-    const HeadPerm perm{d / desc->n_heads, desc->n_heads};
     if (gather) {
         rc = launch_compact_live_rows((long)M, ids, live, compact ? pos : nullptr, n_live, (int*)(base + L.cscr), s);
         if (rc) return rc;
@@ -836,6 +847,7 @@
         g.M = M; g.N = d; g.K = 3 * d; g.rows_per_tile = NT_BM;
         g.A = dqkv; g.lda = 3 * d; g.W = wqkv_t;
         g.C = gather ? dctx : dx; g.ldc = d;
+        if (!gather) g.absmax = dx_absmax;
         if (gather) { g.a_rows = compact ? nullptr : live; g.m_dev = n_live; }
         if (side && wo && gather && hipStreamWaitEvent(s, ss->ev[3], 0) != hipSuccess) {
             set_error("encoder_bwd: hipStreamWaitEvent failed");
@@ -870,15 +882,31 @@
                                 const float* x, const uint8_t* mask, const nrms_encoder_acts* acts, const float* dout,
                                 const nrms_encoder_grads* grads, float* dx, void* workspace, size_t workspace_bytes,
                                 void* stream) {
-    return nrms_encoder_bwd_adam(desc, w, ids, x, mask, acts, dout, grads, dx, workspace, workspace_bytes, nullptr, stream);
+    return nrms_encoder_bwd_absmax(desc, w, ids, x, mask, acts, dout, grads, dx, workspace, workspace_bytes, nullptr, nullptr, stream);
 }
 
 extern "C" int nrms_encoder_bwd_adam(const nrms_encoder_desc* desc, const nrms_encoder_weights* w, const int64_t* ids,
                                      const float* x, const uint8_t* mask, const nrms_encoder_acts* acts, const float* dout,
                                      const nrms_encoder_grads* grads, float* dx, void* workspace, size_t workspace_bytes,
                                      const nrms_table_adam* table_adam, void* stream) {
+    return nrms_encoder_bwd_absmax(desc, w, ids, x, mask, acts, dout, grads, dx, workspace, workspace_bytes, table_adam, nullptr, stream);
+}
+
+extern "C" int nrms_encoder_bwd_absmax(const nrms_encoder_desc* desc, const nrms_encoder_weights* w, const int64_t* ids,
+                                       const float* x, const uint8_t* mask, const nrms_encoder_acts* acts, const float* dout,
+                                       const nrms_encoder_grads* grads, float* dx, void* workspace, size_t workspace_bytes,
+                                       const nrms_table_adam* table_adam, uint32_t* absmax, void* stream) {
     int rc = validate_desc(desc, "encoder_bwd");
     if (rc) return rc;
+    unsigned* dx_absmax = nullptr;
+    unsigned* dout_absmax = nullptr;
+    if (absmax != nullptr) {
+        NRMS_REQUIRE(((uintptr_t)absmax & 3) == 0, "encoder_bwd: absmax must be 4-byte aligned");
+        if (desc->vocab == 0 && desc->precision != NRMS_PRECISION_FP16) dx_absmax = (unsigned*)absmax;
+        else if (desc->vocab > 0 && desc->precision == NRMS_PRECISION_FP16 && !desc->use_output_proj) dout_absmax = (unsigned*)absmax;
+        else NRMS_REQUIRE(false, "encoder_bwd: absmax belongs to a user encoder (vocab == 0) in fp32 / bf16x3 / bf16, which folds its dx "
+                                 "into it, or to the NRMS_PRECISION_FP16 news encoder (vocab > 0) without use_output_proj, which reads it");
+    }
     NRMS_REQUIRE(((desc->flags & NRMS_FLAG_TABLE_ADAM) != 0) == (table_adam != nullptr),
                  "encoder_bwd: NRMS_FLAG_TABLE_ADAM and the nrms_table_adam operands (nrms_encoder_bwd_adam) go together");
     TableAdam tadam_v{};
@@ -891,9 +919,10 @@
                      "encoder_bwd: NRMS_FLAG_TABLE_ADAM needs the grouped scatter (NRMS_ATOMIC_SCATTER is set)");
     }
     if (desc->precision == NRMS_PRECISION_FP16)
-        rc = encoder_bwd16(desc, w, ids, x, acts, dout, grads, dx, workspace, workspace_bytes, tadam, (hipStream_t)stream);
+        rc = encoder_bwd16(desc, w, ids, x, acts, dout, grads, dx, workspace, workspace_bytes, tadam, dout_absmax, (hipStream_t)stream);
     else
-        rc = encoder_bwd_chain(desc, w, ids, x, mask, acts, dout, grads, dx, workspace, workspace_bytes, tadam, (hipStream_t)stream);
+        rc = encoder_bwd_chain(desc, w, ids, x, mask, acts, dout, grads, dx, workspace, workspace_bytes, tadam, dx_absmax,
+                               (hipStream_t)stream);
     if (rc == NRMS_OK && tadam != nullptr && desc->n_seq == 0) {
         const size_t n = (size_t)desc->vocab * desc->d_model;
         if (hipMemsetAsync(grads->table, 0, n * sizeof(float), (hipStream_t)stream) != hipSuccess) {
diff --git a/pytorch_news_recommender_amd/csrc/common.h b/pytorch_news_recommender_amd/csrc/common.h
--- a/pytorch_news_recommender_amd/csrc/common.h
+++ b/pytorch_news_recommender_amd/csrc/common.h
@@ -160,10 +160,11 @@
 void set_error(const char* fmt, ...);
 int check_launch(const char* what);
 
-constexpr int SIDE_EVENTS = 9, SIDE_EV_USER = 8;
+constexpr int SIDE_EVENTS = 11, SIDE_EV_USER = 8;
+constexpr int SIDE_EV_PREP_FORK = 9, SIDE_EV_PREP_JOIN = 10;
 struct SideSet {
     hipStream_t s[2] = {nullptr, nullptr};
-    hipEvent_t ev[SIDE_EVENTS] = {nullptr, nullptr, nullptr, nullptr, nullptr, nullptr, nullptr, nullptr, nullptr};
+    hipEvent_t ev[SIDE_EVENTS] = {};
     bool pending = false;
     bool pending_user = false;
 };
diff --git a/pytorch_news_recommender_amd/csrc/fused16_bwd.hip b/pytorch_news_recommender_amd/csrc/fused16_bwd.hip
--- a/pytorch_news_recommender_amd/csrc/fused16_bwd.hip
+++ b/pytorch_news_recommender_amd/csrc/fused16_bwd.hip
@@ -906,7 +906,8 @@
 }
 
 __global__ __launch_bounds__(1024) void red16_kernel(const float* red, int n_wg, int h, int dk, int d, int q, const float* sc,
-                                                    float qscale, float* db_qkv, float* db_add, float* dq_vec) {
+                                                    float qscale, float* db_qkv, float* db_add, float* dq_vec, unsigned* zero_word) {
+    if (zero_word != nullptr && blockIdx.x == 0 && threadIdx.x == 0) *zero_word = 0u;
     const float inv_scale = sc[1];
     __shared__ float part[32][33];
     const int c = threadIdx.x & 31, rg = threadIdx.x >> 5;
@@ -1066,23 +1067,58 @@
     unsigned* max_bits = (unsigned*)(sc + 2);
     if (hipMemsetAsync(max_bits, 0, sizeof(unsigned), stream) != hipSuccess) { set_error("fused_bwd16: memset failed"); return NRMS_ELAUNCH; }
     const long nd = n_seq * d;
-    if (!(fixed_scale > 0.f))
+    if (!(fixed_scale > 0.f)) {
+        TimingScope ts("absmax", stream);
         hipLaunchKernelGGL(absmax_kernel, dim3(nd > 512L * 1024 ? 512 : (int)cdiv(nd, 1024)), dim3(256), 0, stream, nd, dout, max_bits);
+    }
     hipLaunchKernelGGL(dout16_kernel, dim3(cdiv(n_seq * F16_DP, 256) > 4096 ? 4096 : cdiv(n_seq * F16_DP, 256)),
                        dim3(256), 0, stream, n_seq, d, h, dk, fixed_scale, max_bits, sc, dout, dout16);
     return check_launch("dout16");
 }
 
 static int launch_dout16_maps(long n_seq, int d, int h, int dk, int q, float fixed_scale, float qscale, float* sc, const float* dout,
-                              _Float16* dout16, const Maps16& m, hipStream_t stream) {
-    unsigned* max_bits = (unsigned*)(sc + 2);
+                              _Float16* dout16, const Maps16& m, const unsigned* given_max, hipStream_t stream) {
+    const unsigned* max_bits = given_max != nullptr ? given_max : (const unsigned*)(sc + 2);
     const long nd = n_seq * d;
-    if (!(fixed_scale > 0.f))
-        hipLaunchKernelGGL(absmax_kernel, dim3(nd > 512L * 1024 ? 512 : (int)cdiv(nd, 1024)), dim3(256), 0, stream, nd, dout, max_bits);
+    if (!(fixed_scale > 0.f) && given_max == nullptr) {
+        TimingScope ts("absmax", stream);
+        hipLaunchKernelGGL(absmax_kernel, dim3(nd > 512L * 1024 ? 512 : (int)cdiv(nd, 1024)), dim3(256), 0, stream, nd, dout,
+                           (unsigned*)(sc + 2));
+    }
     const int row_blocks = cdiv(n_seq * F16_DP, 256) > 4096 ? 4096 : cdiv(n_seq * F16_DP, 256);
     hipLaunchKernelGGL(dout16_maps_kernel, dim3(row_blocks + MAPS16_BLOCKS), dim3(256), 0, stream, n_seq, d, h, dk, q, fixed_scale,
                        qscale, max_bits, sc, dout, dout16, m);
     return check_launch("dout16");
+}
+
+static int launch_prep16b(const Fused16Bwd& f, unsigned* max_bits, hipStream_t stream) {
+    const Fused16BwdLayout L = fused16_bwd_layout((long)f.n_seq * f.S, f.n_seq);
+    char* base = (char*)f.workspace;
+    Prep16bArgs p{};
+    p.d = f.d; p.h = f.h; p.dk = f.d / f.h; p.q = f.q; p.w_qkv = f.w_qkv; p.b_qkv = f.b_qkv; p.w_add = f.w_add; p.q_vec = f.q_vec;
+    p.btiles = (_Float16*)(base + L.btiles); p.xtiles = (_Float16*)(base + L.xtiles); p.qv16 = (_Float16*)(base + L.qv16);
+    p.bqkv32 = (float*)(base + L.bqkv32);
+    p.max_bits = max_bits;
+    TimingScope ts("prep16", stream);
+    hipLaunchKernelGGL(prep16b_kernel, dim3(2048), dim3(256), 0, stream, p);
+    return check_launch("prep16b");
+}
+
+int launch_prep16b_side(const Fused16Bwd& f, hipStream_t stream, bool* on_side) {
+    *on_side = false;
+    if (f.n_seq <= 0 || f.dout_absmax == nullptr) return NRMS_OK;
+    { const int jr = fused_bwd16_join(stream, false); if (jr) return jr; }
+    SideSet* ss = side_streams_for(stream);
+    if (ss == nullptr) return NRMS_OK;
+    SideJoinGuard guard(ss, stream);
+    int rc = side_order(ss, SIDE_EV_PREP_FORK, stream, ss->s[1], "fused_bwd16");
+    if (rc) return rc;
+    rc = launch_prep16b(f, nullptr, ss->s[1]);
+    if (rc) return rc;
+    if (hipEventRecord(ss->ev[SIDE_EV_PREP_JOIN], ss->s[1]) != hipSuccess) { set_error("fused_bwd16: hipEventRecord failed"); return NRMS_ELAUNCH; }
+    guard.disarm();
+    *on_side = true;
+    return NRMS_OK;
 }
 
 int launch_fused_bwd16(const Fused16Bwd& f, hipStream_t stream) {
@@ -1118,19 +1154,20 @@
     SideJoinGuard join_guard(ss, stream);
     const int Mp = f.n_seq * 32 * (f.S > 32 ? 2 : 1);
     {
-        Prep16bArgs p{};
-        p.d = f.d; p.h = f.h; p.dk = dk; p.q = f.q; p.w_qkv = f.w_qkv; p.b_qkv = f.b_qkv; p.w_add = f.w_add; p.q_vec = f.q_vec;
-        p.btiles = btiles; p.xtiles = xtiles; p.qv16 = qv16; p.bqkv32 = bqkv32;
-        p.max_bits = (unsigned*)(sc + 2);
-        TimingScope ts("prep16", stream);
-        hipLaunchKernelGGL(prep16b_kernel, dim3(2048), dim3(256), 0, stream, p);
-        int rc = check_launch("prep16b");
-        if (rc) return rc;
+        int rc;
+        if (!f.prep_on_side) {
+            rc = launch_prep16b(f, f.dout_absmax != nullptr ? nullptr : (unsigned*)(sc + 2), stream);
+            if (rc) return rc;
+        }
         Maps16 mp;
         mp.nmap_qkv = nmap_qkv; mp.nscale_qkv = nscale_qkv; mp.kmap_x = kmap_x; mp.nmap_add = nmap_add; mp.nscale_add = nscale_add;
         mp.kmap_ctx = kmap_ctx;
-        rc = launch_dout16_maps((long)f.n_seq, f.d, f.h, dk, f.q, f.loss_scale, qscale, sc, f.dout, dout16, mp, stream);
+        rc = launch_dout16_maps((long)f.n_seq, f.d, f.h, dk, f.q, f.loss_scale, qscale, sc, f.dout, dout16, mp, f.dout_absmax, stream);
         if (rc) return rc;
+        if (f.prep_on_side && hipStreamWaitEvent(stream, ss->ev[SIDE_EV_PREP_JOIN], 0) != hipSuccess) {
+            set_error("fused_bwd16: hipStreamWaitEvent failed");
+            return NRMS_ELAUNCH;
+        }
     }
     Bwd16Args a{};
     a.n_seq = f.n_seq; a.S = f.S; a.d = f.d; a.h = f.h; a.dk = dk; a.q = f.q;
@@ -1198,7 +1235,7 @@
     if (rc == NRMS_OK) {
         TimingScope ts("red16", stream);
         hipLaunchKernelGGL(red16_kernel, dim3(cdiv(B16_RED, 32)), dim3(1024), 0, stream, red, 2 * n_wg, f.h, dk, f.d, f.q, sc,
-                           qscale, f.db_qkv, f.db_add, f.dq_vec);
+                           qscale, f.db_qkv, f.db_add, f.dq_vec, f.dout_absmax);
         rc = check_launch("red16");
     }
     if (side && rc == NRMS_OK) {
diff --git a/pytorch_news_recommender_amd/csrc/gemm.h b/pytorch_news_recommender_amd/csrc/gemm.h
--- a/pytorch_news_recommender_amd/csrc/gemm.h
+++ b/pytorch_news_recommender_amd/csrc/gemm.h
@@ -28,6 +28,7 @@
     const int* a_rows;
     const int* m_dev;
     const int* c_rows;
+    unsigned* absmax;
 };
 
 __device__ __forceinline__ int nt_swz(int row) { return (0x1230 >> (((row >> 2) & 3) * 4)) & 3; }
@@ -121,8 +122,8 @@
 }
 
 template <int NT, int EMODE>
-__device__ __forceinline__ void nt_epilogue(const NTArgs& g, const f32x4 (&acc)[2][NT], int row0, int rows_valid,
-                                            int col0, int wave, int lane, float* wave_lds) {
+__device__ __forceinline__ unsigned nt_epilogue(const NTArgs& g, const f32x4 (&acc)[2][NT], int row0, int rows_valid,
+                                                int col0, int wave, int lane, float* wave_lds) {
     constexpr int S = 16 * NT + 8;
     constexpr int F4_ROW = 4 * NT;
     constexpr int LPR = F4_ROW >= 64 ? 64 : F4_ROW;
@@ -143,6 +144,12 @@
         return v + g.wrow[gr] * *reinterpret_cast<const f32x4*>(g.dout + seq * (long)g.N + n);
     };
     const bool dropped = g.drop.thresh != 0u;
+    const bool track = EMODE == E_STORE && g.absmax != nullptr;
+    unsigned amax = 0u;
+    auto fold = [&](const f32x4& v) {
+#pragma unroll
+        for (int e = 0; e < 4; ++e) amax = max(amax, __float_as_uint(v[e]) & 0x7FFFFFFFu);
+    };
     auto rem_pos = [&](int idx, int rbase, int& sr, int& c4, int& rl, int& n) {
         constexpr int REMD = REM > 0 ? REM : 1;
         sr = idx / REMD; c4 = 64 + idx - sr * REMD;
@@ -199,6 +206,7 @@
                     const long gr = (long)row0 + rl;
                     f32x4 v = *reinterpret_cast<const f32x4*>(wave_lds + sr * S + 4 * c4a);
                     if (!dropped) v = fix(v, gr, na, bias_a);
+                    if (track) fold(v);
                     *reinterpret_cast<f32x4*>(g.C + (g.c_rows != nullptr ? (long)g.c_rows[gr] : gr) * g.ldc + na) = v;
                 }
             }
@@ -213,6 +221,7 @@
                         if (EMODE == E_STORE && g.bias != nullptr) b4 = *reinterpret_cast<const f32x4*>(g.bias + n);
                         v = fix(v, gr, n, b4);
                     }
+                    if (track) fold(v);
                     *reinterpret_cast<f32x4*>(g.C + (g.c_rows != nullptr ? (long)g.c_rows[gr] : gr) * g.ldc + n) = v;
                 }
             }
@@ -220,6 +229,20 @@
             __builtin_amdgcn_wave_barrier();
             __builtin_amdgcn_fence(__ATOMIC_ACQUIRE, "wavefront");
         }
+    }
+    return amax;
+}
+
+__device__ __forceinline__ void nt_block_absmax(unsigned m, unsigned* words, unsigned* dst) {
+#pragma unroll
+    for (int o = 32; o > 0; o >>= 1) m = max(m, (unsigned)__shfl_xor((int)m, o, 64));
+    const int n_waves = (int)blockDim.x >> 6;
+    __syncthreads();
+    if ((threadIdx.x & 63) == 0) words[threadIdx.x >> 6] = m;
+    __syncthreads();
+    if (threadIdx.x == 0) {
+        for (int w = 1; w < n_waves; ++w) m = max(m, words[w]);
+        if (m != 0u) atomicMax(dst, m);
     }
 }
 
@@ -318,8 +341,11 @@
     const float** sc_out;
     bool defer_join;
     const float* w_o; const void* attn16; float* dw_o; float* db_o;
+    unsigned* dout_absmax;
+    bool prep_on_side;
 };
 int launch_fused_bwd16(const Fused16Bwd& f, hipStream_t stream);
+int launch_prep16b_side(const Fused16Bwd& f, hipStream_t stream, bool* on_side);
 size_t fused16v1_bwd_bytes(long M, int n_seq, int h);
 int launch_fused_bwd16v1(const Fused16Bwd& f, hipStream_t stream);
 int fused_bwd16_join(hipStream_t stream, bool user = true);
diff --git a/pytorch_news_recommender_amd/csrc/gemm.hip b/pytorch_news_recommender_amd/csrc/gemm.hip
--- a/pytorch_news_recommender_amd/csrc/gemm.hip
+++ b/pytorch_news_recommender_amd/csrc/gemm.hip
@@ -25,7 +25,8 @@
 
     static_assert(4 * 8 * (16 * NT + 8) <= 2 * (NT_BM + 16 * NT) * NT_BK, "epilogue strips must fit the stage buffers");
     const int lane = threadIdx.x & 63, wave = __builtin_amdgcn_readfirstlane(threadIdx.x >> 6);
-    nt_epilogue<NT, EMODE>(a, acc, row0, rows_valid, col0, wave, lane, lds + wave * 8 * (16 * NT + 8));
+    const unsigned amax = nt_epilogue<NT, EMODE>(a, acc, row0, rows_valid, col0, wave, lane, lds + wave * 8 * (16 * NT + 8));
+    if (EMODE == E_STORE && a.absmax != nullptr) nt_block_absmax(amax, reinterpret_cast<unsigned*>(lds), a.absmax);
 }
 
 template <int NT, int AMODE, int EMODE>
diff --git a/pytorch_news_recommender_amd/csrc/gemm_bf16.hip b/pytorch_news_recommender_amd/csrc/gemm_bf16.hip
--- a/pytorch_news_recommender_amd/csrc/gemm_bf16.hip
+++ b/pytorch_news_recommender_amd/csrc/gemm_bf16.hip
@@ -234,8 +234,9 @@
     bf16_nt_mainloop<NT, AMODE, NPASS>(a, row0, rows_valid, col0, acc, smem);
 
     const int lane = threadIdx.x & 63, wave = __builtin_amdgcn_readfirstlane(threadIdx.x >> 6);
-    nt_epilogue<NT, EMODE>(g, acc, row0, rows_valid, col0, wave, lane,
-                           reinterpret_cast<float*>(smem) + wave * 8 * (16 * NT + 8));
+    const unsigned amax = nt_epilogue<NT, EMODE>(g, acc, row0, rows_valid, col0, wave, lane,
+                                                 reinterpret_cast<float*>(smem) + wave * 8 * (16 * NT + 8));
+    if (EMODE == E_STORE && g.absmax != nullptr) nt_block_absmax(amax, reinterpret_cast<unsigned*>(smem), g.absmax);
 }
 
 template <int NT, int AMODE, int EMODE, int NPASS>
diff --git a/pytorch_news_recommender_amd/csrc/pool.hip b/pytorch_news_recommender_amd/csrc/pool.hip
--- a/pytorch_news_recommender_amd/csrc/pool.hip
+++ b/pytorch_news_recommender_amd/csrc/pool.hip
@@ -259,19 +259,33 @@
     if (lane == 0) scores[u] = (mask != nullptr && mask[u] == 0) ? -1e9f : (ok ? p : __builtin_nanf(""));
 }
 
-__global__ void click_bwd_kernel(int B, int C, int d, const float* cand, const float* user, const uint8_t* mask,
-                                 const float* dscores, float* dcand, float* duser) {
+constexpr int CLICK_BWD_THREADS = 128;
+__global__ __launch_bounds__(CLICK_BWD_THREADS) void click_bwd_kernel(int B, int C, int d, const float* cand, const float* user, const uint8_t* mask,
+                                 const float* dscores, float* dcand, float* duser, unsigned* absmax) {
     const int b = blockIdx.x;
+    unsigned m = 0u;
     for (int k = threadIdx.x; k < d; k += blockDim.x) {
         const float uv = user[(long)b * d + k];
         float du = 0.f;
         for (int c = 0; c < C; ++c) {
             const long u = (long)b * C + c;
             const float g = (mask != nullptr && mask[u] == 0) ? 0.f : dscores[u];
-            dcand[u * d + k] = g * uv;
+            const float dc = g * uv;
+            dcand[u * d + k] = dc;
+            m = max(m, __float_as_uint(dc) & 0x7FFFFFFFu);
             du += g * cand[u * d + k];
         }
         duser[(long)b * d + k] = du;
+    }
+    if (absmax == nullptr) return;
+#pragma unroll
+    for (int o = 32; o > 0; o >>= 1) m = max(m, (unsigned)__shfl_xor((int)m, o, 64));
+    __shared__ unsigned wmax[CLICK_BWD_THREADS / 64];
+    if ((threadIdx.x & 63) == 0) wmax[threadIdx.x >> 6] = m;
+    __syncthreads();
+    if (threadIdx.x == 0) {
+        for (int w = 1; w < CLICK_BWD_THREADS / 64; ++w) m = max(m, wmax[w]);
+        if (m != 0u) atomicMax(absmax, m);
     }
 }
 
@@ -455,15 +469,23 @@
     return check_launch("click_indexed");
 }
 
+extern "C" int nrms_click_score_bwd_absmax(int32_t B, int32_t C, int32_t d, const float* cand, const float* user,
+                                           const uint8_t* mask, const float* dscores, float* dcand, float* duser,
+                                           uint32_t* absmax, void* stream) {
+    NRMS_REQUIRE(B >= 0 && C > 0 && d > 0 && cand && user && dscores && dcand && duser, "click_score_bwd: bad arguments");
+    NRMS_REQUIRE(((uintptr_t)absmax & 3) == 0, "click_score_bwd: absmax must be 4-byte aligned");
+    if (B == 0) return NRMS_OK;
+    hipStream_t s = (hipStream_t)stream;
+    TimingScope ts("click_bwd", s);
+    hipLaunchKernelGGL(click_bwd_kernel, dim3(B), dim3(CLICK_BWD_THREADS), 0, s, B, C, d, cand, user, mask, dscores, dcand, duser,
+                       (unsigned*)absmax);
+    return check_launch("click_bwd");
+}
+
 extern "C" int nrms_click_score_bwd(int32_t B, int32_t C, int32_t d, const float* cand, const float* user,
                                     const uint8_t* mask, const float* dscores, float* dcand, float* duser,
                                     void* stream) {
-    NRMS_REQUIRE(B >= 0 && C > 0 && d > 0 && cand && user && dscores && dcand && duser, "click_score_bwd: bad arguments");
-    if (B == 0) return NRMS_OK;
-    hipStream_t s = (hipStream_t)stream;
-    TimingScope ts("click_bwd", s);
-    hipLaunchKernelGGL(click_bwd_kernel, dim3(B), dim3(128), 0, s, B, C, d, cand, user, mask, dscores, dcand, duser);
-    return check_launch("click_bwd");
+    return nrms_click_score_bwd_absmax(B, C, d, cand, user, mask, dscores, dcand, duser, nullptr, stream);
 }
 
 extern "C" int nrms_ce_loss_fwd_bwd(int32_t B, int32_t C, const float* scores, float* loss_sum, float* dscores,
diff --git a/pytorch_news_recommender_amd/engine.py b/pytorch_news_recommender_amd/engine.py
--- a/pytorch_news_recommender_amd/engine.py
+++ b/pytorch_news_recommender_amd/engine.py
@@ -125,6 +125,8 @@
         self._bufs = {}
         self._saved = None
         self._fuse_table_adam = os.environ.get("NRMS_NO_FUSED_TABLE_ADAM", "0") in ("", "0")
+        self._fold_absmax = os.environ.get("NRMS_NO_ABSMAX_FOLD", "0") in ("", "0")
+        self._absmax_word = torch.zeros(1, dtype=torch.int32, device=self.device)
         self.fp16_user_encoder = False
         self.fp16_backward = True
         self.loss_scale = 0.0
@@ -380,7 +382,7 @@
         return self._buf("bwd_ws", (nbytes + 3) // 4)
 
     def encode_users_backward(self, flat, gflat, news_vectors, dout, dx=None, tag="user", mask=None, mask_mode=0,
-                              defer_join=False):
+                              defer_join=False, dx_absmax=None):
         B, H, d = news_vectors.shape
         if dx is None:
             dx = torch.empty(B * H, d, dtype=torch.float32, device=self.device)
@@ -393,10 +395,10 @@
             ws = self._bwd_workspace(desc)
         w, g = self._weights(flat, "user_encoder"), self._grads(gflat, "user_encoder")
         acts = self._acts(tag, B * H, True, desc=desc)
-        rc = self.lib.nrms_encoder_bwd(C.byref(desc), C.byref(w), None, _lib.ptr(news_vectors),
-                                       _lib.ptr(None if mask is None else mask.contiguous()), C.byref(acts),
-                                       _lib.ptr(dout.contiguous()), C.byref(g), _lib.ptr(dx), _lib.ptr(ws),
-                                       C.c_size_t(ws.numel() * 4), _stream())
+        rc = self.lib.nrms_encoder_bwd_absmax(C.byref(desc), C.byref(w), None, _lib.ptr(news_vectors),
+                                              _lib.ptr(None if mask is None else mask.contiguous()), C.byref(acts),
+                                              _lib.ptr(dout.contiguous()), C.byref(g), _lib.ptr(dx), _lib.ptr(ws),
+                                              C.c_size_t(ws.numel() * 4), None, dx_absmax, _stream())
         _lib.check(rc, "nrms_encoder_bwd(user)")
         return dx[:B * H].view(B, H, d)
 
@@ -413,7 +415,7 @@
         duser = self._buf("d_user_vec", B * width)[:B * width].view(B, width)
         return sv[key][B * H:], sv["user"], dvec, duser
 
-    def _head_backward(self, dscores, gen, width):
+    def _head_backward(self, dscores, gen, width, absmax=None):
         sv = self._saved
         if sv is None:
             raise _lib.NrmsError("backward() without a training forward()")
@@ -427,9 +429,10 @@
                 raise _lib.NrmsError("backward(dscores=None) needs the gradients of pooled_ce_loss(), and none was computed for "
                                      "training forward #%d" % sv["gen"])
         else:
-            rc = self.lib.nrms_click_score_bwd(B, Cn, width, _lib.ptr(cand), _lib.ptr(user), _lib.ptr(sv["mask"]),
-                                               _lib.ptr(dscores.contiguous()), C.c_void_p(dvec[B * H:].data_ptr()), _lib.ptr(duser),
-                                               _stream())
+            word = absmax(sv) if absmax is not None else None
+            rc = self.lib.nrms_click_score_bwd_absmax(B, Cn, width, _lib.ptr(cand), _lib.ptr(user), _lib.ptr(sv["mask"]),
+                                                      _lib.ptr(dscores.contiguous()), C.c_void_p(dvec[B * H:].data_ptr()),
+                                                      _lib.ptr(duser), word, _stream())
             _lib.check(rc, "nrms_click_score_bwd")
         return sv, dvec, duser
 
@@ -492,8 +495,25 @@
                 or not self._fp16_ok("news_encoder", sv["L"], 0, True))
 
     def backward(self, flat, gflat, dscores=None, table_grad_ready=None, gen=None, table_adam=None):
+        try:
+            self._backward(flat, gflat, dscores, table_grad_ready, gen, table_adam)
+        except BaseException:
+            self._absmax_word.zero_()
+            raise
+
+    def _folds_absmax(self, sv, dscores):
+        if not self._fold_absmax or dscores is None or self.precision != "fp16" or self.dims.output_proj:
+            return False
+        user_mask_mode = sv["user_mask_mode"] if sv["user_mask"] is not None else 0
+        return (self._fp16_ok("news_encoder", sv["L"], 0, True)
+                and not self._fp16_ok("user_encoder", sv["H"], user_mask_mode, True))
+
+    def _backward(self, flat, gflat, dscores, table_grad_ready, gen, table_adam):
         d = self.dims.word_embed_size
-        sv, dnv, duser = self._head_backward(dscores, gen, d)
+        word = self._absmax_word.data_ptr()
+        sv, dnv, duser = self._head_backward(dscores, gen, d,
+                                             absmax=lambda saved: word if self._folds_absmax(saved, dscores) else None)
+        fold = self._folds_absmax(sv, dscores)
         B, H, Cn, L = sv["B"], sv["H"], sv["C"], sv["L"]
         N = B * (H + Cn)
         self.poll_grad_overflow()
@@ -505,7 +525,7 @@
         ws = self._bwd_workspace(desc_u, desc_n)
         defer_user = desc_n.precision == _lib.NRMS_PRECISION_FP16 and not self.dims.output_proj
         self.encode_users_backward(flat, gflat, hist.view(B, H, d), duser, dx=dnv, tag="user", mask=sv["user_mask"],
-                                   mask_mode=sv["user_mask_mode"], defer_join=defer_user)
+                                   mask_mode=sv["user_mask_mode"], defer_join=defer_user, dx_absmax=word if fold else None)
         wn, gn = self._weights(flat, "news_encoder"), self._grads(gflat, "news_encoder")
         acts_n = self._acts("news", N * L, True, gather=True, desc=desc_n)
         if desc_n.precision == _lib.NRMS_PRECISION_FP16:
@@ -531,9 +551,10 @@
             desc_n.flags |= _lib.NRMS_FLAG_TABLE_ADAM
         rc_join = 0
         try:
-            rc = self.lib.nrms_encoder_bwd_adam(C.byref(desc_n), C.byref(wn), _lib.ptr(sv["ids"]), None, None, C.byref(acts_n),
-                                                _lib.ptr(dnv), C.byref(gn), None, _lib.ptr(ws),
-                                                C.c_size_t(ws.numel() * 4), None if ta is None else C.byref(ta), _stream())
+            rc = self.lib.nrms_encoder_bwd_absmax(C.byref(desc_n), C.byref(wn), _lib.ptr(sv["ids"]), None, None, C.byref(acts_n),
+                                                  _lib.ptr(dnv), C.byref(gn), None, _lib.ptr(ws),
+                                                  C.c_size_t(ws.numel() * 4), None if ta is None else C.byref(ta),
+                                                  word if fold else None, _stream())
             _lib.check(rc, "nrms_encoder_bwd(news)")
             if table_grad_ready is not None:
                 table_grad_ready()
```

After: 175,700 users/s, median of 2. No clear change (+0.0%).
